# spcl/gms

Measured on AMD Instinct MI355X. Metric: edges-intersected/sec + achieved HBM GB/s, RMAT-26 triangle count @1/2/4/8 GPU, higher is better.
Workload: dtype int32 ids / uint64 counts

## Files before the change

### gms_amd/capi.py

```python
import ctypes as C
import os
import weakref

import numpy as np

_HERE = os.path.dirname(os.path.abspath(__file__))
LIB_PATH = os.environ.get("GMSX_LIB") or os.path.join(_HERE, "lib", "libgmsx.so")

_i64p = np.ctypeslib.ndpointer(np.int64, flags="C_CONTIGUOUS")
_i32p = np.ctypeslib.ndpointer(np.int32, flags="C_CONTIGUOUS")
_u32p = np.ctypeslib.ndpointer(np.uint32, flags="C_CONTIGUOUS")

GEN_KRONECKER, GEN_UNIFORM = 0, 1
RELABEL_NEVER, RELABEL_AUTO, RELABEL_ALWAYS = 0, 1, 2
TC_AUTO, TC_ORIENTED, TC_FULL = 0, 1, 2
UPLOAD_DEFAULT, UPLOAD_TRUSTED, UPLOAD_FOR_TC = 0, 1, 2
PREPARE_TC = 1
SETOP_INTERSECT, SETOP_DIFFERENCE = 0, 1
OK, ERR_INVALID, ERR_NOMEM, ERR_IO, ERR_FORMAT, ERR_DIRECTED, ERR_NO_DEVICE = 0, -1, -2, -3, -4, -5, -6
ERR_DEVICE_MEM, ERR_NOT_CANONICAL, ERR_OVERFLOW, ERR_UNSUPPORTED, ERR_KERNEL, ERR_COMM, ERR_TIMEOUT = -7, -8, -9, -10, -11, -12, -13
COMM_ID_BYTES = 128

SYMBOLS = [
    "gmsx_strerror", "gmsx_version",
# ... 264 lines not shown
        _check(lib().gmsx_csr_save_sgx(self._h, os.fsencode(path)), "gmsx_csr_save_sgx")

    @property
    def is_mapped(self):
        return bool(lib().gmsx_csr_is_mapped(self._h))

    def relabel_by_degree(self):
        h = C.c_void_p()
        _check(lib().gmsx_csr_relabel_by_degree(self._h, C.byref(h)), "gmsx_csr_relabel_by_degree")
        return HostCSR(h)

    def worth_relabelling(self):
        return bool(lib().gmsx_csr_worth_relabelling(self._h))

    @property
    def num_nodes(self):
        return lib().gmsx_csr_num_nodes(self._h)

    @property
    def num_edges(self):
        return lib().gmsx_csr_num_edges(self._h)

    @property
    def nnz(self):
        return lib().gmsx_csr_num_edges_directed(self._h)

    def offsets(self):
        return np.ctypeslib.as_array(lib().gmsx_csr_offsets(self._h), shape=(self.num_nodes + 1,))

    def neighbors(self):
        nnz = self.nnz
        if nnz == 0:
            return np.zeros(0, dtype=np.int32)
        return np.ctypeslib.as_array(lib().gmsx_csr_neighbors(self._h), shape=(nnz,))

    def merge_elements(self):
        return int(lib().gmsx_csr_merge_elements(self._h))

    def fingerprint(self):
        return int(lib().gmsx_csr_fingerprint(self._h, 0)), int(lib().gmsx_csr_fingerprint(self._h, 1))

    def __del__(self):
        if getattr(self, "_h", None):
            lib().gmsx_csr_free(self._h)
            self._h = None


def set_host_threads(n=0):
    return int(lib().gmsx_set_host_threads(int(n)))


def set_option(name, value):
    _check(lib().gmsx_set_option(name.encode(), None if value is None else str(value).encode()), f"gmsx_set_option({name})")


def reset_options():
    lib().gmsx_reset_options()


def option_names():
    out, i, p = [], 0, C.c_char_p()
    while lib().gmsx_option_name(i, C.byref(p)) == 0:
        out.append(p.value.decode())
        i += 1
    return out


class options:

    def __init__(self, **kw):
        self.kw = kw

    def __enter__(self):
        for k, v in self.kw.items():
            set_option(k, v)
        return self

    def __exit__(self, *exc):
        for k in self.kw:
            set_option(k, None)
        return False


def init(device=-1):
    _check(lib().gmsx_init(device), "gmsx_init")


def set_stream(stream_ptr):
    _check(lib().gmsx_set_stream(C.c_void_p(stream_ptr)), "gmsx_set_stream")


def hbm_read_probe(nbytes=4 << 30, iterations=20):
    v = C.c_double(0)
    _check(lib().gmsx_hbm_read_probe(int(nbytes), int(iterations), C.byref(v)), "gmsx_hbm_read_probe")
    return v.value


def device_info():
    name = C.create_string_buffer(256)
    cu, mem = C.c_int(0), C.c_int64(0)
    _check(lib().gmsx_device_info(name, 256, C.byref(cu), C.byref(mem)), "gmsx_device_info")
    return {"name": name.value.decode(), "compute_units": cu.value, "hbm_bytes": mem.value}


class DeviceGraph:

    def __init__(self, handle):
        self._h = handle

    @classmethod
    def upload(cls, off, neigh, flags=UPLOAD_DEFAULT):
        off = np.ascontiguousarray(off, dtype=np.int64)
        neigh = np.ascontiguousarray(neigh, dtype=np.int32)
        h = C.c_void_p()
        _check(lib().gmsx_graph_upload(off.size - 1, off, neigh if neigh.size else np.zeros(1, np.int32), flags, C.byref(h)),
               "gmsx_graph_upload")
        g = cls(h)
        g._host = (weakref.ref(off), weakref.ref(neigh))
        return g

    @classmethod
    def from_csr(cls, csr, flags=UPLOAD_DEFAULT, shard=None):
        h = C.c_void_p()
        if shard is None:
            _check(lib().gmsx_graph_upload_csr(csr._h, flags, C.byref(h)), "gmsx_graph_upload_csr")
        else:
            _check(lib().gmsx_graph_upload_csr_shard(csr._h, flags, int(shard[0]), int(shard[1]), C.byref(h)), "gmsx_graph_upload_csr_shard")
        g = cls(h)
        g._host = (weakref.ref(csr),)
        return g

    num_nodes = property(lambda self: lib().gmsx_graph_num_nodes(self._h))
    num_edges = property(lambda self: lib().gmsx_graph_num_edges(self._h))
    device_bytes = property(lambda self: lib().gmsx_graph_device_bytes(self._h))
    max_out_degree = property(lambda self: lib().gmsx_graph_max_out_degree(self._h))
    tc_passes = property(lambda self: lib().gmsx_graph_tc_passes(self._h))

    def prepare(self, what=PREPARE_TC):
        _check(lib().gmsx_graph_prepare(self._h, what), "gmsx_graph_prepare")

    def tc_total(self, algo=TC_AUTO, stats=False):
        out, st = C.c_uint64(0), Stats()
        _check(lib().gmsx_tc_total(self._h, algo, C.byref(out), C.byref(st)), "gmsx_tc_total")
        return (int(out.value), st.as_dict()) if stats else int(out.value)

    def tc_partial(self, part, nparts, algo=TC_AUTO, stats=False):
        out, st = C.c_uint64(0), Stats()
        _check(lib().gmsx_tc_partial(self._h, algo, part, nparts, C.byref(out), C.byref(st)), "gmsx_tc_partial")
        return (int(out.value), st.as_dict()) if stats else int(out.value)

    BREAKDOWN = ["hub_rows_list", "hub_rows_bitset", "hub_rows_delta", "tail_rows_list", "tail_rows_delta", "entries", "pivot_containers",
                 "of_which_inline_rows", "light_streamed_hub_rows", "light_streamed_tail_rows", "light_pivot_lists_and_descriptors",
                 "count_entries", "count_inline_entries", "count_work_items", "count_light_streamed_members",
                 "core_matrix", "core_k", "reserved17", "reserved18", "reserved19", "reserved20"]
    BREAKDOWN_BYTES = ("hub_rows_list", "hub_rows_bitset", "hub_rows_delta", "tail_rows_list", "tail_rows_delta", "entries", "pivot_containers",
                       "light_streamed_hub_rows", "light_streamed_tail_rows", "light_pivot_lists_and_descriptors", "core_matrix")

    def tc_stream_breakdown(self):
        out = np.zeros(21, dtype=np.uint64)
        _check(lib().gmsx_tc_stream_breakdown(self._h, out), "gmsx_tc_stream_breakdown")
        return dict(zip(self.BREAKDOWN, (int(x) for x in out)))

    def tc_row_histogram(self):
        out = np.zeros(256, dtype=np.uint64)
        _check(lib().gmsx_tc_row_histogram(self._h, out), "gmsx_tc_row_histogram")
        return out[:240].reshape(5, 24, 2).astype(np.int64), out[240:].astype(np.int64)

    def tc_comembership(self, batch):
        out = np.zeros(8, dtype=np.uint64)
        _check(lib().gmsx_tc_comembership(self._h, int(batch), out), "gmsx_tc_comembership")
        return dict(entries=int(out[0]), units=int(out[1]), distinct_rows=int(out[2]), batched_units=int(out[3]), items=int(out[4]))

    def tc_vertex_count2(self, stats=False):
        c, st = np.zeros(self.num_nodes, dtype=np.int64), Stats()
        _check(lib().gmsx_tc_vertex_count2(self._h, c, C.byref(st)), "gmsx_tc_vertex_count2")
        return (c, st.as_dict()) if stats else c

    def intersect_count_batch(self, u, v, stats=False):
        u = np.ascontiguousarray(u, dtype=np.int32)
        v = np.ascontiguousarray(v, dtype=np.int32)
        out, st = np.zeros(max(u.size, 1), dtype=np.uint32), Stats()
        _check(lib().gmsx_intersect_count_batch(self._h, u.size, u if u.size else np.zeros(1, np.int32),
                                                v if v.size else np.zeros(1, np.int32), out, C.byref(st)),
               "gmsx_intersect_count_batch")
        out = out[:u.size]
        return (out, st.as_dict()) if stats else out

    def set_op_batch(self, op, u, v, stats=False):
        code = {"intersect": SETOP_INTERSECT, "difference": SETOP_DIFFERENCE}[op]
        u = np.ascontiguousarray(u, dtype=np.int32)
        v = np.ascontiguousarray(v, dtype=np.int32)
        uu, vv = (u if u.size else np.zeros(1, np.int32)), (v if v.size else np.zeros(1, np.int32))
        off, st = np.zeros(u.size + 1, dtype=np.int64), Stats()
        _check(lib().gmsx_set_op_batch(self._h, code, u.size, uu, vv, off, None, 0, C.byref(st)), "gmsx_set_op_batch (sizing)")
        ids = np.zeros(max(int(off[-1]), 1), dtype=np.int32)
        _check(lib().gmsx_set_op_batch(self._h, code, u.size, uu, vv, off, ids.ctypes.data_as(C.c_void_p), int(off[-1]), C.byref(st)), "gmsx_set_op_batch")
        ids = ids[:int(off[-1])]
        return (off, ids, st.as_dict()) if stats else (off, ids)

    SIM = {"jaccard": 0, "overlap": 1, "adamic_adar": 2, "resource": 3, "common_neighbors": 4, "total_neighbors": 5, "pref_attachment": 6}

    def vertex_similarity_batch(self, metric, u, v, stats=False):
        u = np.ascontiguousarray(u, dtype=np.int32)
        v = np.ascontiguousarray(v, dtype=np.int32)
        out, st = np.zeros(max(u.size, 1), dtype=np.float64), Stats()
        m = self.SIM[metric] if isinstance(metric, str) else int(metric)
        _check(lib().gmsx_vertex_similarity_batch(self._h, m, u.size, u if u.size else np.zeros(1, np.int32),
                                                  v if v.size else np.zeros(1, np.int32), out, C.byref(st)), "gmsx_vertex_similarity_batch")
        out = out[:u.size]
        return (out, st.as_dict()) if stats else out

    def kclique_count(self, k, stats=False):
        ordered, cliques, st = C.c_uint64(0), C.c_uint64(0), Stats()
        _check(lib().gmsx_kclique_count(self._h, k, C.byref(ordered), C.byref(cliques), C.byref(st)), "gmsx_kclique_count")
        r = (int(ordered.value), int(cliques.value))
        return (r + (st.as_dict(),)) if stats else r

    def kclique_star_count(self, k, members=True, stats=False):
        stars, mem, st = C.c_uint64(0), C.c_uint64(0), Stats()
        _check(lib().gmsx_kclique_star_count(self._h, k, C.byref(stars), C.byref(mem) if members else None, C.byref(st)), "gmsx_kclique_star_count")
        r = (int(stars.value), int(mem.value) if members else None)
        return (r + (st.as_dict(),)) if stats else r

    def kclique_star_list_info(self, k, cliques_only=False, part=0, nparts=1):
        info = KcliqueStarListInfo()
        flags = KCSTAR_CLIQUES_ONLY if cliques_only else KCSTAR_DEFAULT
        _check(lib().gmsx_kclique_star_list(self._h, k, flags, part, nparts, None, None, None, 0, 0, C.byref(info), None),
               "gmsx_kclique_star_list (sizing)")
        return info.as_dict()

    def kclique_star_list(self, k, cliques_only=False, part=0, nparts=1, stats=False):
        info, st = KcliqueStarListInfo(), Stats()
        flags = KCSTAR_CLIQUES_ONLY if cliques_only else KCSTAR_DEFAULT
        _check(lib().gmsx_kclique_star_list(self._h, k, flags, part, nparts, None, None, None, 0, 0, C.byref(info), C.byref(st)),
               "gmsx_kclique_star_list (sizing)")
        sizing = st.as_dict()
        nc, nm = int(info.cliques), int(info.star_members)
        cl = np.zeros(max(nc * k, 1), dtype=np.int32)
        soff = mem = None
        if not cliques_only:
            soff = np.zeros(nc + 1, dtype=np.int64)
            mem = np.zeros(max(nm, 1), dtype=np.int32)
        _check(lib().gmsx_kclique_star_list(self._h, k, flags, part, nparts, cl.ctypes.data_as(C.c_void_p),
                                            None if cliques_only else soff.ctypes.data_as(C.c_void_p),
                                            None if cliques_only else mem.ctypes.data_as(C.c_void_p), nc, nm, C.byref(info), C.byref(st)),
               "gmsx_kclique_star_list")
        cl = cl[:nc * k].reshape(nc, k)
        if mem is not None:
            mem = mem[:nm]
        if stats:
            return cl, soff, mem, {"sizing": sizing, "fill": st.as_dict(), "info": info.as_dict()}
        return cl, soff, mem

    def kclique_partial(self, k, part, nparts, stats=False):
        out, st = C.c_uint64(0), Stats()
        _check(lib().gmsx_kclique_partial(self._h, k, part, nparts, C.byref(out), C.byref(st)), "gmsx_kclique_partial")
        return (int(out.value), st.as_dict()) if stats else int(out.value)

    def bk_count(self, rank=None, stats=False):
        out, st = C.c_uint64(0), Stats()
        rp = None
        if rank is not None:
            rank = np.ascontiguousarray(rank, dtype=np.int32)
            rp = rank.ctypes.data_as(C.c_void_p)
        _check(lib().gmsx_bk_count(self._h, rp, C.byref(out), C.byref(st)), "gmsx_bk_count")
        return (int(out.value), st.as_dict()) if stats else int(out.value)

    def bk_partial(self, part, nparts, rank=None, stats=False):
        out, st = C.c_uint64(0), Stats()
        rp = None
        if rank is not None:
            rank = np.ascontiguousarray(rank, dtype=np.int32)
            rp = rank.ctypes.data_as(C.c_void_p)
        _check(lib().gmsx_bk_partial(self._h, rp, part, nparts, C.byref(out), C.byref(st)), "gmsx_bk_partial")
        return (int(out.value), st.as_dict()) if stats else int(out.value)

    def bk_list_info(self, rank=None, part=0, nparts=1):
        info = BkListInfo()
        rp = None
        if rank is not None:
            rank = np.ascontiguousarray(rank, dtype=np.int32)
            rp = rank.ctypes.data_as(C.c_void_p)
        _check(lib().gmsx_bk_list(self._h, rp, part, nparts, None, None, 0, 0, C.byref(info), None), "gmsx_bk_list (sizing)")
        return info.as_dict()

    def bk_list(self, rank=None, part=0, nparts=1, stats=False):
        info, st = BkListInfo(), Stats()
        rp = None
        if rank is not None:
            rank = np.ascontiguousarray(rank, dtype=np.int32)
            rp = rank.ctypes.data_as(C.c_void_p)
        _check(lib().gmsx_bk_list(self._h, rp, part, nparts, None, None, 0, 0, C.byref(info), C.byref(st)), "gmsx_bk_list (sizing)")
        sizing = st.as_dict()
        off = np.zeros(int(info.cliques) + 1, dtype=np.int64)
        mem = np.zeros(max(int(info.members), 1), dtype=np.int32)
        _check(lib().gmsx_bk_list(self._h, rp, part, nparts, off.ctypes.data_as(C.c_void_p), mem.ctypes.data_as(C.c_void_p), off.size,
                                  int(info.members), C.byref(info), C.byref(st)), "gmsx_bk_list")
        mem = mem[:int(info.members)]
        if stats:
            return off, mem, {"sizing": sizing, "fill": st.as_dict(), "info": info.as_dict()}
        return off, mem

    def adg_rank(self, epsilon=0.001, rank_format=True, stats=False):
        out, rounds, st = np.zeros(max(self.num_nodes, 1), dtype=np.int32), C.c_int32(0), Stats()
        _check(lib().gmsx_adg_rank(self._h, float(epsilon), int(bool(rank_format)), out, C.byref(rounds), C.byref(st)), "gmsx_adg_rank")
        r = (out[:self.num_nodes], int(rounds.value))
        return (r + (st.as_dict(),)) if stats else r
# ... 182 lines not shown
```

### gms_amd/csrc/hip/device_graph.hip

```cpp
#include "device_graph.hpp"

#include <algorithm>
#include <mutex>
#include <array>
#include <chrono>
#include <cstdio>
#include <cstdlib>
#include <cstring>
#include <memory>
#include <new>
#include <random>

#include <rocprim/device/device_radix_sort.hpp>
#include <rocprim/device/device_scan.hpp>
#include <rocprim/device/device_segmented_radix_sort.hpp>
#include <rocprim/iterator/transform_iterator.hpp>

#include "../host/gmsx_internal.hpp"
#include "../host/tc_core_plan.hpp"
#include "kc4_mfma.hpp"

namespace gmsx {

Ctx &ctx() {
// ... 235 lines not shown
            int rf = kFormList;
            if (rl >= 24 && delta_mode > 0) {
                const uint32_t d = delta_encode(hadj + b + k, rl, nullptr);
                if (d * 100u <= r * uint32_t(delta_pct)) { r = d; rf = kFormDelta; }
            }
            const uint32_t cand = uint32_t(B / 128) + r;
            if (cand < tot && (hybrid_mode == 2 || cand * 100u <= best * 90u)) {
                tot = cand;
                ks = k;
                best2 = r;
                form2 = rf;
            }
        }
        if (ks > 0) {
            best = tot - best2;
            form = kFormBitset;
        }
    }
    ksplit[v] = ks;
    const uint32_t u2[2] = {best, best2};
    const int f2[2] = {form, form2};
    for (int sl = 0; sl < 2; ++sl) {
        const bool big = u2[sl] >= 8u;
        units_out[2 * v + sl] = big ? int64_t((u2[sl] + 7u) & ~7u) : 0;
        small_out[2 * v + sl] = big ? 0 : int64_t(u2[sl]);
        real_out[2 * v + sl] = u2[sl];
        form_out[2 * v + sl] = (unsigned char)f2[sl];
    }
}
__global__ void k_srow_fill(int64_t n, const int64_t *__restrict__ hoff, const uint16_t *__restrict__ hadj, const int64_t *__restrict__ bmoff,
                            const uint32_t *__restrict__ bmpool, const int64_t *__restrict__ uoff, const int64_t *__restrict__ soff,
                            const uint32_t *__restrict__ real, const unsigned char *__restrict__ form, const int32_t *__restrict__ ksplit,
                            unsigned long long *__restrict__ srow, unsigned long long *__restrict__ srow2, uint32_t *__restrict__ spool) {
    const int64_t v = int64_t(blockIdx.x) * blockDim.x + threadIdx.x;
    if (v >= n) return;
    const int64_t b = hoff[v];
    const int len = int(hoff[v + 1] - b);
    const int ks = ksplit[v];
    for (int sl = 0; sl < 2; ++sl) {
        const int64_t units = int64_t(real[2 * v + sl]);
        const int64_t u0 = units >= 8 ? uoff[2 * v + sl] : uoff[2 * n] + soff[2 * v + sl];
        const int fm = form[2 * v + sl];
        const unsigned long long d = units ? ((unsigned long long)u0 << 24) | ((unsigned long long)fm << 22) | (unsigned long long)units : 0ull;
        if (sl == 0) srow[v] = units ? d : ((unsigned long long)u0 << 24) | ((unsigned long long)fm << 22);
        else srow2[v] = d;
        if (units == 0) continue;
        uint32_t *dst = spool + u0 * 4;
        const uint16_t *row = hadj + b + (sl ? ks : 0);
        const int rl = sl ? len - ks : len;
        if (sl == 0 && ks > 0) {
            for (int64_t w = 0; w < units * 4; ++w) dst[w] = 0;
            for (int i = 0; i < ks; ++i) dst[row[i] >> 5] |= 1u << (row[i] & 31u);
        } else if (fm == kFormDelta) {
            delta_encode(row, rl, dst);
        } else if (fm == kFormGap12) {
            gap12_encode(row, rl, dst);
        } else if (fm == kFormBitset) {
            const uint32_t *src = bmpool + bmoff[v];
            for (int64_t w = 0; w < units * 4; ++w) dst[w] = src[w];
        } else {
            for (int64_t w = 0; w < units * 4; ++w) {
                const int i = int(w) * 2;
                const uint32_t lo = i < rl ? row[i] : 0xFFFFu, hi = i + 1 < rl ? row[i + 1] : 0xFFFFu;
                dst[w] = lo | (hi << 16);
            }
        }
    }
}

__device__ inline uint32_t tail_delta_encode(const int32_t *__restrict__ row, int len, uint32_t *__restrict__ emit) {
    uint32_t units = 0;
    int i = 0;
    while (i < len) {
        uint32_t w[4] = {uint32_t(row[i]), 0u, 0u, 0u};
        uint32_t cur = uint32_t(row[i]);
        int slot = 1;
        ++i;
        while (i < len && slot < 6) {
            const uint32_t gap = uint32_t(row[i]) - cur;
            if (gap > 65535u) break;
            w[1 + (slot >> 1)] |= gap << ((slot & 1) * 16);
            ++slot;
            cur = uint32_t(row[i]);
            ++i;
        }
        w[1] |= uint32_t(slot);
        if (emit) {
            emit[units * 4 + 0] = w[0]; emit[units * 4 + 1] = w[1]; emit[units * 4 + 2] = w[2]; emit[units * 4 + 3] = w[3];
        }
        ++units;
    }
    return units;
}
__global__ void k_trow_sizes(int64_t n, const int64_t *__restrict__ toff, const int32_t *__restrict__ tadj, int delta_mode,
                             int64_t *__restrict__ units_out, int64_t *__restrict__ small_out, uint32_t *__restrict__ real_out, unsigned char *__restrict__ form_out) {
    const int64_t v = int64_t(blockIdx.x) * blockDim.x + threadIdx.x;
    if (v > n) return;
    if (v == n) { units_out[n] = 0; small_out[n] = 0; return; }
    const int64_t b = toff[v];
    const int len = int(toff[v + 1] - b);
    uint32_t best = uint32_t((len + 3) / 4);
    int form = kFormList;
    if (len >= 8 && delta_mode > 0) {
        const uint32_t d = tail_delta_encode(tadj + b, len, nullptr);
        if (delta_mode == 2 || d * 100u <= best * 85u) { best = d; form = kFormDelta; }
    }
    const bool big = best >= 8u;
    units_out[v] = big ? int64_t((best + 7u) & ~7u) : 0;
    small_out[v] = big ? 0 : int64_t(best);
    real_out[v] = best;
    form_out[v] = (unsigned char)form;
}
__global__ void k_trow_fill(int64_t n, const int64_t *__restrict__ toff, const int32_t *__restrict__ tadj, const int64_t *__restrict__ uoff,
                            const int64_t *__restrict__ soff, const uint32_t *__restrict__ real, const unsigned char *__restrict__ form,
                            unsigned long long *__restrict__ trow, uint32_t *__restrict__ tpool) {
    const int64_t v = int64_t(blockIdx.x) * blockDim.x + threadIdx.x;
    if (v >= n) return;
    const int64_t units = int64_t(real[v]);
    const int64_t u0 = units >= 8 ? uoff[v] : uoff[n] + soff[v];
    trow[v] = ((unsigned long long)u0 << 24) | ((unsigned long long)form[v] << 22) | (unsigned long long)units;
    if (units == 0) return;
    uint32_t *dst = tpool + u0 * 4;
    const int64_t b = toff[v];
    const int64_t len = toff[v + 1] - b;
    if (form[v] == kFormDelta) tail_delta_encode(tadj + b, int(len), dst);
    else
        for (int64_t w = 0; w < units * 4; ++w) dst[w] = w < len ? uint32_t(tadj[b + w]) : 0xfffffffeu;
}

__global__ void k_dense_sizes(int32_t limit, const int32_t *__restrict__ dplus, int64_t *__restrict__ sizes) {
    const int32_t v = int32_t(blockIdx.x * blockDim.x + threadIdx.x);
    if (v < limit) sizes[v] = bitset_words(v);
    if (v == limit) sizes[v] = 0;
}
__global__ __launch_bounds__(256) void k_dense_fill(int32_t limit, const int64_t *__restrict__ hoff, const uint16_t *__restrict__ hadj,
                                                    const int64_t *__restrict__ toff, const int32_t *__restrict__ tadj,
                                                    const int64_t *__restrict__ bmoff, uint32_t *__restrict__ pool) {
    const int lane = threadIdx.x & 63;
    const int32_t wave0 = int32_t((int64_t(blockIdx.x) * blockDim.x + threadIdx.x) >> 6);
    const int32_t nwaves = int32_t((int64_t(gridDim.x) * blockDim.x) >> 6);
    for (int32_t v = wave0; v < limit; v += nwaves) {
        const int64_t b = bmoff[v];
        if (bmoff[v + 1] == b) continue;
        for (int64_t j = hoff[v] + lane; j < hoff[v + 1]; j += 64) {
            const uint32_t id = hadj[j];
            if (id != 0xFFFFu) atomicOr(&pool[b + (id >> 5)], 1u << (id & 31u));
        }
        for (int64_t j = toff[v] + lane; j < toff[v + 1]; j += 64) {
            const uint32_t id = uint32_t(tadj[j]);
            atomicOr(&pool[b + (id >> 5)], 1u << (id & 31u));
        }
    }
}
__global__ __launch_bounds__(256) void k_core_fill(int32_t K, int WS, const int64_t *__restrict__ hoff, const uint16_t *__restrict__ hadj,
                                                   uint32_t *__restrict__ bits) {
    const int lane = threadIdx.x & 63;
    const int32_t wave0 = int32_t((int64_t(blockIdx.x) * blockDim.x + threadIdx.x) >> 6);
    const int32_t nwaves = int32_t((int64_t(gridDim.x) * blockDim.x) >> 6);
    for (int32_t i = wave0; i < K; i += nwaves)
        for (int64_t j = hoff[i] + lane; j < hoff[i + 1]; j += 64) {
            const uint32_t id = hadj[j];
            if (id < uint32_t(i)) atomicOr(&bits[size_t(i) * size_t(WS) + (id >> 5)], 1u << (id & 31u));
        }
}
__global__ __launch_bounds__(256) void k_core_units(int32_t cap, const int64_t *__restrict__ hoff, const uint16_t *__restrict__ hadj,
                                                    const int32_t *__restrict__ dplus, unsigned long long *__restrict__ bucket) {
    const int lane = threadIdx.x & 63;
    const int32_t wave0 = int32_t((int64_t(blockIdx.x) * blockDim.x + threadIdx.x) >> 6);
    const int32_t nwaves = int32_t((int64_t(gridDim.x) * blockDim.x) >> 6);
    for (int32_t u = wave0; u < cap; u += nwaves) {
        const int64_t hb = hoff[u];
        const int hl = int(hoff[u + 1] - hb);
        unsigned long long units = 0;
        for (int i = lane; i < hl; i += 64) {
            const uint32_t v = hadj[hb + i];
            if (v >= uint32_t(u)) continue;
            const uint32_t ids = uint32_t(min(i, dplus[v]));
            units += min((ids + 7u) / 8u, (v + 127u) / 128u);
        }
        for (int s = 32; s > 0; s >>= 1) units += __shfl_down(units, s);
        if (lane == 0 && units) atomicAdd(&bucket[u / kTcCoreBucket], units);
    }
}
__global__ __launch_bounds__(256) void k_tail_split(int64_t n, const int64_t *__restrict__ toff, const int32_t *__restrict__ tadj, int32_t limit,
                                                    int32_t *__restrict__ tsplit) {
    const int lane = threadIdx.x & 63;
    const int64_t wave0 = (int64_t(blockIdx.x) * blockDim.x + threadIdx.x) >> 6;
    const int64_t nwaves = (int64_t(gridDim.x) * blockDim.x) >> 6;
    for (int64_t u = wave0; u < n; u += nwaves) {
        int c = 0;
        for (int64_t j = toff[u] + lane; j < toff[u + 1]; j += 64) c += tadj[j] < limit;
        for (int s = 32; s > 0; s >>= 1) c += __shfl_down(c, s);
        if (lane == 0) tsplit[u] = c;
    }
}

__global__ void k_order_keys(int64_t n, const int32_t *__restrict__ dplus, int32_t *__restrict__ keys, int32_t *__restrict__ vals) {
    const int64_t i = int64_t(blockIdx.x) * blockDim.x + threadIdx.x;
    if (i < n) {
        keys[i] = dplus[i];
        vals[i] = int32_t(i);
    }
}

__global__ void k_warm(unsigned long long *p) {
    if (p) p[0] = 0;
}
__global__ void k_count_ge(int64_t n, const int32_t *__restrict__ order, const int32_t *__restrict__ dplus, int32_t thr, int64_t *__restrict__ out) {
    int64_t lo = 0, hi = n;
    while (lo < hi) {
        const int64_t mid = (lo + hi) >> 1;
        if (dplus[order[mid]] >= thr) lo = mid + 1; else hi = mid;
    }
    out[0] = lo;
}
__global__ void k_task_limits(int64_t n, const unsigned long long *__restrict__ srow, const unsigned long long *__restrict__ srow2,
                              const unsigned long long *__restrict__ trow, uint32_t hub_max, uint32_t tail_max, unsigned long long *__restrict__ out) {
    const int64_t v = int64_t(blockIdx.x) * blockDim.x + threadIdx.x;
    if (v >= n) return;
    if ((srow[v] & 0x3fffffull) > hub_max || (srow2[v] & 0x3fffffull) > hub_max || (trow[v] & 0x3fffffull) > tail_max) atomicOr(out, 1ull);
}

static constexpr int kInlineChunk = 64;
static constexpr int kDefaultInlineFirst = 28;
static constexpr int kInlineFirstMax = 64;
__device__ __forceinline__ bool takes_inline(int32_t v, int32_t inline_limit, const int32_t *__restrict__ dplus) {
    return v < inline_limit || dplus[v] >= kHeavy;
}
template <bool FILL>
__global__ __launch_bounds__(256) void k_inline_rows(int64_t first, int64_t end, const int32_t *__restrict__ order, const int64_t *__restrict__ hoff,
                                                     const uint16_t *__restrict__ hadj, const int64_t *__restrict__ toff, const int32_t *__restrict__ tadj,
                                                     const int32_t *__restrict__ dplus, int32_t inline_limit, int inline_first, int32_t core, const int32_t *__restrict__ opos, int nparts, int part,
                                                     unsigned long long *__restrict__ cnt_h,
                                                     unsigned long long *__restrict__ cnt_t, const int64_t *__restrict__ ihoff,
                                                     const int64_t *__restrict__ itoff, int64_t base_h, uint16_t *__restrict__ pool_h, int64_t base_t,
                                                     int32_t *__restrict__ pool_t) {
    const int lane = threadIdx.x & 63;
    const int64_t wave0 = (int64_t(blockIdx.x) * blockDim.x + threadIdx.x) >> 6;
    const int64_t nwaves = (int64_t(gridDim.x) * blockDim.x) >> 6;
    for (int64_t pos = first + wave0; pos < end; pos += nwaves) {
        const int32_t u = order[pos];
        if (u < core) continue;
        const int64_t hb = hoff[u], tb = toff[u];
        const int first_u = dplus[u] >= kHeavy ? inline_first : kInlineFirstMax;
        const int hl = min(int(hoff[u + 1] - hb), first_u), tl = min(int(toff[u + 1] - tb), first_u - hl);
        int32_t mv = 0x7fffffff;
        if (lane < hl) {
            const uint32_t x = hadj[hb + lane];
            if (x != 0xFFFFu) mv = int32_t(x);
        } else if (lane - hl < tl) {
            mv = tadj[tb + (lane - hl)];
        }
        const bool valid = mv != 0x7fffffff, is_tail = valid && lane >= hl;
        const unsigned long long vmask = __ballot(valid);
        const int nhub = __popcll(__ballot(valid && lane < hl));
        const int below = __popcll(vmask & ((1ull << lane) - 1ull));
        const bool give = valid && below > 0 && takes_inline(mv, inline_limit, dplus);
        const bool mine = give && (nparts <= 1 || shard_of(opos[mv], nparts) == part);
        const int nh = mine ? (is_tail ? nhub : below) : 0;
        const int nt = mine && is_tail ? lane - hl : 0;
        if (!FILL) {
            if (nh) atomicAdd(&cnt_h[mv], (unsigned long long)nh);
            if (nt) atomicAdd(&cnt_t[mv], (unsigned long long)nt);
        } else {
            int64_t at_h = 0, at_t = 0;
            if (nh) at_h = (base_h + ihoff[mv]) * 8 + int64_t(atomicAdd(&cnt_h[mv], (unsigned long long)nh));
            if (nt) at_t = (base_t + itoff[mv]) * 4 + int64_t(atomicAdd(&cnt_t[mv], (unsigned long long)nt));
            for (int k = 0; k < nhub; ++k) {
                const int32_t x = __shfl(mv, k);
                if (k < nh) pool_h[at_h + k] = uint16_t(x);
            }
            for (int k = 0; k < tl; ++k) {
                const int32_t x = __shfl(mv, hl + k);
                if (k < nt) pool_t[at_t + k] = x;
            }
        }
    }
}
__global__ void k_inline_units(int64_t n, const unsigned long long *__restrict__ ids_h, const unsigned long long *__restrict__ ids_t,
                               int64_t *__restrict__ units_h, int64_t *__restrict__ units_t) {
    const int64_t v = int64_t(blockIdx.x) * blockDim.x + threadIdx.x;
    if (v > n) return;
    units_h[v] = v < n ? int64_t((ids_h[v] + 7) / 8) : 0;
    units_t[v] = v < n ? int64_t((ids_t[v] + 3) / 4) : 0;
}
static constexpr int kDefaultHotWindows = 0, kDefaultHotKB = 2048, kDefaultHotMin = 16;
__device__ __forceinline__ int64_t receiver_of(int32_t w, const int32_t *__restrict__ dplus, const int32_t *__restrict__ opos, const int64_t *__restrict__ lidx,
                                               int64_t n_heavy) {
    return dplus[w] >= kHeavy ? int64_t(opos[w]) : n_heavy + lidx[w];
}
__global__ void k_opos(int64_t n, const int32_t *__restrict__ order, int32_t *__restrict__ opos) {
    const int64_t p = int64_t(blockIdx.x) * blockDim.x + threadIdx.x;
    if (p < n) opos[order[p]] = int32_t(p);
}
__global__ void k_light_flags(int64_t limit, const int32_t *__restrict__ dplus, int64_t *__restrict__ flags) {
    const int64_t w = int64_t(blockIdx.x) * blockDim.x + threadIdx.x;
    if (w <= limit) flags[w] = (w < limit && dplus[w] < kHeavy) ? 1 : 0;
}
__global__ void k_recv_vertices(int64_t n_heavy, int64_t limit, const int32_t *__restrict__ order, const int32_t *__restrict__ dplus, const int64_t *__restrict__ lidx,
                                int32_t *__restrict__ recv_v) {
    const int64_t i = int64_t(blockIdx.x) * blockDim.x + threadIdx.x;
    if (i < n_heavy) recv_v[i] = order[i];
    if (i < limit && dplus[i] < kHeavy) recv_v[n_heavy + lidx[i]] = int32_t(i);
}
template <bool FILL>
__global__ void k_inline_entries(int64_t n, const int32_t *__restrict__ dplus, const int32_t *__restrict__ opos, const int64_t *__restrict__ lidx, int64_t n_heavy,
                                 int32_t inline_limit, const int64_t *__restrict__ ihoff, const int64_t *__restrict__ itoff, int64_t base_h, int64_t base_t,
                                 uint32_t *__restrict__ cnt, uint32_t *__restrict__ cur, const int64_t *__restrict__ hbeg, const int64_t *__restrict__ tbeg,
                                 TaskList htask, TaskList ttask, unsigned long long *__restrict__ totals, TcClasses cc) {
    const int kClasses = cc.count();
    const int64_t v = int64_t(blockIdx.x) * blockDim.x + threadIdx.x;
    if (v >= n) return;
    const int64_t uh = ihoff[v + 1] - ihoff[v], ut = itoff[v + 1] - itoff[v];
    if (uh == 0 && ut == 0) return;
    if (dplus[v] < kHeavy && v >= inline_limit) return;
    const int64_t p = receiver_of(int32_t(v), dplus, opos, lidx, n_heavy);
    uint32_t *c = cnt + p * kClasses;
    for (int64_t o = 0; o < uh; o += kInlineChunk) {
        const unsigned long long units = (unsigned long long)min(int64_t(kInlineChunk), uh - o);
        const unsigned long long d = ((unsigned long long)(base_h + ihoff[v] + o) << 24) | ((unsigned long long)kFormList << 22) | units;
        const int cls = hub_class(cc, d);
        if (!FILL) atomicAdd(&c[cls], 1u);
        else htask.put(hbeg[p] + c[cls] + atomicAdd(&cur[p * kClasses + cls], 1u), d);
    }
    for (int64_t o = 0; o < ut; o += kInlineChunk) {
        const unsigned long long units = (unsigned long long)min(int64_t(kInlineChunk), ut - o);
        const unsigned long long d = ((unsigned long long)(base_t + itoff[v] + o) << 24) | ((unsigned long long)kFormList << 22) | units;
        const int cls = tail_class(cc, d);
        if (!FILL) atomicAdd(&c[cls], 1u);
        else ttask.put(tbeg[p] + c[cls] + atomicAdd(&cur[p * kClasses + cls], 1u), d);
    }
    if (!FILL) {
        atomicAdd(&totals[0], (unsigned long long)((uh + kInlineChunk - 1) / kInlineChunk));
        atomicAdd(&totals[1], (unsigned long long)((ut + kInlineChunk - 1) / kInlineChunk));
    }
}
__global__ void k_list_sizes(int64_t n_recv, uint32_t *__restrict__ cnt, int64_t *__restrict__ hcnt, int64_t *__restrict__ tcnt, TcClasses cc) {
    const int kClasses = cc.count(), hub_end = cc.tail_base();
    const int64_t p = int64_t(blockIdx.x) * blockDim.x + threadIdx.x;
    if (p > n_recv) return;
    if (p == n_recv) { hcnt[p] = 0; tcnt[p] = 0; return; }
    uint32_t *c = cnt + p * kClasses;
    uint32_t run = 0;
    for (int k = 0; k < hub_end; ++k) { const uint32_t x = c[k]; c[k] = run; run += x; }
    hcnt[p] = run;
    run = 0;
    for (int k = hub_end; k < kClasses; ++k) { const uint32_t x = c[k]; c[k] = run; run += x; }
    tcnt[p] = run;
}

__global__ void k_ledge_count(int64_t first, int64_t end, const int32_t *__restrict__ order, const int64_t *__restrict__ toff, const int32_t *__restrict__ tadj,
                              const int32_t *__restrict__ tsplit, const int32_t *__restrict__ dplus, int32_t core, int64_t *__restrict__ cnt) {
    const int64_t pos = first + int64_t(blockIdx.x) * blockDim.x + threadIdx.x;
    if (pos > end) return;
    int64_t c = 0;
    if (pos < end) {
        const int32_t u = order[pos];
        const int64_t tb = toff[u];
        const int tl = int(toff[u + 1] - tb);
        if (u >= core)
            for (int i = tsplit[u]; i < tl; ++i) c += dplus[tadj[tb + i]] < kHeavy ? 1 : 0;
    }
    cnt[pos - first] = c;
}
__global__ void k_ledge_fill(int64_t first, int64_t end, const int32_t *__restrict__ order, const int64_t *__restrict__ hoff, const int64_t *__restrict__ toff,
                             const int32_t *__restrict__ tadj, const int32_t *__restrict__ tsplit, const int32_t *__restrict__ dplus,
                             int32_t core, const int64_t *__restrict__ ebeg, int nparts, int part, uint4 *__restrict__ ledge) {
    const int64_t pos = first + int64_t(blockIdx.x) * blockDim.x + threadIdx.x;
    if (pos >= end) return;
    const int32_t u = order[pos];
    if (u < core) return;
    const int64_t hb = hoff[u], tb = toff[u];
    const int tl = int(toff[u + 1] - tb);
    const unsigned long long hu = (unsigned long long)hb | ((unsigned long long)(hoff[u + 1] - hb) << 40);
    int64_t e = ebeg[pos - first];
    for (int i = tsplit[u]; i < tl; ++i) {
        const int32_t v = tadj[tb + i];
        if (dplus[v] >= kHeavy) continue;
        if (nparts <= 1 || shard_of(e, nparts) == part) {
            const unsigned long long tu = (unsigned long long)tb | ((unsigned long long)i << 40);
            const unsigned long long hv = (unsigned long long)hoff[v] | ((unsigned long long)(hoff[v + 1] - hoff[v]) << 40);
            const unsigned long long tv = (unsigned long long)toff[v] | ((unsigned long long)(toff[v + 1] - toff[v]) << 40);
            const int64_t slot = nparts <= 1 ? e : e / nparts;
            ledge[2 * slot] = make_uint4(uint32_t(hu), uint32_t(hu >> 32), uint32_t(tu), uint32_t(tu >> 32));
            ledge[2 * slot + 1] = make_uint4(uint32_t(hv), uint32_t(hv >> 32), uint32_t(tv), uint32_t(tv >> 32));
        }
        ++e;
    }
}

__device__ __forceinline__ uint32_t cut_hub_units(const uint32_t *__restrict__ spool, unsigned long long d, int below, int32_t v) {
    const uint32_t units = uint32_t(d) & 0x3fffffu, form = (uint32_t(d) >> 22) & 3u;
    if (form == kFormList) return min(units, uint32_t(below + 7) / 8u);
    if (form == kFormBitset) return min(units, uint32_t(v + 127) / 128u);
    const uint4 *row = reinterpret_cast<const uint4 *>(spool) + (d >> 24);
    uint32_t lo = 0, hi = units;
    while (lo < hi) {
        const uint32_t mid = (lo + hi) >> 1;
        if (int32_t(row[mid].x & 0xffffu) < v) lo = mid + 1; else hi = mid;
    }
    return lo;
}
__device__ __forceinline__ uint32_t cut_tail_units(const uint32_t *__restrict__ tpool, unsigned long long d, int below, int32_t v) {
    const uint32_t units = uint32_t(d) & 0x3fffffu, form = (uint32_t(d) >> 22) & 3u;
    if (form != kFormDelta) return min(units, uint32_t(below + 3) / 4u);
    const uint4 *row = reinterpret_cast<const uint4 *>(tpool) + (d >> 24);
    uint32_t lo = 0, hi = units;
    while (lo < hi) {
        const uint32_t mid = (lo + hi) >> 1;
        if (int32_t(row[mid].x) < v) lo = mid + 1; else hi = mid;
    }
    return lo;
}
__device__ __forceinline__ uint32_t claim_by_class(uint32_t *ctr, int cls, bool active, int lane) {
    uint32_t mine = 0;
    unsigned long long todo = __ballot(active);
    while (todo) {
        const int leader = __ffsll((long long)todo) - 1;
        const int c = __builtin_amdgcn_readlane(cls, leader);
        const unsigned long long same = __ballot(active && cls == c);
        uint32_t base = 0;
        if (lane == leader) base = atomicAdd(&ctr[c], uint32_t(__popcll(same)));
        base = uint32_t(__builtin_amdgcn_readlane(int(base), leader));
        if (active && cls == c) mine = base + uint32_t(__popcll(same & ((1ull << lane) - 1ull)));
        todo &= ~same;
    }
    return mine;
}
template <bool FILL>
__global__ __launch_bounds__(256) void k_task_lists(int64_t n_heavy, const int32_t *__restrict__ order, const int64_t *__restrict__ hoff,
                                                    const uint16_t *__restrict__ hadj, const int64_t *__restrict__ toff, const int32_t *__restrict__ tadj,
                                                    const int32_t *__restrict__ dplus, const unsigned long long *__restrict__ srow,
                                                    const unsigned long long *__restrict__ srow2, const int32_t *__restrict__ ksplit,
                                                    const unsigned long long *__restrict__ trow, int two_sided, const int32_t *__restrict__ opos,
                                                    uint32_t *__restrict__ cnt, uint32_t *__restrict__ cur, const int64_t *__restrict__ hbeg,
                                                    const int64_t *__restrict__ tbeg, TaskList htask, TaskList ttask,
                                                    int32_t *__restrict__ tunits, unsigned long long *__restrict__ reversed, const uint32_t *__restrict__ spool,
                                                    const uint32_t *__restrict__ tpool, int32_t inline_limit, int inline_first, int32_t core, int nparts, int part, TcClasses cc) {
    const int kClasses = cc.count();
    const int lane = threadIdx.x & 63;
    const int64_t wave0 = (int64_t(blockIdx.x) * blockDim.x + threadIdx.x) >> 6;
    const int64_t nwaves = (int64_t(gridDim.x) * blockDim.x) >> 6;
    unsigned long long rev = 0;
    for (int64_t pos = wave0; pos < n_heavy; pos += nwaves) {
        const int32_t u = order[pos];
        if (u < core) continue;
        const int64_t hb = hoff[u], tb = toff[u];
        const int hl = int(hoff[u + 1] - hb), tl = int(toff[u + 1] - tb);
        const unsigned long long du_s = srow[u], du_s2 = srow2[u], du_t = trow[u];
        const int ks_u = ksplit[u];
        uint32_t *cu = cnt + pos * kClasses, *ru = cur + pos * kClasses;
        const bool own_u = nparts <= 1 || shard_of(pos, nparts) == part;
        int kept = 0;
        for (int base = 0; base < hl + tl; base += 64) {
            const int i = base + lane;
            int32_t v = -1;
            if (i < hl) {
                const uint32_t x = hadj[hb + i];
                if (x != 0xFFFFu) v = int32_t(x);
            } else if (i < hl + tl) v = tadj[tb + i - hl];
            if (v >= 0 && i > 0 && i < inline_first && takes_inline(v, inline_limit, dplus)) v = -1;
            bool reverse = false;
            uint32_t ch = 0, ch2 = 0, ct = 0;
            if (v >= 0 && i > 0 && two_sided && dplus[v] >= kHeavy) {
                if (i < hl) {
                    ch = cut_hub_units(spool, du_s, i, v);
                    if (du_s2 && i > ks_u) ch2 = cut_hub_units(spool, du_s2, i - ks_u, v);
                } else {
                    ch = uint32_t(du_s) & 0x3fffffu;
                    ch2 = uint32_t(du_s2) & 0x3fffffu;
                }
                ct = (i < hl || toff[v + 1] == toff[v]) ? 0u : cut_tail_units(tpool, du_t, i - hl, v);
                const uint32_t keep = uint32_t(srow[v] & 0x3fffffull) + uint32_t(srow2[v] & 0x3fffffull) + (i > hl ? uint32_t(trow[v] & 0x3fffffull) : 0u);
                reverse = ch + ch2 + ct < keep;
            }
            const bool fwd = v >= 0 && !reverse && own_u;
            if (reverse && nparts > 1 && shard_of(opos[v], nparts) != part) v = -1;
            const unsigned long long fh = (fwd && i > 0) ? srow[v] : 0ull, fh2 = (fwd && i > 0) ? srow2[v] : 0ull, ft = (fwd && i > hl) ? trow[v] : 0ull;
            const bool fh_on = (fh & 0x3fffffull) != 0, fh2_on = (fh2 & 0x3fffffull) != 0, ft_on = (ft & 0x3fffffull) != 0;
            const uint32_t sh = claim_by_class(FILL ? ru : cu, hub_class(cc, fh), fh_on, lane);
            const uint32_t sh2 = claim_by_class(FILL ? ru : cu, hub_class(cc, fh2), fh2_on, lane);
            const uint32_t st = claim_by_class(FILL ? ru : cu, tail_class(cc, ft), ft_on, lane);
            if (FILL) {
                if (fh_on) htask.put(hbeg[pos] + cu[hub_class(cc, fh)] + sh, fh);
                if (fh2_on) htask.put(hbeg[pos] + cu[hub_class(cc, fh2)] + sh2, fh2);
                if (ft_on) ttask.put(tbeg[pos] + cu[tail_class(cc, ft)] + st, ft);
            }
            kept += __popcll(__ballot(fwd));
            if (v >= 0 && reverse) {
                const int64_t pv = opos[v];
                const unsigned long long rh = ch ? (du_s & ~0x3fffffull) | ch : 0ull, rh2 = ch2 ? (du_s2 & ~0x3fffffull) | ch2 : 0ull,
                                         rt = ct ? (du_t & ~0x3fffffull) | ct : 0ull;
                uint32_t *cv = cnt + pv * kClasses;
                if (!FILL) {
                    if (rh) atomicAdd(&cv[hub_class(cc, rh)], 1u);
                    if (rh2) atomicAdd(&cv[hub_class(cc, rh2)], 1u);
                    if (rt) atomicAdd(&cv[tail_class(cc, rt)], 1u);
                    atomicAdd(&tunits[pv], 1);
                    ++rev;
                } else {
                    uint32_t *rv = cur + pv * kClasses;
                    if (rh) htask.put(hbeg[pv] + cv[hub_class(cc, rh)] + atomicAdd(&rv[hub_class(cc, rh)], 1u), rh);
                    if (rh2) htask.put(hbeg[pv] + cv[hub_class(cc, rh2)] + atomicAdd(&rv[hub_class(cc, rh2)], 1u), rh2);
                    if (rt) ttask.put(tbeg[pv] + cv[tail_class(cc, rt)] + atomicAdd(&rv[tail_class(cc, rt)], 1u), rt);
                }
            }
        }
        if (!FILL && lane == 0 && kept) atomicAdd(&tunits[pos], kept);
    }
    if (!FILL) {
        for (int s = 32; s > 0; s >>= 1) rev += __shfl_down(rev, s);
        if (lane == 0 && rev) atomicAdd(reversed, rev);
    }
}
__global__ void k_item_counts(int64_t n_recv, const int64_t *__restrict__ lbeg, const uint32_t *__restrict__ cnt, TcClasses cc, int phases, int64_t *__restrict__ items) {
    const int64_t p = int64_t(blockIdx.x) * blockDim.x + threadIdx.x;
    if (p > n_recv) return;
    if (p == n_recv) { items[int64_t(phases) * n_recv] = 0; return; }
    for (int ph = 0; ph < phases; ++ph) {
        int64_t b = 0, e = lbeg[p + 1] - lbeg[p];
        if (phases > 1) hub_phase_range(cc, cnt + p * cc.count(), e, ph, &b, &e);
        items[int64_t(ph) * n_recv + p] = (e - b + kTaskChunk - 1) / kTaskChunk;
    }
}
__global__ void k_item_fill(int64_t n_recv, const int32_t *__restrict__ recv_v, const int32_t *__restrict__ opos, const int64_t *__restrict__ lbeg,
                            const int64_t *__restrict__ ioff, TaskList task, const int64_t *__restrict__ coff, int kind,
                            const uint32_t *__restrict__ cnt, TcClasses cc, int phases, gmsx_tc_item *__restrict__ items) {
    const int64_t p = int64_t(blockIdx.x) * blockDim.x + threadIdx.x;
    if (p >= n_recv) return;
    const int32_t w = recv_v[p];
    const uint64_t cont = uint64_t(coff[w]) | (uint64_t(coff[w + 1] - coff[w]) << 40);
    for (int ph = 0; ph < phases; ++ph) {
    int64_t b = 0, e = lbeg[p + 1] - lbeg[p];
    if (phases > 1) hub_phase_range(cc, cnt + p * cc.count(), e, ph, &b, &e);
    b += lbeg[p];
    e += lbeg[p];
    int64_t k = ioff[int64_t(ph) * n_recv + p];
    for (int64_t x = b; x < e; x += kTaskChunk, ++k) {
        const int ne = int(min(int64_t(kTaskChunk), e - x));
        gmsx_tc_item it{};
        it.bc = uint64_t(x) | (uint64_t(ne) << 40);
        it.cont = cont;
        it.pivot = w;
        it.pos = opos[w];
        it.kind = uint32_t(kind);
        for (int f = 0; f < 4; ++f) {
            int lo = 0, hi = ne;
            while (lo < hi) {
                const int mid = (lo + hi) >> 1;
                if (int((uint32_t(task.get(x + mid)) >> 22) & 3u) < f) lo = mid + 1; else hi = mid;
            }
            it.fbeg[f] = uint16_t(lo);
        }
        items[k] = it;
    }
    }
}

static int grid_for_waves(int64_t rows) {
    const int64_t want = (rows + 3) / 4;
    const int64_t cap = int64_t(ctx().compute_units > 0 ? ctx().compute_units : 256) * 32;
    return int(want < 1 ? 1 : (want > cap ? cap : want));
}

template <class T>
static int dmalloc(T **p, int64_t count, gmsx_graph *g, int line = __builtin_LINE()) {
    const size_t bytes = size_t(count > 0 ? count : 1) * sizeof(T);
    const bool trace = opt("MEM_TRACE") != nullptr;
    if (trace && g && bytes >= (1u << 20)) std::fprintf(stderr, "gmsx mem: device_graph.hip:%d %.3f GB (elements of %zu B)\n", line, double(bytes) * 1e-9, sizeof(T));
    if (g && g->tc_building && g->tc_limit_bytes > 0 && g->device_bytes + int64_t(bytes) - g->tc_base_bytes > g->tc_limit_bytes) {
        *p = nullptr;
        return GMSX_ERR_DEVICE_MEM;
    }
    if (hipMalloc(reinterpret_cast<void **>(p), bytes) != hipSuccess) {
        (void)hipGetLastError();
        *p = nullptr;
        return GMSX_ERR_DEVICE_MEM;
    }
    if (g) g->device_bytes += int64_t(bytes);
    return GMSX_OK;
}

struct DevGuard {
    void *p;
    ~DevGuard() { (void)hipFree(p); }
};

static void free_tc(gmsx_graph *g) {
    auto drop = [](auto *&p) {
        (void)hipFree(p);
        p = nullptr;
    };
    drop(g->tsplit); drop(g->srow); drop(g->srow2); drop(g->ksplit); drop(g->spool); drop(g->trow); drop(g->htask.lo); drop(g->htask.hi); drop(g->ttask.lo); drop(g->ttask.hi); drop(g->hitem); drop(g->titem); drop(g->tunits);
    drop(g->ledge); drop(g->tpool); drop(g->shard_hitem); drop(g->shard_titem); drop(g->core_bits);
    g->tc_core = 0;
    g->shard_idx_part = g->shard_idx_nparts = -1;
    g->device_bytes -= g->tc_bytes;
    g->tc_bytes = 0;
    g->tc_ready = false;
    g->htask_entries = g->ttask_entries = g->hitems = g->titems = g->inline_hentries = g->inline_tentries = 0;
    g->n_ledge = g->ledge_total = 0;
    g->task_reverse = g->inline_units = g->spool_units = g->tpool_units = 0;
    g->stats_part = g->stats_nparts = -1;
}

static void free_graph(gmsx_graph *g) {
    if (!g) return;
    (void)hipFree(g->off);
    (void)hipFree(g->adj);
    (void)hipFree(g->newid);
    (void)hipFree(g->oldid);
    (void)hipFree(g->hoff);
    (void)hipFree(g->hadj);
    (void)hipFree(g->toff);
    (void)hipFree(g->tadj);
    (void)hipFree(g->bmoff);
    (void)hipFree(g->bmpool);
    (void)hipFree(g->tsplit);
    (void)hipFree(g->srow);
    (void)hipFree(g->srow2);
    (void)hipFree(g->ksplit);
    (void)hipFree(g->spool);
    (void)hipFree(g->trow);
    (void)hipFree(g->htask.lo);
    (void)hipFree(g->htask.hi);
    (void)hipFree(g->ttask.lo);
    (void)hipFree(g->ttask.hi);
    (void)hipFree(g->hitem);
    (void)hipFree(g->titem);
    (void)hipFree(g->tunits);
    (void)hipFree(g->shard_hitem);
    (void)hipFree(g->shard_titem);
    (void)hipFree(g->ledge);
    (void)hipFree(g->core_bits);
    (void)hipFree(g->tpool);
    (void)hipFree(g->dplus);
    (void)hipFree(g->order);
    (void)hipFree(g->kc_rel);
    (void)hipFree(g->kc_aoff);
    (void)hipFree(g->kc_arena);
    (void)hipFree(g->kc_rec);
    (void)hipFree(g->kc_item);
    (void)hipFree(g->kc_relt);
    (void)hipFree(g->kc_rect);
    (void)hipFree(g->kc_itemt);
    (void)hipFree(g->scratch);
    (void)hipFree(g->acc);
    delete g;
}

int exclusive_scan_i64(const int64_t *in, int64_t *out, int64_t count, hipStream_t s) {
    size_t tmp_bytes = 0;
    GMSX_HIP(rocprim::exclusive_scan(nullptr, tmp_bytes, in, out, int64_t(0), size_t(count), rocprim::plus<int64_t>(), s));
    void *tmp = nullptr;
    GMSX_HIP(hipMalloc(&tmp, tmp_bytes ? tmp_bytes : 8));
    DevGuard g_tmp{tmp};
    GMSX_HIP(rocprim::exclusive_scan(tmp, tmp_bytes, in, out, int64_t(0), size_t(count), rocprim::plus<int64_t>(), s));
    GMSX_HIP(hipStreamSynchronize(s));
    return GMSX_OK;
}

struct OffsetMinus {
    int64_t base;
    __host__ __device__ int64_t operator()(int64_t x) const { return x - base; }
};
__global__ void k_lower_bound_i64(int64_t count, const int64_t *__restrict__ a, int64_t target, int64_t *__restrict__ out) {
    int64_t lo = 0, hi = count;
    while (lo < hi) {
        const int64_t mid = (lo + hi) >> 1;
        if (a[mid] < target) lo = mid + 1; else hi = mid;
    }
    out[0] = lo;
}
template <class K>
static int sort_rows(K *keys, int64_t entries, int64_t n, const int64_t *d_off, int end_bit, hipStream_t s) {
    if (n <= 0 || entries <= 0) return GMSX_OK;
    int64_t chunk = int64_t(1) << 31;
    if (const char *e = opt("SORT_CHUNK")) {
        const long long v = std::atoll(e);
        if (v > 0) chunk = v;
    }
    int64_t *d_v = nullptr;
    GMSX_HIP(hipMalloc(reinterpret_cast<void **>(&d_v), sizeof(int64_t)));
    DevGuard g_v{d_v};
    GMSX_HIP(hipStreamSynchronize(s));
    int64_t v0 = 0, base = 0;
    while (v0 < n) {
        int64_t v1 = n;
        if (entries - base > chunk) {
            hipLaunchKernelGGL(k_lower_bound_i64, dim3(1), dim3(1), 0, s, n + 1, d_off, base + chunk + 1, d_v);
            GMSX_HIP(hipStreamSynchronize(s));
            GMSX_HIP(hipMemcpy(&v1, d_v, sizeof(int64_t), hipMemcpyDeviceToHost));
            v1 = std::max(v0 + 1, std::min(n, v1 - 1));
        }
        int64_t end = 0;
        GMSX_HIP(hipMemcpy(&end, d_off + v1, sizeof(int64_t), hipMemcpyDeviceToHost));
        const int64_t cnt = end - base;
        if (cnt >= (int64_t(1) << 32)) return GMSX_ERR_UNSUPPORTED;
        if (cnt > 0) {
            K *sorted = nullptr;
            GMSX_HIP(hipMalloc(reinterpret_cast<void **>(&sorted), size_t(cnt) * sizeof(K)));
            DevGuard g_sorted{sorted};
            auto begin = rocprim::make_transform_iterator(d_off + v0, OffsetMinus{base});
            auto endit = rocprim::make_transform_iterator(d_off + v0 + 1, OffsetMinus{base});
            size_t tmp_bytes = 0;
            GMSX_HIP(rocprim::segmented_radix_sort_keys(nullptr, tmp_bytes, keys + base, sorted, unsigned(cnt), unsigned(v1 - v0), begin, endit, 0, end_bit, s));
            void *tmp = nullptr;
            GMSX_HIP(hipMalloc(&tmp, tmp_bytes ? tmp_bytes : 8));
            DevGuard g_tmp{tmp};
            GMSX_HIP(rocprim::segmented_radix_sort_keys(tmp, tmp_bytes, keys + base, sorted, unsigned(cnt), unsigned(v1 - v0), begin, endit, 0, end_bit, s));
            GMSX_HIP(hipMemcpyAsync(keys + base, sorted, size_t(cnt) * sizeof(K), hipMemcpyDeviceToDevice, s));
            GMSX_HIP(hipStreamSynchronize(s));
        }
        v0 = v1;
        base = end;
    }
    return GMSX_OK;
}

template <class K, class V>
static int sort_segment_pairs(K *keys, V *vals, int64_t entries, int64_t n, const int64_t *d_off, int end_bit, hipStream_t s) {
    if (n <= 0 || entries <= 0) return GMSX_OK;
    int64_t chunk = int64_t(1) << 31;
    if (const char *e = opt("SORT_CHUNK")) {
        const long long v = std::atoll(e);
        if (v > 0) chunk = v;
    }
    int64_t *d_v = nullptr;
    GMSX_HIP(hipMalloc(reinterpret_cast<void **>(&d_v), sizeof(int64_t)));
    DevGuard g_v{d_v};
    GMSX_HIP(hipStreamSynchronize(s));
    int64_t v0 = 0, base = 0;
    while (v0 < n) {
        int64_t v1 = n;
        if (entries - base > chunk) {
            hipLaunchKernelGGL(k_lower_bound_i64, dim3(1), dim3(1), 0, s, n + 1, d_off, base + chunk + 1, d_v);
            GMSX_HIP(hipStreamSynchronize(s));
            GMSX_HIP(hipMemcpy(&v1, d_v, sizeof(int64_t), hipMemcpyDeviceToHost));
            v1 = std::max(v0 + 1, std::min(n, v1 - 1));
        }
        int64_t end = 0;
        GMSX_HIP(hipMemcpy(&end, d_off + v1, sizeof(int64_t), hipMemcpyDeviceToHost));
        const int64_t cnt = end - base;
        if (cnt >= (int64_t(1) << 32)) return GMSX_ERR_UNSUPPORTED;
        if (cnt > 0) {
            K *k_out = nullptr;
            V *v_out = nullptr;
            GMSX_HIP(hipMalloc(reinterpret_cast<void **>(&k_out), size_t(cnt) * sizeof(K)));
            DevGuard g_ko{k_out};
            GMSX_HIP(hipMalloc(reinterpret_cast<void **>(&v_out), size_t(cnt) * sizeof(V)));
            DevGuard g_vo{v_out};
            auto begin = rocprim::make_transform_iterator(d_off + v0, OffsetMinus{base});
            auto endit = rocprim::make_transform_iterator(d_off + v0 + 1, OffsetMinus{base});
            size_t tmp_bytes = 0;
            GMSX_HIP(rocprim::segmented_radix_sort_pairs(nullptr, tmp_bytes, keys + base, k_out, vals + base, v_out, unsigned(cnt), unsigned(v1 - v0), begin, endit, 0,
                                                         end_bit, s));
            void *tmp = nullptr;
            GMSX_HIP(hipMalloc(&tmp, tmp_bytes ? tmp_bytes : 8));
            DevGuard g_tmp{tmp};
            GMSX_HIP(rocprim::segmented_radix_sort_pairs(tmp, tmp_bytes, keys + base, k_out, vals + base, v_out, unsigned(cnt), unsigned(v1 - v0), begin, endit, 0,
                                                         end_bit, s));
            GMSX_HIP(hipMemcpyAsync(vals + base, v_out, size_t(cnt) * sizeof(V), hipMemcpyDeviceToDevice, s));
            GMSX_HIP(hipStreamSynchronize(s));
        }
        v0 = v1;
        base = end;
    }
    return GMSX_OK;
}

struct PhaseTimer {
    hipStream_t s;
    bool on;
    std::chrono::steady_clock::time_point t0;
    const char *what;
    PhaseTimer(hipStream_t st, const char *w) : s(st), on(opt("TIMING") != nullptr), t0(std::chrono::steady_clock::now()), what(w) {}
    void mark(const char *phase) {
        if (!on) return;
        (void)hipStreamSynchronize(s);
        const auto t1 = std::chrono::steady_clock::now();
        std::fprintf(stderr, "[gmsx %s] %-28s %8.1f ms\n", what, phase, std::chrono::duration<double, std::milli>(t1 - t0).count());
        t0 = t1;
    }
};

static constexpr size_t kH2dChunk = size_t(64) << 20;
struct H2dStage {
// ... 44 lines not shown
        used[b] = true;
    }
    return GMSX_OK;
}

static int build_device_sets(gmsx_graph *g, uint32_t flags) {
    hipStream_t s = ctx().stream;
    PhaseTimer pt(s, "base build");
    const int64_t n = g->n;
    if (int rc = dmalloc(&g->scratch, 16, g)) return rc;
    if (int rc = dmalloc(&g->acc, kAccWords, g)) return rc;
    GMSX_HIP(hipMemsetAsync(g->scratch, 0, 16 * sizeof(unsigned long long), s));

    const int check_sym = (flags & GMSX_UPLOAD_TRUSTED) ? 0 : 1;
    static const std::array<unsigned long long, 2> sym_keys = []() noexcept {
        try {
            std::random_device rd;
            return std::array<unsigned long long, 2>{((unsigned long long)rd() << 32) | rd(), ((unsigned long long)rd() << 32) | rd()};
        } catch (...) {
            const unsigned long long t = (unsigned long long)std::chrono::steady_clock::now().time_since_epoch().count();
            const unsigned long long a = (unsigned long long)reinterpret_cast<uintptr_t>(&t);
            return std::array<unsigned long long, 2>{t * 0x9E3779B97F4A7C15ull ^ a, (a * 0xC2B2AE3D27D4EB4Full) ^ (t << 17)};
        }
    }();
    if (n > 0)
        hipLaunchKernelGGL(k_validate, dim3(grid_for_waves(n)), dim3(256), 0, s, n, g->off, g->adj, check_sym, sym_keys[0], sym_keys[1], g->scratch);
    unsigned long long acc[7] = {0, 0, 0, 0, 0, 0, 0};
    GMSX_HIP(hipMemcpyAsync(acc, g->scratch, sizeof(acc), hipMemcpyDeviceToHost, s));
    GMSX_HIP(hipStreamSynchronize(s));
    if (check_sym && (acc[3] != acc[4] || acc[5] != acc[6])) acc[0] |= 8;
    if (!(flags & GMSX_UPLOAD_TRUSTED) && acc[0] != 0) return GMSX_ERR_NOT_CANONICAL;
    if ((flags & GMSX_UPLOAD_TRUSTED) && (acc[0] & 2)) return GMSX_ERR_NOT_CANONICAL;
    if (!(flags & GMSX_UPLOAD_TRUSTED) && (g->nnz & 1)) return GMSX_ERR_NOT_CANONICAL;
    g->alg_elements = acc[1];
    g->max_deg = int32_t(acc[2]);
    g->m = g->nnz / 2;

    pt.mark("validate");
    const unsigned tb = unsigned((n + 255) / 256);
    if (int rc = dmalloc(&g->newid, n, g)) return rc;
    if (int rc = dmalloc(&g->oldid, n, g)) return rc;
    if (n > 0) {
        unsigned long long *k_in = nullptr, *k_out = nullptr;
        if (int rc = dmalloc(&k_in, n, nullptr)) return rc;
        DevGuard g1{k_in};
        if (int rc = dmalloc(&k_out, n, nullptr)) return rc;
        DevGuard g2{k_out};
        hipLaunchKernelGGL(k_rank_keys, dim3(tb), dim3(256), 0, s, n, g->off, k_in);
        size_t tmp_bytes = 0;
        GMSX_HIP(rocprim::radix_sort_keys_desc(nullptr, tmp_bytes, k_in, k_out, size_t(n), 0, 64, s));
        void *tmp = nullptr;
        GMSX_HIP(hipMalloc(&tmp, tmp_bytes ? tmp_bytes : 8));
        DevGuard g3{tmp};
        GMSX_HIP(rocprim::radix_sort_keys_desc(tmp, tmp_bytes, k_in, k_out, size_t(n), 0, 64, s));
        hipLaunchKernelGGL(k_assign_ids, dim3(tb), dim3(256), 0, s, n, k_out, g->oldid, g->newid);
        GMSX_HIP(hipStreamSynchronize(s));
    }

    pt.mark("rank ids");
    int hub_limit = int((flags >> 8) & 0xffffu);
    if (hub_limit == 0 || hub_limit > kHub) hub_limit = kHub;
    int64_t *hcnt = nullptr, *tcnt = nullptr;
    if (int rc = dmalloc(&hcnt, n + 1, nullptr)) return rc;
    DevGuard g_h{hcnt};
    if (int rc = dmalloc(&tcnt, n + 1, nullptr)) return rc;
    DevGuard g_t{tcnt};
    GMSX_HIP(hipMemsetAsync(hcnt, 0, size_t(n + 1) * sizeof(int64_t), s));
    GMSX_HIP(hipMemsetAsync(tcnt, 0, size_t(n + 1) * sizeof(int64_t), s));
    if (int rc = dmalloc(&g->dplus, n, g)) return rc;
    if (n > 0)
        hipLaunchKernelGGL(k_count_parts, dim3(grid_for_waves(n)), dim3(256), 0, s, n, g->off, g->adj, g->newid, hub_limit, hcnt, tcnt, g->dplus);
    if (int rc = dmalloc(&g->hoff, n + 1, g)) return rc;
    if (int rc = dmalloc(&g->toff, n + 1, g)) return rc;
    if (int rc = exclusive_scan_i64(hcnt, g->hoff, n + 1, s)) return rc;
    if (int rc = exclusive_scan_i64(tcnt, g->toff, n + 1, s)) return rc;
    GMSX_HIP(hipMemcpy(&g->hub_entries, g->hoff + n, sizeof(int64_t), hipMemcpyDeviceToHost));
    GMSX_HIP(hipMemcpy(&g->tail_entries, g->toff + n, sizeof(int64_t), hipMemcpyDeviceToHost));

    if (int rc = dmalloc(&g->hadj, g->hub_entries + 8, g)) return rc;
    if (int rc = dmalloc(&g->tadj, g->tail_entries + 4, g)) return rc;
    GMSX_HIP(hipMemsetAsync(g->hadj + g->hub_entries, 0xff, 8 * sizeof(uint16_t), s));
    GMSX_HIP(hipMemsetAsync(g->tadj + g->tail_entries, 0xff, 4 * sizeof(int32_t), s));
    if (n > 0)
        hipLaunchKernelGGL(k_fill_parts, dim3(grid_for_waves(n)), dim3(256), 0, s, n, g->off, g->adj, g->newid, hub_limit, g->hoff, g->toff,
                           g->hadj, g->tadj);

    pt.mark("containers count+fill");
    if (int rc = sort_rows(g->hadj, g->hub_entries, n, g->hoff, 16, s)) return rc;
    if (int rc = sort_rows(g->tadj, g->tail_entries, n, g->toff, 32, s)) return rc;
    g->rows_sorted = true;

    pt.mark("row sorts");
    g->dense_limit = int32_t(std::min<int64_t>(n, hub_limit));
    g->bitset_limit = g->dense_limit;
    {
        const int32_t K = g->bitset_limit;
        int64_t *sizes = nullptr;
        if (int rc = dmalloc(&sizes, int64_t(K) + 1, nullptr)) return rc;
        DevGuard g_sz{sizes};
        if (int rc = dmalloc(&g->bmoff, int64_t(K) + 1, g)) return rc;
        hipLaunchKernelGGL(k_dense_sizes, dim3(unsigned(K / 256 + 1)), dim3(256), 0, s, K, g->dplus, sizes);
        if (int rc = exclusive_scan_i64(sizes, g->bmoff, int64_t(K) + 1, s)) return rc;
        GMSX_HIP(hipMemcpy(&g->bmpool_words, g->bmoff + K, sizeof(int64_t), hipMemcpyDeviceToHost));
        if (int rc = dmalloc(&g->bmpool, g->bmpool_words + 4, g)) return rc;
        GMSX_HIP(hipMemsetAsync(g->bmpool, 0, size_t(g->bmpool_words + 4) * sizeof(uint32_t), s));
        if (K > 0 && g->bmpool_words > 0)
            hipLaunchKernelGGL(k_dense_fill, dim3(grid_for_waves(K)), dim3(256), 0, s, K, g->hoff, g->hadj, g->toff, g->tadj, g->bmoff, g->bmpool);
    }
    pt.mark("bitsets");
    if (int rc = dmalloc(&g->order, n, g)) return rc;
    if (n > 0) {
        int32_t *keys_in = nullptr, *vals_in = nullptr, *keys_out = nullptr;
        if (int rc = dmalloc(&keys_out, n, nullptr)) return rc;
        DevGuard g_ko{keys_out};
        if (int rc = dmalloc(&keys_in, n, nullptr)) return rc;
        DevGuard g_ki{keys_in};
        if (int rc = dmalloc(&vals_in, n, nullptr)) return rc;
        DevGuard g_vi{vals_in};
        hipLaunchKernelGGL(k_order_keys, dim3(tb), dim3(256), 0, s, n, g->dplus, keys_in, vals_in);
        size_t tmp_bytes = 0;
        GMSX_HIP(rocprim::radix_sort_pairs_desc(nullptr, tmp_bytes, keys_in, keys_out, vals_in, g->order, size_t(n), 0, 32, s));
        void *tmp = nullptr;
        GMSX_HIP(hipMalloc(&tmp, tmp_bytes ? tmp_bytes : 8));
        DevGuard g_tmp{tmp};
        GMSX_HIP(rocprim::radix_sort_pairs_desc(tmp, tmp_bytes, keys_in, keys_out, vals_in, g->order, size_t(n), 0, 32, s));
        int32_t top = 0;
        GMSX_HIP(hipMemcpyAsync(&top, keys_out, sizeof(int32_t), hipMemcpyDeviceToHost, s));
        GMSX_HIP(hipStreamSynchronize(s));
        g->max_dplus = top;
    }

    pt.mark("d+ order");
    GMSX_HIP(hipStreamSynchronize(s));
    GMSX_HIP(hipGetLastError());
    g->hub_limit = hub_limit;
    g->upload_flags = flags;
    return GMSX_OK;
}

static int build_tc_sets(gmsx_graph *g) {
    hipStream_t s = ctx().stream;
    PhaseTimer pt(s, "tc build");
    const int64_t n = g->n;
    const uint32_t flags = g->upload_flags;
    const int hub_limit = g->hub_limit;
    const unsigned tb = unsigned((n + 255) / 256);
    int32_t *opos = nullptr;
    if (int rc = dmalloc(&opos, n + 1, nullptr)) return rc;
    DevGuard g_opos{opos};
    if (n > 0) hipLaunchKernelGGL(k_opos, dim3(tb), dim3(256), 0, s, n, g->order, opos);
    {
        long long want = kTcCoreDefault;
        if (const char *e = opt("TC_CORE")) want = std::atoll(e);
        g->tc_core = 0;
        if (want > 0) g->tc_core = tc_core_clamp(want, hub_limit, n);
        else if (want < 0) {
            const int cap = tc_core_clamp(kTcCoreCap, hub_limit, n) / kTcCoreBucket * kTcCoreBucket;
            if (cap > 0) {
                const int nbk = cap / kTcCoreBucket;
                unsigned long long *bucket = nullptr;
                if (int rc = dmalloc(&bucket, nbk, nullptr)) return rc;
                DevGuard g_b{bucket};
                GMSX_HIP(hipMemsetAsync(bucket, 0, size_t(nbk) * sizeof(unsigned long long), s));
                hipLaunchKernelGGL(k_core_units, dim3(grid_for_waves(cap)), dim3(256), 0, s, cap, g->hoff, g->hadj, g->dplus, bucket);
                std::vector<uint64_t> h(size_t(nbk), 0);
                static_assert(sizeof(uint64_t) == sizeof(unsigned long long), "bucket words");
                GMSX_HIP(hipMemcpyAsync(h.data(), bucket, size_t(nbk) * sizeof(uint64_t), hipMemcpyDeviceToHost, s));
                GMSX_HIP(hipStreamSynchronize(s));
                g->tc_core = choose_tc_core(h, cap);
            }
        }
        if (g->tc_core > 0) {
            const int32_t K = g->tc_core;
            const int WS = kc4m_stride(K);
            const int64_t words = int64_t(K) * WS + 8;
            if (int rc = dmalloc(&g->core_bits, words, g)) return rc;
            GMSX_HIP(hipMemsetAsync(g->core_bits, 0, size_t(words) * sizeof(uint32_t), s));
            hipLaunchKernelGGL(k_core_fill, dim3(grid_for_waves(K)), dim3(256), 0, s, K, WS, g->hoff, g->hadj, g->core_bits);
        }
    }
    pt.mark("core matrix");
    {
        int64_t want = std::min<int64_t>(524288, n / 256);
        bool forced = false;
        if (const char *e = opt("INLINE_LIMIT")) {
            const long long v = std::atoll(e);
            if (v >= 0 && v <= (1ll << 31) - 1) { want = v; forced = true; }
        }
        if (!forced && ((flags >> 8) & 0xffffu)) want = int64_t(4) * hub_limit;
        g->inline_limit = int32_t(std::min<int64_t>(n, std::max<int64_t>(want, g->dense_limit)));
        g->inline_first = kDefaultInlineFirst;
        if (const char *e = opt("TC_INLINE_FIRST")) g->inline_first = std::max(1, std::min(kInlineFirstMax, std::atoi(e)));
        if (int rc = dmalloc(&g->tsplit, n, g)) return rc;
        if (n > 0) hipLaunchKernelGGL(k_tail_split, dim3(grid_for_waves(n)), dim3(256), 0, s, n, g->toff, g->tadj, g->inline_limit, g->tsplit);
    }

    pt.mark("tail split");
    int64_t n_heavy = 0, n_work = 0;
    unsigned long long *inl_h = nullptr, *inl_t = nullptr;
    int64_t *ihoff = nullptr, *itoff = nullptr;
    if (int rc = dmalloc(&inl_h, n + 1, nullptr)) return rc;
    DevGuard g_inl_h{inl_h};
    if (int rc = dmalloc(&inl_t, n + 1, nullptr)) return rc;
    DevGuard g_inl_t{inl_t};
    if (int rc = dmalloc(&ihoff, n + 1, nullptr)) return rc;
    DevGuard g_ihoff{ihoff};
    if (int rc = dmalloc(&itoff, n + 1, nullptr)) return rc;
    DevGuard g_itoff{itoff};
    int64_t inline_h_units = 0, inline_t_units = 0;
    {
        if (n > 0) {
            int64_t *d_cnt = nullptr;
            if (int rc = dmalloc(&d_cnt, 2, nullptr)) return rc;
            DevGuard g_c{d_cnt};
            hipLaunchKernelGGL(k_count_ge, dim3(1), dim3(1), 0, s, n, g->order, g->dplus, int32_t(kHeavy), d_cnt);
            hipLaunchKernelGGL(k_count_ge, dim3(1), dim3(1), 0, s, n, g->order, g->dplus, int32_t(2), d_cnt + 1);
            GMSX_HIP(hipStreamSynchronize(s));
            int64_t h[2] = {0, 0};
            GMSX_HIP(hipMemcpy(h, d_cnt, sizeof(h), hipMemcpyDeviceToHost));
            n_heavy = h[0];
            n_work = h[1];
        }
        GMSX_HIP(hipMemsetAsync(inl_h, 0, size_t(n + 1) * sizeof(unsigned long long), s));
        GMSX_HIP(hipMemsetAsync(inl_t, 0, size_t(n + 1) * sizeof(unsigned long long), s));
        if (n_work > 0)
            hipLaunchKernelGGL(k_inline_rows<false>, dim3(grid_for_waves(n_work)), dim3(256), 0, s, int64_t(0), n_work, g->order, g->hoff, g->hadj,
                               g->toff, g->tadj, g->dplus, g->inline_limit, g->inline_first, g->tc_core, opos, g->shard_nparts, g->shard_part, inl_h, inl_t, ihoff, itoff, int64_t(0), static_cast<uint16_t *>(nullptr),
                               int64_t(0), static_cast<int32_t *>(nullptr));
        int64_t *uh = nullptr, *ut = nullptr;
        if (int rc = dmalloc(&uh, n + 1, nullptr)) return rc;
        DevGuard g_uh{uh};
        if (int rc = dmalloc(&ut, n + 1, nullptr)) return rc;
        DevGuard g_ut{ut};
        hipLaunchKernelGGL(k_inline_units, dim3(unsigned(n / 256 + 1)), dim3(256), 0, s, n, inl_h, inl_t, uh, ut);
        if (int rc = exclusive_scan_i64(uh, ihoff, n + 1, s)) return rc;
        if (int rc = exclusive_scan_i64(ut, itoff, n + 1, s)) return rc;
        GMSX_HIP(hipMemcpy(&inline_h_units, ihoff + n, sizeof(int64_t), hipMemcpyDeviceToHost));
        GMSX_HIP(hipMemcpy(&inline_t_units, itoff + n, sizeof(int64_t), hipMemcpyDeviceToHost));
        g->inline_units = inline_h_units + inline_t_units;
    }

    pt.mark("inline row sizes");
    int64_t inline_h_base = 0, inline_t_base = 0;
    {
        int delta_mode = g->rows_sorted ? 1 : 0;
        if (const char *e = opt("TC_DELTA")) {
            const int v = std::atoi(e);
            if (v >= 0 && v <= 2 && g->rows_sorted) delta_mode = v;
        }
        int delta_pct = 85;
        if (const char *e = opt("TC_DELTA_PCT")) {
            const int v = std::atoi(e);
            if (v >= 10 && v <= 100) delta_pct = v;
        }
        int gap12_mode = 0;
        if (const char *e = opt("TC_GAP12")) {
            const int v = std::atoi(e);
            if (v >= 0 && v <= 2 && g->rows_sorted) gap12_mode = v;
        }
        int hybrid_mode = 0;
        if (const char *e = opt("TC_HYBRID")) {
            const int v = std::atoi(e);
            if (v >= 0 && v <= 2 && g->rows_sorted) hybrid_mode = v;
        }
        int64_t *units = nullptr, *uoff = nullptr, *small = nullptr, *soff = nullptr;
        uint32_t *real = nullptr;
        unsigned char *form = nullptr;
        const int64_t n2 = 2 * n;
        if (int rc = dmalloc(&units, n2 + 1, nullptr)) return rc;
        DevGuard g_u{units};
        if (int rc = dmalloc(&uoff, n2 + 1, nullptr)) return rc;
        DevGuard g_o{uoff};
        if (int rc = dmalloc(&small, n2 + 1, nullptr)) return rc;
        DevGuard g_s{small};
        if (int rc = dmalloc(&soff, n2 + 1, nullptr)) return rc;
        DevGuard g_so{soff};
        if (int rc = dmalloc(&real, n2 + 1, nullptr)) return rc;
        DevGuard g_r{real};
        if (int rc = dmalloc(&form, n2 + 1, nullptr)) return rc;
        DevGuard g_f{form};
        if (int rc = dmalloc(&g->ksplit, n + 1, g)) return rc;
        hipLaunchKernelGGL(k_srow_sizes, dim3(unsigned(n / 256 + 1)), dim3(256), 0, s, n, g->hoff, g->hadj, g->dplus, g->dense_limit, delta_mode, delta_pct, gap12_mode,
                           hybrid_mode, units, small, real, form, g->ksplit);
        if (int rc = exclusive_scan_i64(units, uoff, n2 + 1, s)) return rc;
        if (int rc = exclusive_scan_i64(small, soff, n2 + 1, s)) return rc;
        int64_t big_units = 0, small_units = 0;
        GMSX_HIP(hipMemcpy(&big_units, uoff + n2, sizeof(int64_t), hipMemcpyDeviceToHost));
        GMSX_HIP(hipMemcpy(&small_units, soff + n2, sizeof(int64_t), hipMemcpyDeviceToHost));
        g->spool_units = big_units + small_units + inline_h_units;
        inline_h_base = big_units + small_units;
        if (g->spool_units >= (int64_t(1) << 40)) return GMSX_ERR_DEVICE_MEM;
        if (int rc = dmalloc(&g->srow, n, g)) return rc;
        if (int rc = dmalloc(&g->srow2, n, g)) return rc;
        if (int rc = dmalloc(&g->spool, (g->spool_units + kPoolSlack) * 4, g)) return rc;
        GMSX_HIP(hipMemsetAsync(g->spool, 0, size_t((g->spool_units + kPoolSlack) * 4) * sizeof(uint32_t), s));
        if (inline_h_units > 0) GMSX_HIP(hipMemsetAsync(g->spool + inline_h_base * 4, 0xff, size_t(inline_h_units) * 16, s));
        if (n > 0)
            hipLaunchKernelGGL(k_srow_fill, dim3(unsigned((n + 255) / 256)), dim3(256), 0, s, n, g->hoff, g->hadj, g->bmoff, g->bmpool, uoff, soff, real, form,
                               g->ksplit, g->srow, g->srow2, g->spool);
        GMSX_HIP(hipStreamSynchronize(s));
    }
    {
        int delta_mode = g->rows_sorted ? 1 : 0;
        if (const char *e = opt("TC_TAIL_DELTA")) {
            const int v = std::atoi(e);
            if (v >= 0 && v <= 2 && g->rows_sorted) delta_mode = v;
        }
        int64_t *units = nullptr, *uoff = nullptr, *small = nullptr, *soff = nullptr;
        uint32_t *real = nullptr;
        unsigned char *form = nullptr;
        if (int rc = dmalloc(&units, n + 1, nullptr)) return rc;
        DevGuard g_u{units};
        if (int rc = dmalloc(&uoff, n + 1, nullptr)) return rc;
        DevGuard g_o{uoff};
        if (int rc = dmalloc(&small, n + 1, nullptr)) return rc;
        DevGuard g_s{small};
        if (int rc = dmalloc(&soff, n + 1, nullptr)) return rc;
        DevGuard g_so{soff};
        if (int rc = dmalloc(&real, n + 1, nullptr)) return rc;
        DevGuard g_r{real};
        if (int rc = dmalloc(&form, n + 1, nullptr)) return rc;
        DevGuard g_f{form};
        hipLaunchKernelGGL(k_trow_sizes, dim3(unsigned(n / 256 + 1)), dim3(256), 0, s, n, g->toff, g->tadj, delta_mode, units, small, real, form);
        if (int rc = exclusive_scan_i64(units, uoff, n + 1, s)) return rc;
        if (int rc = exclusive_scan_i64(small, soff, n + 1, s)) return rc;
        int64_t big_units = 0, small_units = 0;
        GMSX_HIP(hipMemcpy(&big_units, uoff + n, sizeof(int64_t), hipMemcpyDeviceToHost));
        GMSX_HIP(hipMemcpy(&small_units, soff + n, sizeof(int64_t), hipMemcpyDeviceToHost));
        inline_t_base = big_units + small_units;
        g->tpool_units = inline_t_base + inline_t_units;
        if (g->tpool_units >= (int64_t(1) << 40)) return GMSX_ERR_DEVICE_MEM;
        if (int rc = dmalloc(&g->trow, n, g)) return rc;
        if (int rc = dmalloc(&g->tpool, (g->tpool_units + kPoolSlack) * 4, g)) return rc;
        GMSX_HIP(hipMemsetD32Async(reinterpret_cast<hipDeviceptr_t>(g->tpool), int(0xFFFFFFFEu), size_t(g->tpool_units + kPoolSlack) * 4, s));
        if (n > 0)
            hipLaunchKernelGGL(k_trow_fill, dim3(unsigned((n + 255) / 256)), dim3(256), 0, s, n, g->toff, g->tadj, uoff, soff, real, form, g->trow, g->tpool);
        GMSX_HIP(hipStreamSynchronize(s));
    }

    pt.mark("tail stream rows");
    if (n_work > 0) {
        GMSX_HIP(hipMemsetAsync(inl_h, 0, size_t(n + 1) * sizeof(unsigned long long), s));
        GMSX_HIP(hipMemsetAsync(inl_t, 0, size_t(n + 1) * sizeof(unsigned long long), s));
        hipLaunchKernelGGL(k_inline_rows<true>, dim3(grid_for_waves(n_work)), dim3(256), 0, s, int64_t(0), n_work, g->order, g->hoff, g->hadj, g->toff,
                           g->tadj, g->dplus, g->inline_limit, g->inline_first, g->tc_core, opos, g->shard_nparts, g->shard_part, inl_h, inl_t, ihoff, itoff, inline_h_base, reinterpret_cast<uint16_t *>(g->spool),
                           inline_t_base, reinterpret_cast<int32_t *>(g->tpool));
    }
    pt.mark("inline rows fill");
    {
        const int64_t nl = n_work - n_heavy;
        g->n_ledge = g->ledge_total = 0;
        if (nl > 0) {
            int64_t *ecnt = nullptr, *ebeg = nullptr;
            if (int rc = dmalloc(&ecnt, nl + 1, nullptr)) return rc;
            DevGuard g_ec{ecnt};
            if (int rc = dmalloc(&ebeg, nl + 1, nullptr)) return rc;
            DevGuard g_eb{ebeg};
            hipLaunchKernelGGL(k_ledge_count, dim3(unsigned(nl / 256 + 1)), dim3(256), 0, s, n_heavy, n_work, g->order, g->toff, g->tadj, g->tsplit, g->dplus, g->tc_core, ecnt);
            if (int rc = exclusive_scan_i64(ecnt, ebeg, nl + 1, s)) return rc;
            GMSX_HIP(hipMemcpy(&g->ledge_total, ebeg + nl, sizeof(int64_t), hipMemcpyDeviceToHost));
            const int np = g->shard_nparts > 1 ? g->shard_nparts : 1, pp = g->shard_nparts > 1 ? g->shard_part : 0;
            {
                const int64_t full = g->ledge_total / np, rem = g->ledge_total % np;
                g->n_ledge = np <= 1 ? g->ledge_total : full + (((full & 1) ? np - 1 - pp : pp) < rem ? 1 : 0);
            }
            if (int rc = dmalloc(&g->ledge, 2 * g->n_ledge + 2, g)) return rc;
            hipLaunchKernelGGL(k_ledge_fill, dim3(unsigned(nl / 256 + 1)), dim3(256), 0, s, n_heavy, n_work, g->order, g->hoff, g->toff, g->tadj, g->tsplit, g->dplus, g->tc_core, ebeg,
                               np, pp, g->ledge);
            GMSX_HIP(hipStreamSynchronize(s));
        }
    }
    pt.mark("light pivot list");
    {
        int two_sided = 1;
        if (const char *e = opt("TC_TWO_SIDED")) two_sided = std::atoi(e) != 0;
        const unsigned vb = unsigned(n / 256 + 1);
        const int64_t L = g->inline_limit;
        int64_t *lflag = nullptr, *lidx = nullptr;
        if (int rc = dmalloc(&lflag, L + 1, nullptr)) return rc;
        DevGuard g_lf{lflag};
        if (int rc = dmalloc(&lidx, L + 1, nullptr)) return rc;
        DevGuard g_li{lidx};
        hipLaunchKernelGGL(k_light_flags, dim3(unsigned(L / 256 + 1)), dim3(256), 0, s, L, g->dplus, lflag);
        if (int rc = exclusive_scan_i64(lflag, lidx, L + 1, s)) return rc;
        int64_t n_light_recv = 0;
        GMSX_HIP(hipMemcpy(&n_light_recv, lidx + L, sizeof(int64_t), hipMemcpyDeviceToHost));
        const int64_t n_recv = n_heavy + n_light_recv;
        int32_t *recv_v = nullptr;
        if (int rc = dmalloc(&recv_v, n_recv + 1, nullptr)) return rc;
        DevGuard g_rv{recv_v};
        if (std::max<int64_t>(n_heavy, L) > 0)
            hipLaunchKernelGGL(k_recv_vertices, dim3(unsigned(std::max<int64_t>(n_heavy, L) / 256 + 1)), dim3(256), 0, s, n_heavy, L, g->order, g->dplus, lidx, recv_v);
        {
            auto env_int = [](const char *name, int dflt) { return int(opt_int(name, dflt)); };
            g->tc_hot_windows = std::max(0, std::min(kMaxHotWindows, env_int("TC_HOT_WINDOWS", kDefaultHotWindows)));
            g->tc_window_units = uint32_t(std::max(1, env_int("TC_HOT_KB", kDefaultHotKB))) * 64u;
            g->tc_hot_min = std::max(1, env_int("TC_HOT_MIN", kDefaultHotMin));
        }
        const TcClasses cc{g->tc_hot_windows, g->tc_window_units, g->tc_hot_min};
        const int kClasses = cc.count();
        uint32_t *cnt = nullptr, *cur = nullptr;
        if (int rc = dmalloc(&cnt, n_recv * kClasses + 1, nullptr)) return rc;
        DevGuard g_cnt{cnt};
        if (int rc = dmalloc(&cur, n_recv * kClasses + 1, nullptr)) return rc;
        DevGuard g_cur{cur};
        GMSX_HIP(hipMemsetAsync(cnt, 0, size_t(n_recv * kClasses + 1) * sizeof(uint32_t), s));
        GMSX_HIP(hipMemsetAsync(cur, 0, size_t(n_recv * kClasses + 1) * sizeof(uint32_t), s));
        if (int rc = dmalloc(&g->tunits, n_heavy + 1, g)) return rc;
        GMSX_HIP(hipMemsetAsync(g->tunits, 0, size_t(n_heavy + 1) * sizeof(int32_t), s));
        unsigned long long *totals = nullptr;
        if (int rc = dmalloc(&totals, 4, nullptr)) return rc;
        DevGuard g_tot{totals};
        GMSX_HIP(hipMemsetAsync(totals, 0, 4 * sizeof(unsigned long long), s));
        int64_t *hcnt = nullptr, *tcnt = nullptr, *hbeg = nullptr, *tbeg = nullptr;
        if (int rc = dmalloc(&hcnt, n_recv + 1, nullptr)) return rc;
        DevGuard g_hc{hcnt};
        if (int rc = dmalloc(&tcnt, n_recv + 1, nullptr)) return rc;
        DevGuard g_tc{tcnt};
        if (int rc = dmalloc(&hbeg, n_recv + 1, nullptr)) return rc;
        DevGuard g_hb{hbeg};
        if (int rc = dmalloc(&tbeg, n_recv + 1, nullptr)) return rc;
        DevGuard g_tb{tbeg};
        const int grid = grid_for_waves(n_heavy);
        if (g->spool_units + kPoolSlack >= (int64_t(1) << 32) || g->tpool_units + kPoolSlack >= (int64_t(1) << 32)) return GMSX_ERR_DEVICE_MEM;
        {
            uint32_t hub_max = kTaskHubUnitsMax, tail_max = kTaskTailUnitsMax;
            if (const char *e = opt("TC_TEST_MAX_UNITS")) hub_max = tail_max = uint32_t(std::max(1, std::atoi(e)));
            if (n > 0) hipLaunchKernelGGL(k_task_limits, dim3(vb), dim3(256), 0, s, n, g->srow, g->srow2, g->trow, hub_max, tail_max, totals + 3);
        }
        if (n > 0)
            hipLaunchKernelGGL(k_inline_entries<false>, dim3(vb), dim3(256), 0, s, n, g->dplus, opos, lidx, n_heavy, g->inline_limit, ihoff, itoff, inline_h_base,
                               inline_t_base, cnt, cur, hbeg, tbeg, TaskList{}, TaskList{}, totals, cc);
        if (n_heavy > 0)
            hipLaunchKernelGGL(k_task_lists<false>, dim3(grid), dim3(256), 0, s, n_heavy, g->order, g->hoff, g->hadj, g->toff, g->tadj, g->dplus, g->srow, g->srow2, g->ksplit, g->trow,
                               two_sided, opos, cnt, cur, hbeg, tbeg, TaskList{}, TaskList{}, g->tunits,
                               totals + 2, g->spool, g->tpool, g->inline_limit, g->inline_first, g->tc_core, g->shard_nparts, g->shard_part, cc);
        pt.mark("task lists count");
        hipLaunchKernelGGL(k_list_sizes, dim3(unsigned(n_recv / 256 + 1)), dim3(256), 0, s, n_recv, cnt, hcnt, tcnt, cc);
        if (int rc = exclusive_scan_i64(hcnt, hbeg, n_recv + 1, s)) return rc;
        if (int rc = exclusive_scan_i64(tcnt, tbeg, n_recv + 1, s)) return rc;
        unsigned long long tot[4] = {0, 0, 0, 0};
        GMSX_HIP(hipMemcpy(&g->htask_entries, hbeg + n_recv, sizeof(int64_t), hipMemcpyDeviceToHost));
        GMSX_HIP(hipMemcpy(&g->ttask_entries, tbeg + n_recv, sizeof(int64_t), hipMemcpyDeviceToHost));
        GMSX_HIP(hipMemcpy(tot, totals, sizeof(tot), hipMemcpyDeviceToHost));
        if (tot[3]) return GMSX_ERR_UNSUPPORTED;
        g->inline_hentries = int64_t(tot[0]);
        g->inline_tentries = int64_t(tot[1]);
        g->task_reverse = int64_t(tot[2]);
        if (g->htask_entries >= (int64_t(1) << 40) || g->ttask_entries >= (int64_t(1) << 40)) return GMSX_ERR_DEVICE_MEM;
        if (int rc = dmalloc(&g->htask.lo, g->htask_entries + 2, g)) return rc;
        if (int rc = dmalloc(&g->htask.hi, g->htask_entries + 2, g)) return rc;
        if (int rc = dmalloc(&g->ttask.lo, g->ttask_entries + 2, g)) return rc;
        if (int rc = dmalloc(&g->ttask.hi, g->ttask_entries + 2, g)) return rc;
        if (n > 0)
            hipLaunchKernelGGL(k_inline_entries<true>, dim3(vb), dim3(256), 0, s, n, g->dplus, opos, lidx, n_heavy, g->inline_limit, ihoff, itoff, inline_h_base,
                               inline_t_base, cnt, cur, hbeg, tbeg, g->htask, g->ttask, totals, cc);
        if (n_heavy > 0)
            hipLaunchKernelGGL(k_task_lists<true>, dim3(grid), dim3(256), 0, s, n_heavy, g->order, g->hoff, g->hadj, g->toff, g->tadj, g->dplus, g->srow, g->srow2, g->ksplit, g->trow,
                               two_sided, opos, cnt, cur, hbeg, tbeg, g->htask, g->ttask, g->tunits, totals + 2, g->spool, g->tpool, g->inline_limit, g->inline_first, g->tc_core, g->shard_nparts, g->shard_part, cc);
        pt.mark("task lists fill");
        const int hub_phases = cc.hub_phases();
        const int64_t slots = int64_t(hub_phases) * n_recv;
        int64_t *icnt = nullptr, *ioff = nullptr;
        if (int rc = dmalloc(&icnt, slots + 1, nullptr)) return rc;
        DevGuard g_ic{icnt};
        if (int rc = dmalloc(&ioff, slots + 1, nullptr)) return rc;
        DevGuard g_io{ioff};
        const unsigned rb = unsigned(n_recv / 256 + 1);
        hipLaunchKernelGGL(k_item_counts, dim3(rb), dim3(256), 0, s, n_recv, hbeg, cnt, cc, hub_phases, icnt);
        if (int rc = exclusive_scan_i64(icnt, ioff, slots + 1, s)) return rc;
        GMSX_HIP(hipMemcpy(&g->hitems, ioff + slots, sizeof(int64_t), hipMemcpyDeviceToHost));
        if (int rc = dmalloc(&g->hitem, g->hitems + 1, g)) return rc;
        if (n_recv > 0) hipLaunchKernelGGL(k_item_fill, dim3(rb), dim3(256), 0, s, n_recv, recv_v, opos, hbeg, ioff, g->htask, g->hoff, 0, cnt, cc, hub_phases, g->hitem);
        hipLaunchKernelGGL(k_item_counts, dim3(rb), dim3(256), 0, s, n_recv, tbeg, cnt, cc, 1, icnt);
        if (int rc = exclusive_scan_i64(icnt, ioff, n_recv + 1, s)) return rc;
        GMSX_HIP(hipMemcpy(&g->titems, ioff + n_recv, sizeof(int64_t), hipMemcpyDeviceToHost));
        if (int rc = dmalloc(&g->titem, g->titems + 1, g)) return rc;
        if (n_recv > 0) hipLaunchKernelGGL(k_item_fill, dim3(rb), dim3(256), 0, s, n_recv, recv_v, opos, tbeg, ioff, g->ttask, g->toff, 1, cnt, cc, 1, g->titem);
        if (g->hitems >= (int64_t(1) << 31) || g->titems >= (int64_t(1) << 31)) return GMSX_ERR_DEVICE_MEM;
        GMSX_HIP(hipStreamSynchronize(s));
    }
    pt.mark("work items");
    GMSX_HIP(hipStreamSynchronize(s));
    GMSX_HIP(hipGetLastError());
    {
        auto drop = [&](auto *&p, size_t bytes) {
            if (!p) return;
            (void)hipFree(p);
            p = nullptr;
            g->device_bytes -= int64_t(bytes);
        };
        const size_t nn = size_t(n > 0 ? n : 1);
        drop(g->tsplit, nn * sizeof(int32_t));
        drop(g->srow2, nn * sizeof(unsigned long long));
        const char *keep = opt("TC_KEEP_ROWS");
        if (!(keep && std::atoi(keep) != 0)) {
            drop(g->srow, nn * sizeof(unsigned long long));
            drop(g->trow, nn * sizeof(unsigned long long));
        }
        drop(g->ksplit, size_t(n + 1) * sizeof(int32_t));
    }
    return GMSX_OK;
}

static int build_tc_once(gmsx_graph *g) {
    g->tc_base_bytes = g->device_bytes;
    g->tc_building = true;
    const int rc = build_tc_sets(g);
    g->tc_building = false;
    g->tc_bytes = g->device_bytes - g->tc_base_bytes;
    if (rc) {
        free_tc(g);
        return rc;
    }
    g->tc_ready = true;
    return GMSX_OK;
}

int ensure_tc(const gmsx_graph *cg) {
    gmsx_graph *g = const_cast<gmsx_graph *>(cg);
    if (g->tc_ready) return GMSX_OK;
    if (const char *e = opt("TC_MEM_LIMIT_MB")) {
        const long long v = std::atoll(e);
        g->tc_limit_bytes = v > 0 ? int64_t(v) << 20 : 0;
    }
    int rc = build_tc_once(g);
    if (rc == GMSX_ERR_DEVICE_MEM && g->shard_nparts == 1) {
        (void)hipGetLastError();
        for (int k = 2; k <= 4096 && rc == GMSX_ERR_DEVICE_MEM; k *= 2) {
            g->shard_part = 0;
            g->shard_nparts = k;
            rc = build_tc_once(g);
            if (rc == GMSX_OK) g->tc_passes = k;
        }
        if (rc) {
            g->shard_part = 0;
            g->shard_nparts = 1;
        }
    }
    return rc;
}

__global__ void k_shard_flags(int64_t n_items, const gmsx_tc_item *__restrict__ items, int nparts, int part, int64_t *__restrict__ flags) {
    const int64_t i = int64_t(blockIdx.x) * blockDim.x + threadIdx.x;
    if (i <= n_items) flags[i] = (i < n_items && shard_of(items[i].pos, nparts) == part) ? 1 : 0;
}
__global__ void k_shard_scatter(int64_t n_items, const int64_t *__restrict__ flags, const int64_t *__restrict__ slot, const gmsx_tc_item *__restrict__ items,
                                gmsx_tc_item *__restrict__ out) {
    const int64_t i = int64_t(blockIdx.x) * blockDim.x + threadIdx.x;
    if (i < n_items && flags[i]) out[slot[i]] = items[i];
}
int tc_shard_items(const gmsx_graph *g, int part, int nparts) {
    if (g->shard_idx_part == part && g->shard_idx_nparts == nparts) return GMSX_OK;
    hipStream_t s = ctx().stream;
    (void)hipFree(g->shard_hitem);
    (void)hipFree(g->shard_titem);
    g->shard_hitem = g->shard_titem = nullptr;
    g->shard_idx_part = g->shard_idx_nparts = -1;
    auto one = [&](const gmsx_tc_item *items, int64_t n_items, gmsx_tc_item **idx, int64_t *count) -> int {
        *count = 0;
        if (n_items == 0) return GMSX_OK;
        int64_t *flags = nullptr, *slot = nullptr;
        if (int rc = dmalloc(&flags, n_items + 1, nullptr)) return rc;
        DevGuard g_f{flags};
        if (int rc = dmalloc(&slot, n_items + 1, nullptr)) return rc;
        DevGuard g_s{slot};
        hipLaunchKernelGGL(k_shard_flags, dim3(unsigned(n_items / 256 + 1)), dim3(256), 0, s, n_items, items, nparts, part, flags);
        if (int rc = exclusive_scan_i64(flags, slot, n_items + 1, s)) return rc;
        GMSX_HIP(hipMemcpy(count, slot + n_items, sizeof(int64_t), hipMemcpyDeviceToHost));
        if (int rc = dmalloc(idx, *count + 1, nullptr)) return rc;
        hipLaunchKernelGGL(k_shard_scatter, dim3(unsigned(n_items / 256 + 1)), dim3(256), 0, s, n_items, flags, slot, items, *idx);
        GMSX_HIP(hipStreamSynchronize(s));
        return GMSX_OK;
    };
    if (int rc = one(g->hitem, g->hitems, &g->shard_hitem, &g->shard_hitems)) return rc;
    if (int rc = one(g->titem, g->titems, &g->shard_titem, &g->shard_titems)) return rc;
    g->shard_idx_part = part;
    g->shard_idx_nparts = nparts;
    return GMSX_OK;
}

int ensure_tc_shard(const gmsx_graph *cg, int part, int nparts) {
    gmsx_graph *g = const_cast<gmsx_graph *>(cg);
    if (g->tc_ready && g->shard_part == part && g->shard_nparts == nparts) return GMSX_OK;
    free_tc(g);
    g->shard_part = part;
    g->shard_nparts = nparts;
    return build_tc_once(g);
}

int count_dplus_ge(const gmsx_graph *g, int32_t threshold, int64_t *out) {
    if (g->n == 0) {
        *out = 0;
        return GMSX_OK;
    }
    for (int i = 0; i < g->ge_used; ++i)
        if (g->ge_thr[i] == threshold) {
            *out = g->ge_cnt[i];
            return GMSX_OK;
        }
    hipStream_t s = ctx().stream;
    hipLaunchKernelGGL(k_count_ge, dim3(1), dim3(1), 0, s, g->n, g->order, g->dplus, threshold, reinterpret_cast<int64_t *>(g->scratch + 8));
    GMSX_HIP(hipMemcpyAsync(out, g->scratch + 8, sizeof(int64_t), hipMemcpyDeviceToHost, s));
    GMSX_HIP(hipStreamSynchronize(s));
    if (g->ge_used < 40) {
        g->ge_thr[g->ge_used] = threshold;
        g->ge_cnt[g->ge_used] = *out;
        ++g->ge_used;
    }
    return GMSX_OK;
}

// ... 167 lines not shown
```

### gms_amd/csrc/hip/device_graph.hpp

```cpp
#pragma once
#include <hip/hip_runtime.h>

#include <cstdint>

#include "gmsx.h"
#include "gmsx_internal.hpp"

#if !defined(GMSX_DEV_HOOKS) &&                                                                                                               \
    (defined(GMSX_KC_NO_PROBE) || defined(GMSX_KC_NO_HITS) || defined(GMSX_KC_NO_TAIL) || defined(GMSX_KC_NO_INNER) || defined(GMSX_KC_CELLS_ONLY) ||   \
     defined(GMSX_KC_NO_ROWS) || defined(GMSX_KC_BUILD_ONLY) || defined(GMSX_KC_NO_SLAB_CALL) || defined(GMSX_KC_NO_PAIRS) || defined(GMSX_KC_SLAB_ROW_SCAN) || \
     defined(GMSX_BK_AB) || defined(GMSX_BK_NO_HIT_ATOMICS) || defined(GMSX_BK_STATS) || defined(GMSX_TC_NO_PROBE) || defined(GMSX_TC_STAGING_ONLY))
#error "A/B switches need -DGMSX_DEV_HOOKS (tools/ab_lib.sh sets it); the default build of libgmsx.so carries none of them"
#endif

struct __attribute__((aligned(64))) gmsx_tc_item {
    uint64_t bc;
    uint64_t cont;
    int32_t pivot;
    int32_t pos;
    uint32_t kind;
    uint16_t fbeg[4];
    uint32_t reserved[7];
};
static_assert(sizeof(gmsx_tc_item) == 64, "work item record = one 64-byte line");
constexpr uint32_t kTaskHubUnitsMax = (1u << 14) - 1, kTaskTailUnitsMax = (1u << 15) - 1;
struct TaskList {
    uint32_t *lo = nullptr;
    uint16_t *hi = nullptr;
    bool tail = false;
    __host__ __device__ TaskList at(int64_t first) const { return TaskList{lo + first, hi + first, tail}; }
    __device__ __forceinline__ unsigned long long get(int64_t i) const {
        const uint32_t l = lo[i], h = hi[i];
        const unsigned long long first = ((unsigned long long)h << 16) | (l >> 16);
        const uint32_t form = tail ? ((l >> 15) & 1u) << 1 : (l >> 14) & 3u, units = tail ? l & kTaskTailUnitsMax : l & kTaskHubUnitsMax;
        return (first << 24) | ((unsigned long long)form << 22) | units;
    }
    __device__ __forceinline__ void put(int64_t i, unsigned long long d) const {
        const uint32_t first = uint32_t(d >> 24), form = (uint32_t(d) >> 22) & 3u, units = uint32_t(d) & 0x3fffffu;
        lo[i] = (first << 16) | (tail ? (form >> 1) << 15 : form << 14) | units;
        hi[i] = uint16_t(first >> 16);
    }
};
struct gmsx_graph {
    int64_t n = 0, nnz = 0, m = 0;
    int64_t *off = nullptr;
    int32_t *adj = nullptr;
    int32_t *newid = nullptr;
    int32_t *oldid = nullptr;
    int64_t *hoff = nullptr;
    uint16_t *hadj = nullptr;
    int64_t *toff = nullptr;
    int32_t *tadj = nullptr;
    int64_t *bmoff = nullptr;
    uint32_t *bmpool = nullptr;
    int32_t dense_limit = 0;
    int32_t bitset_limit = 0;
    unsigned long long *srow = nullptr;
    unsigned long long *srow2 = nullptr;
    int32_t *ksplit = nullptr;
    uint32_t *spool = nullptr;
    int64_t spool_units = 0;
    TaskList htask{nullptr, nullptr, false};
    TaskList ttask{nullptr, nullptr, true};
    int64_t htask_entries = 0, ttask_entries = 0;
    struct gmsx_tc_item *hitem = nullptr, *titem = nullptr;
    int64_t hitems = 0, titems = 0;
    int64_t inline_hentries = 0, inline_tentries = 0;
    mutable struct gmsx_tc_item *shard_hitem = nullptr, *shard_titem = nullptr;
    mutable int64_t shard_hitems = 0, shard_titems = 0;
    mutable int shard_idx_part = -1, shard_idx_nparts = -1;
    int32_t *tunits = nullptr;
    int64_t task_reverse = 0;
    uint4 *ledge = nullptr;
    int64_t n_ledge = 0, ledge_total = 0;
    uint32_t *core_bits = nullptr;
    int32_t tc_core = 0;
    mutable int core_bytes_k = -1, core_bytes_part = -1, core_bytes_nparts = -1;
    mutable uint64_t core_bytes = 0;
    int tc_hot_windows = 0;
    uint32_t tc_window_units = 1;
    int tc_hot_min = 0;
    int inline_first = 64;
    int32_t inline_limit = 0;
    int64_t inline_units = 0;
    unsigned long long *trow = nullptr;
    uint32_t *tpool = nullptr;
    int64_t tpool_units = 0;
    int32_t *tsplit = nullptr;
    int64_t dense_rows = 0, bmpool_words = 0;
    bool rows_sorted = false;
    int32_t *dplus = nullptr;
    int32_t *order = nullptr;
    int64_t hub_entries = 0, tail_entries = 0;
    int32_t max_dplus = 0;
    int32_t max_deg = 0;
    mutable bool kc_rev_tried = false;
    mutable uint32_t *kc_rel = nullptr;
    mutable int64_t *kc_aoff = nullptr;
    mutable uint32_t *kc_arena = nullptr;
    mutable ulonglong2 *kc_rec = nullptr;
    mutable uint4 *kc_item = nullptr;
    mutable uint32_t *kc_relt = nullptr;
    mutable ulonglong2 *kc_rect = nullptr;
    mutable uint4 *kc_itemt = nullptr;
    mutable int64_t kc_recst = 0, kc_itemst = 0;
    mutable int64_t kc_recs = 0, kc_items = 0, kc_arena_words = 0, kc_rev_bytes = 0;
    mutable double kc_rev_build_ms = 0.0;
    unsigned long long *scratch = nullptr;
    unsigned long long *acc = nullptr;
    mutable int32_t ge_thr[40] = {0};
    mutable int64_t ge_cnt[40] = {0};
    mutable int ge_used = 0;
    mutable int stats_part = -1, stats_nparts = -1;
    mutable uint64_t stats_units = 0, stats_probes = 0, stats_bytes = 0;
    int shard_part = 0, shard_nparts = 1;
    int tc_passes = 1;
    int64_t tc_limit_bytes = 0, tc_base_bytes = 0;
    bool tc_building = false;
    bool tc_ready = false;
    int64_t tc_bytes = 0;
    int hub_limit = 0;
    uint32_t upload_flags = 0;
    uint64_t alg_elements = 0;
    int64_t device_bytes = 0;
};

namespace gmsx {

static constexpr int kHub = 65535;
static constexpr int kBitmapWords = 2048;
static constexpr int kAccWords = 64 * 16 + 16;
static constexpr int kFormList = 0, kFormBitset = 1, kFormDelta = 2, kFormGap12 = 3;
static constexpr int kPoolSlack = 64;
static constexpr int kTaskChunk = 512;
static constexpr int kLenClasses = 12;
static constexpr int kHubClasses = 4 * kLenClasses, kTailClasses = 2 * kLenClasses;
static constexpr int kMaxHotWindows = 8;
struct TcClasses {
    int hot_windows;
    uint32_t window_units;
    int hot_min;
    __host__ __device__ int hub_phases() const { return hot_windows + 1; }
    __host__ __device__ int tail_base() const { return hub_phases() * kHubClasses; }
    __host__ __device__ int count() const { return tail_base() + kTailClasses; }
    __host__ __device__ int phase(unsigned long long d) const {
        if (hot_windows <= 0) return 0;
        const unsigned long long w = (d >> 24) / window_units;
        return w < (unsigned long long)hot_windows ? int(w) : hot_windows;
    }
};
__host__ __device__ inline int length_class(uint32_t u) {
    return u <= 16 ? (u <= 4 ? 0 : u <= 8 ? 1 : u <= 12 ? 2 : 3) : u <= 64 ? (u <= 24 ? 4 : u <= 32 ? 5 : u <= 48 ? 6 : 7) : (u <= 96 ? 8 : u <= 128 ? 9 : u <= 192 ? 10 : 11);
}
__host__ __device__ inline int hub_class(const TcClasses &cc, unsigned long long d) {
    return cc.phase(d) * kHubClasses + int((uint32_t(d) >> 22) & 3u) * kLenClasses + length_class(uint32_t(d) & 0x3fffffu);
}
__host__ __device__ inline int tail_class(const TcClasses &cc, unsigned long long d) {
    return cc.tail_base() + (((uint32_t(d) >> 22) & 3u) == 2u ? kLenClasses : 0) + length_class(uint32_t(d) & 0x3fffffu);
}
__host__ __device__ inline void hub_phase_range(const TcClasses &cc, const uint32_t *c, int64_t len, int ph, int64_t *b, int64_t *e) {
    int64_t start = 0;
    for (int q = 0;; ++q) {
        const int64_t end = q < cc.hot_windows ? int64_t(c[(q + 1) * kHubClasses]) : len;
        const bool own = q == cc.hot_windows || end - start >= cc.hot_min;
        if (q == ph) {
            *b = start;
            *e = own ? end : start;
            return;
        }
        if (own) start = end;
    }
}
__host__ __device__ inline int shard_of(int64_t pos, int nparts) {
    const int j = int(pos % nparts);
    return ((pos / nparts) & 1) ? nparts - 1 - j : j;
}
static constexpr int kHeavy = 64;
static constexpr int kDeltaIds = 14;

__host__ __device__ inline int64_t bitset_words(int32_t v) { return ((int64_t(v) + 31) / 32 + 3) & ~int64_t(3); }

struct Ctx {
    int device = -1;
    hipStream_t stream = nullptr;
    hipStream_t own_stream = nullptr;
    hipEvent_t ev[4] = {nullptr, nullptr, nullptr, nullptr};
    hipStream_t side[2] = {nullptr, nullptr};
    hipEvent_t ev_fork = nullptr, ev_join[2] = {nullptr, nullptr};
    int compute_units = 0;
};
Ctx &ctx();
int ensure_init();
int kclique_vertex_counts(const gmsx_graph *g, unsigned long long *d_counts, gmsx_stats *st);
int count_dplus_ge(const gmsx_graph *g, int32_t threshold, int64_t *out);
int exclusive_scan_i64(const int64_t *in, int64_t *out, int64_t count, hipStream_t s);
int ensure_tc(const gmsx_graph *g);
int ensure_tc_shard(const gmsx_graph *g, int part, int nparts);
int tc_shard_items(const gmsx_graph *g, int part, int nparts);
int tc_vertex_counts_device(const gmsx_graph *g, unsigned long long *d_counts, gmsx_stats *st);
int tc_full_partial(const gmsx_graph *g, int part, int nparts, uint64_t *partial, gmsx_stats *st);

__device__ __forceinline__ int uni32(int x) { return __builtin_amdgcn_readfirstlane(x); }
__device__ __forceinline__ uint32_t uni32(uint32_t x) { return uint32_t(__builtin_amdgcn_readfirstlane(int(x))); }
__device__ __forceinline__ int64_t uni64(int64_t x) {
    const uint32_t lo = uint32_t(__builtin_amdgcn_readfirstlane(int(uint32_t(uint64_t(x)))));
    const uint32_t hi = uint32_t(__builtin_amdgcn_readfirstlane(int(uint32_t(uint64_t(x) >> 32))));
    return int64_t((uint64_t(hi) << 32) | lo);
}
__device__ __forceinline__ unsigned long long uni64(unsigned long long x) { return (unsigned long long)uni64(int64_t(x)); }

#define GMSX_HIP(call)                                                    \
    do {                                                                  \
        hipError_t e_ = (call);                                           \
        if (e_ != hipSuccess) {                                           \
            (void)hipGetLastError();                                      \
            return e_ == hipErrorOutOfMemory ? GMSX_ERR_DEVICE_MEM : GMSX_ERR_KERNEL; \
        }                                                                 \
    } while (0)

}
```

### gms_amd/csrc/hip/tc.hip

```cpp
#include "device_graph.hpp"
#include "kc4_mfma.hpp"
#include "../host/tc_core_plan.hpp"

#include <algorithm>
#include <type_traits>
#include <rocprim/device/device_radix_sort.hpp>
#include <rocprim/device/device_reduce.hpp>
#include <rocprim/device/device_reduce_by_key.hpp>
#include <cstdio>
#include <cstdlib>
#include <cstring>

namespace gmsx {

static constexpr int kAccSlots = 64;
static constexpr int kAccStride = 16;

struct __attribute__((packed, aligned(4))) u4u { uint32_t x, y, z, w; };

__device__ __forceinline__ int64_t readlane64(int64_t x, int l) {
    const uint32_t lo = __builtin_amdgcn_readlane(uint32_t(uint64_t(x)), l);
    const uint32_t hi = __builtin_amdgcn_readlane(uint32_t(uint64_t(x) >> 32), l);
    return int64_t((uint64_t(hi) << 32) | lo);
}
// ... 484 lines not shown
                if (neA > nl) {
                    st.start(sd, oddA, pool, nl, neA, tid);
                    c += st.run([=](uint4 p, int, int) { return tail_delta_unit_hits(flt, tbl, mask, shift, p); });
                }
#endif
            }
            if (!staged) {
                __syncthreads();
                if (vB) stage(L.rec[rb], buf ^ 1, lane, wave);
                if (fetch) L.chunk[1] = pend < unsigned(n_items) ? int(pend) : -1;
            }
        }
        total += c;
        ra = rb;
        vA = vB;
        vB = vC;
        buf ^= 1;
    }
}

#ifndef GMSX_TC_HUB_MIN_WAVES
#define GMSX_TC_HUB_MIN_WAVES 8
#endif
#ifndef GMSX_TC_TAIL_MIN_WAVES
#define GMSX_TC_TAIL_MIN_WAVES 8
#endif
template <bool TAIL>
__global__ __launch_bounds__(256) __attribute__((amdgpu_waves_per_eu(TAIL ? GMSX_TC_TAIL_MIN_WAVES : GMSX_TC_HUB_MIN_WAVES, 8))) void k_tc_items(
    const uint16_t *__restrict__ hadj, const int32_t *__restrict__ tadj, const uint32_t *__restrict__ pool, const TaskList task,
    const gmsx_tc_item *__restrict__ items, int n_items, unsigned int *__restrict__ qhead, unsigned long long *__restrict__ acc) {
    __shared__ __attribute__((aligned(16))) ItemLds L;
    const int tid = threadIdx.x;
    unsigned long long total = 0;
    item_loop<TAIL>(L, hadj, tadj, pool, task, items, n_items, qhead, total);
    block_add(total, L.red, tid & 63, tid >> 6, tid, acc);
}

template <int K>
__device__ __forceinline__ uint32_t ror_in_row(uint32_t x) {
    if constexpr (K == 0) return x;
    else return uint32_t(__builtin_amdgcn_mov_dpp(int(x), 0x120 + K, 0xf, 0xf, false));
}
__device__ __forceinline__ bool row_has(uint32_t a, uint32_t x) {
    bool m = false;
#define GMSX_ROT(K) m |= a == ror_in_row<K>(x);
    GMSX_ROT(0) GMSX_ROT(1) GMSX_ROT(2) GMSX_ROT(3) GMSX_ROT(4) GMSX_ROT(5) GMSX_ROT(6) GMSX_ROT(7)
    GMSX_ROT(8) GMSX_ROT(9) GMSX_ROT(10) GMSX_ROT(11) GMSX_ROT(12) GMSX_ROT(13) GMSX_ROT(14) GMSX_ROT(15)
#undef GMSX_ROT
    return m;
}
struct LightRows {
    uint32_t ah[4], at[4], bh[4], bt[4];
};
struct LightRec {
    uint4 r0, r1;
};
__global__ __launch_bounds__(256) void k_tc_light(const uint16_t *__restrict__ hadj, const int32_t *__restrict__ tadj, const uint4 *__restrict__ ledge, int nparts,
                                                  int part, int64_t count, unsigned long long *__restrict__ acc) {
    __shared__ unsigned long long red[4];
    const int tid = threadIdx.x, lane = tid & 63, wave = tid >> 6, sub = lane & 15;
    const int64_t ngroups = int64_t(gridDim.x) * 16, g0 = int64_t(blockIdx.x) * 16 + (tid >> 4);
    const int64_t trips = (count + ngroups - 1) / ngroups;
    auto load_rec = [&](int64_t t) -> LightRec {
        const int64_t k = g0 + t * ngroups;
        const int64_t kk = k < count ? k : 0;
        const int64_t e = nparts <= 1 ? kk : kk * nparts + ((kk & 1) ? nparts - 1 - part : part);
        LightRec r;
        r.r0 = ledge[2 * e];
        r.r1 = ledge[2 * e + 1];
        if (k >= count) {
            r.r0.y &= 0xffu;
            r.r0.w &= 0xffu;
            r.r1.y &= 0xffu;
            r.r1.w &= 0xffu;
        }
        return r;
    };
    auto wave_max = [](int x) {
        return max(max(__builtin_amdgcn_readlane(x, 0), __builtin_amdgcn_readlane(x, 16)), max(__builtin_amdgcn_readlane(x, 32), __builtin_amdgcn_readlane(x, 48)));
    };
    auto load_rows = [&](const LightRec &r) -> LightRows {
        const int64_t hu = int64_t((uint64_t(r.r0.y & 0xffu) << 32) | r.r0.x), tu = int64_t((uint64_t(r.r0.w & 0xffu) << 32) | r.r0.z);
        const int64_t hv = int64_t((uint64_t(r.r1.y & 0xffu) << 32) | r.r1.x), tv = int64_t((uint64_t(r.r1.w & 0xffu) << 32) | r.r1.z);
        const int hlu = int(r.r0.y >> 8), tlu = int(r.r0.w >> 8), hlv = int(r.r1.y >> 8), tlv = int(r.r1.w >> 8);
        const int more = wave_max((max(max(hlu, hlv), max(tlu, tlv)) + 15) >> 4);
        LightRows w;
        w.ah[0] = hadj[hlu ? hu + min(sub, hlu - 1) : 0];
        w.bh[0] = hadj[hlv ? hv + min(sub, hlv - 1) : 0];
        w.at[0] = uint32_t(tadj[tlu ? tu + min(sub, tlu - 1) : 0]);
        w.bt[0] = uint32_t(tadj[tlv ? tv + min(sub, tlv - 1) : 0]);
#pragma unroll
        for (int k = 1; k < 4; ++k) {
            w.ah[k] = w.bh[k] = w.at[k] = w.bt[k] = 0;
            if (k < more) {
                const int i = sub + 16 * k;
                w.ah[k] = hadj[hlu ? hu + min(i, hlu - 1) : 0];
                w.bh[k] = hadj[hlv ? hv + min(i, hlv - 1) : 0];
                w.at[k] = uint32_t(tadj[tlu ? tu + min(i, tlu - 1) : 0]);
                w.bt[k] = uint32_t(tadj[tlv ? tv + min(i, tlv - 1) : 0]);
            }
        }
        return w;
    };
    unsigned long long total = 0;
    if (trips > 0) {
        LightRec rec = load_rec(0);
        LightRows rows = load_rows(rec);
        LightRec rec_n = load_rec(1);
        for (int64_t t = 0; t < trips; ++t) {
            const LightRows rows_n = load_rows(rec_n);
            const LightRec rec_nn = load_rec(t + 2);
            const int hlu = int(rec.r0.y >> 8), tlu = int(rec.r0.w >> 8), hlv = int(rec.r1.y >> 8), tlv = int(rec.r1.w >> 8);
            const int nah = wave_max((hlu + 15) >> 4), nbh = wave_max((hlv + 15) >> 4), nat = wave_max((tlu + 15) >> 4), nbt = wave_max((tlv + 15) >> 4);
            uint32_t c = 0;
#pragma unroll
            for (int ka = 0; ka < 4; ++ka) {
                if (ka >= nah) break;
                const int ia = sub + 16 * ka;
                const uint32_t a = (ia < hlu && rows.ah[ka] != 0xFFFFu) ? rows.ah[ka] : 0xFFFFFFFFu;
                bool m = false;
#pragma unroll
                for (int kb = 0; kb < 4; ++kb) {
                    if (kb >= nbh) break;
                    const int ib = sub + 16 * kb;
                    const uint32_t x = (ib < hlv && rows.bh[kb] != 0xFFFFu) ? rows.bh[kb] : 0xFFFFFFFEu;
                    m |= row_has(a, x);
                }
                c += m ? 1u : 0u;
            }
#pragma unroll
            for (int ka = 0; ka < 4; ++ka) {
                if (ka >= nat) break;
                const int ia = sub + 16 * ka;
                const uint32_t a = ia < tlu ? rows.at[ka] : 0xFFFFFFFFu;
                bool m = false;
#pragma unroll
                for (int kb = 0; kb < 4; ++kb) {
                    if (kb >= nbt) break;
                    const int ib = sub + 16 * kb;
                    const uint32_t x = ib < tlv ? rows.bt[kb] : 0xFFFFFFFEu;
                    m |= row_has(a, x);
                }
                c += m ? 1u : 0u;
            }
            total += c;
            rec = rec_n;
            rows = rows_n;
            rec_n = rec_nn;
        }
    }
    block_add(total, red, lane, wave, tid, acc);
}

__global__ __launch_bounds__(1024) void k_tc_core(const uint32_t *__restrict__ bits, int WS, int K, int nb, int nblk, int part, int nparts,
                                                  unsigned long long *__restrict__ acc) {
    __shared__ unsigned long long red[16];
    auto lane_id = [] { return int(__builtin_amdgcn_mbcnt_hi(~0u, __builtin_amdgcn_mbcnt_lo(~0u, 0u))); };
    const int wave = uni32(int(threadIdx.x) >> 6);
    const int x = blockIdx.x & 7, y = blockIdx.x >> 3, Y = int(gridDim.x) >> 3;
    const int Q = 16 * Y, q = y * 16 + wave;
    const int ns = (nblk - part + nparts - 1) / nparts;
    uint32_t cnt = 0;
    for (int j = 0;; ++j) {
        const int sidx = (8 * j + ((j & 1) ? 7 - x : x)) * Q + q;
        if (sidx >= ns) break;
        const int t = sidx * nparts + part;
        int c = int((__builtin_sqrtf(8.0f * float(t) + 1.0f) - 1.0f) * 0.5f);
        while (c * (c + 1) / 2 > t) --c;
        while ((c + 1) * (c + 2) / 2 <= t) ++c;
        const int bj = nb - 1 - c, bi = bj + (t - c * (c + 1) / 2);
        int lane = lane_id();
        asm volatile("" : "+v"(lane));
        cnt += Kc4mBlock<2>::run(bits, WS, K, bi, bj, lane);
    }
    const int lane = lane_id();
    unsigned long long total = cnt;
    for (int sft = 32; sft > 0; sft >>= 1) total += __shfl_down(total, sft);
    if (lane == 0) red[wave] = total;
    __syncthreads();
    if (wave == 0 && lane == 0) {
        unsigned long long t = 0;
        for (int w = 0; w < 16; ++w) t += red[w];
        if (t) atomicAdd(&acc[(blockIdx.x & (kAccSlots - 1)) * kAccStride], t);
    }
}

__global__ __launch_bounds__(256) void k_tc_stats(const int64_t *__restrict__ hoff, const uint16_t *__restrict__ hadj,
                                                  const int64_t *__restrict__ toff, const int32_t *__restrict__ tadj,
                                                  const int32_t *__restrict__ dplus, const int32_t *__restrict__ order,
                                                  const int32_t *__restrict__ tunits, int32_t inline_limit, int inline_first, int32_t core, int64_t end, int nparts, int part,
                                                  unsigned long long *__restrict__ out) {
    const int lane = threadIdx.x & 63;
    const int64_t wave0 = (int64_t(blockIdx.x) * blockDim.x + threadIdx.x) >> 6;
    const int64_t nwaves = (int64_t(gridDim.x) * blockDim.x) >> 6;
    unsigned long long units = 0, probes = 0, bytes = 0;
    for (int64_t pos = wave0; pos < end; pos += nwaves) {
        if (nparts > 1 && shard_of(pos, nparts) != part) continue;
        const int32_t u = order[pos];
        const int du = dplus[u];
        if (du >= kHeavy) {
            if (lane == 0) units += (unsigned long long)tunits[pos];
            if (u < core) {
                if (lane == 0) units += (unsigned long long)du;
                continue;
            }
            const int hl = min(int(hoff[u + 1] - hoff[u]), inline_first), tl = min(int(toff[u + 1] - toff[u]), inline_first - hl);
            int32_t v = -1;
            if (lane < hl) {
                const uint32_t x = hadj[hoff[u] + lane];
                if (x != 0xFFFFu) v = int32_t(x);
            } else if (lane - hl < tl) v = tadj[toff[u] + lane - hl];
            if (v >= 0 && lane > 0 && (v < inline_limit || dplus[v] >= kHeavy)) ++units;
            continue;
        }
        const int hl = int(hoff[u + 1] - hoff[u]);
        if (lane == 0) units += (unsigned long long)du;
        if (du < 2 || u < core) continue;
        for (int64_t j = toff[u] + lane; j < toff[u + 1]; j += 64) {
            const int32_t v = tadj[j];
            if (v < inline_limit || dplus[v] >= kHeavy) continue;
            const unsigned long long hv = (unsigned long long)(hoff[v + 1] - hoff[v]), tv = (unsigned long long)(toff[v + 1] - toff[v]);
            bytes += 32ull + 2ull * hl + 4ull * (unsigned long long)(j - toff[u]) + 2ull * hv + 4ull * tv;
            probes += hv + tv;
        }
    }
    for (int s = 32; s > 0; s >>= 1) {
        units += __shfl_down(units, s);
        probes += __shfl_down(probes, s);
        bytes += __shfl_down(bytes, s);
    }
    if (lane == 0) {
        if (units) atomicAdd(&out[0], units);
        if (probes) atomicAdd(&out[1], probes);
        if (bytes) atomicAdd(&out[2], bytes);
    }
}
__global__ __launch_bounds__(256) void k_tc_item_stats(const int64_t *__restrict__ coff, int bytes_per_id, int tail, const TaskList task,
                                                       const gmsx_tc_item *__restrict__ items, int64_t n_items, int nparts, int part,
                                                       unsigned long long *__restrict__ out) {
    const int lane = threadIdx.x & 63;
    const int64_t wave0 = (int64_t(blockIdx.x) * blockDim.x + threadIdx.x) >> 6;
    const int64_t nwaves = (int64_t(gridDim.x) * blockDim.x) >> 6;
    unsigned long long probes = 0, bytes = 0;
    auto slots = [tail](unsigned long long d) -> unsigned long long {
        const unsigned long long n = d & 0x3fffffull, f = (d >> 22) & 3ull;
        return n * (tail ? (f == kFormDelta ? 6ull : 4ull) : (f == kFormList ? 8ull : f == kFormDelta ? 14ull : f == kFormGap12 ? 10ull : 4ull));
    };
    for (int64_t q = wave0; q < n_items; q += nwaves) {
        const gmsx_tc_item &it = items[q];
        if (nparts > 1 && shard_of(it.pos, nparts) != part) continue;
        const int ne = int(it.bc >> 40);
        const int64_t b = int64_t(it.bc & 0xffffffffffull);
        if (lane == 0) bytes += (unsigned long long)bytes_per_id * (unsigned long long)(coff[it.pivot + 1] - coff[it.pivot]);
        for (int i = lane; i < ne; i += 64) {
            const unsigned long long d = task.get(b + i);
            bytes += 6ull + 16ull * (d & 0x3fffffull);
            probes += slots(d);
        }
    }
    for (int s = 32; s > 0; s >>= 1) {
        probes += __shfl_down(probes, s);
        bytes += __shfl_down(bytes, s);
    }
    if (lane == 0) {
        if (probes) atomicAdd(&out[1], probes);
        if (bytes) atomicAdd(&out[2], bytes);
    }
}

__global__ __launch_bounds__(256) void k_tc_breakdown(const int64_t *__restrict__ hoff, const int64_t *__restrict__ toff, const int32_t *__restrict__ tadj,
                                                      const int32_t *__restrict__ dplus, const int32_t *__restrict__ order,
                                                      const TaskList htask, const gmsx_tc_item *__restrict__ hitem, int64_t hitems,
                                                      const TaskList ttask, const gmsx_tc_item *__restrict__ titem, int64_t titems,
                                                      int32_t inline_limit, int32_t core, int64_t first_light, int64_t end_light,
                                                      unsigned long long *__restrict__ out) {
    const int lane = threadIdx.x & 63;
    const int64_t wave0 = (int64_t(blockIdx.x) * blockDim.x + threadIdx.x) >> 6;
    const int64_t nwaves = (int64_t(gridDim.x) * blockDim.x) >> 6;
    unsigned long long c[15] = {0, 0, 0, 0, 0, 0, 0, 0, 0, 0, 0, 0, 0, 0, 0};
    for (int64_t q = wave0; q < hitems + titems; q += nwaves) {
        const bool tail = q >= hitems;
        const gmsx_tc_item &it = tail ? titem[q - hitems] : hitem[q];
        const TaskList task = tail ? ttask : htask;
        const int ne = int(it.bc >> 40);
        const int64_t b0 = int64_t(it.bc & 0xffffffffffull);
        if (lane == 0) {
            c[6] += tail ? 4ull * (unsigned long long)(toff[it.pivot + 1] - toff[it.pivot]) : 2ull * (unsigned long long)(hoff[it.pivot + 1] - hoff[it.pivot]);
            c[11] += (unsigned long long)ne;
            c[13] += 1;
        }
        for (int i = lane; i < ne; i += 64) {
            const unsigned long long d = task.get(b0 + i);
            const unsigned long long db = 16ull * (d & 0x3fffffull);
            const int fd = int((d >> 22) & 3);
            if (tail) c[fd == kFormDelta ? 4 : 3] += db;
            else c[fd == kFormList ? 0 : fd == kFormBitset ? 1 : 2] += db;
            c[5] += 6;
        }
    }
    for (int64_t pos = first_light + wave0; pos < end_light; pos += nwaves) {
        const int32_t u = order[pos];
        if (u < core) continue;
        const int64_t tb0 = toff[u], te = toff[u + 1];
        const unsigned long long hl = (unsigned long long)(hoff[u + 1] - hoff[u]);
        for (int64_t j = tb0 + lane; j < te; j += 64) {
            const int32_t v = tadj[j];
            if (v < inline_limit || dplus[v] >= kHeavy) continue;
            c[8] += 2ull * (unsigned long long)(hoff[v + 1] - hoff[v]);
            c[9] += 4ull * (unsigned long long)(toff[v + 1] - toff[v]);
            c[10] += 32ull + 2ull * hl + 4ull * (unsigned long long)(j - tb0);
            c[14] += 1;
        }
    }
    for (int k = 0; k < 15; ++k) {
        unsigned long long x = c[k];
        for (int s = 32; s > 0; s >>= 1) x += __shfl_down(x, s);
        if (lane == 0 && x) atomicAdd(&out[k], x);
    }
}

__device__ __forceinline__ int hist_bin(unsigned long long units) {
    if (units <= 16) return int(units) - 1;
    int b = 16;
    for (unsigned long long lim = 32; units > lim && b < 23; lim <<= 1) ++b;
    return b;
}
__global__ __launch_bounds__(256) void k_tc_comember_keys(const TaskList htask, const gmsx_tc_item *__restrict__ hitem, int64_t hitems, int batch,
                                                         unsigned long long *__restrict__ keys, uint32_t *__restrict__ vals, unsigned long long *__restrict__ sums) {
    unsigned long long ents = 0, units = 0;
    for (int64_t i = blockIdx.x; i < hitems; i += gridDim.x) {
        const gmsx_tc_item it = hitem[i];
        const unsigned long long first = it.bc & 0xffffffffffull;
        const int n = int(it.bc >> 40);
        const unsigned long long b = (unsigned long long)(it.pos / batch) << 40;
        for (int e = threadIdx.x; e < n; e += 256) {
            const unsigned long long d = htask.get(int64_t(first + e));
            keys[first + e] = b | (d >> 24);
            vals[first + e] = uint32_t(d & 0x3fffffull);
            ++ents;
            units += d & 0x3fffffull;
        }
    }
    for (int sft = 32; sft > 0; sft >>= 1) {
        ents += __shfl_xor(ents, sft);
        units += __shfl_xor(units, sft);
    }
    if ((threadIdx.x & 63) == 0) {
        atomicAdd(&sums[0], ents);
        atomicAdd(&sums[1], units);
    }
}
__global__ __launch_bounds__(256) void k_tc_sum_u32(const uint32_t *__restrict__ v, unsigned long long n, unsigned long long *__restrict__ out) {
    unsigned long long t = 0;
    for (unsigned long long i = (unsigned long long)blockIdx.x * 256 + threadIdx.x; i < n; i += (unsigned long long)gridDim.x * 256) t += v[i];
    for (int sft = 32; sft > 0; sft >>= 1) t += __shfl_xor(t, sft);
    if ((threadIdx.x & 63) == 0) atomicAdd(out, t);
}
__global__ __launch_bounds__(256) void k_tc_row_hist(const int64_t *__restrict__ hoff, const uint16_t *__restrict__ hadj,
                                                     const int64_t *__restrict__ toff, const int32_t *__restrict__ tadj,
                                                     const int32_t *__restrict__ dplus, const int32_t *__restrict__ order,
                                                     const unsigned long long *__restrict__ srow, const unsigned long long *__restrict__ trow,
                                                     const TaskList htask, const gmsx_tc_item *__restrict__ hitem, int64_t hitems,
                                                     const TaskList ttask, const gmsx_tc_item *__restrict__ titem, int64_t titems,
                                                     int64_t end, unsigned long long *__restrict__ out) {
    __shared__ unsigned long long h[256];
    for (int i = threadIdx.x; i < 256; i += 256) h[i] = 0;
    __syncthreads();
    const int lane = threadIdx.x & 63;
    const int64_t wave0 = (int64_t(blockIdx.x) * blockDim.x + threadIdx.x) >> 6;
    const int64_t nwaves = (int64_t(gridDim.x) * blockDim.x) >> 6;
    auto add = [&](int cls, unsigned long long units) {
        if (units == 0) return;
        const int b = (cls * 24 + hist_bin(units)) * 2;
        atomicAdd(&h[b], 1ull);
        atomicAdd(&h[b + 1], units);
    };
    for (int64_t q = wave0; q < hitems + titems; q += nwaves) {
        const bool tail = q >= hitems;
        const gmsx_tc_item &it = tail ? titem[q - hitems] : hitem[q];
        const TaskList task = tail ? ttask : htask;
        const int ne = int(it.bc >> 40);
        const int64_t b0 = int64_t(it.bc & 0xffffffffffull);
        if (lane == 0) {
            atomicAdd(&h[240], (unsigned long long)ne);
            atomicAdd(&h[242], 1ull);
            atomicAdd(&h[243], tail ? 4ull * (unsigned long long)(toff[it.pivot + 1] - toff[it.pivot]) : 2ull * (unsigned long long)(hoff[it.pivot + 1] - hoff[it.pivot]));
        }
        for (int i = lane; i < ne; i += 64) {
            const unsigned long long d = task.get(b0 + i);
            if (tail) add(((d >> 22) & 3) == kFormDelta ? 4 : 3, d & 0x3fffffull);
            else add(min(int((d >> 22) & 3), 2), d & 0x3fffffull);
        }
    }
    for (int64_t pos = wave0; pos < end; pos += nwaves) {
        if (!srow || !trow) break;
        const int32_t u = order[pos];
        const int du = dplus[u];
        if (du < 2) continue;
        const int64_t hb = hoff[u], tb = toff[u];
        const int hl = int(hoff[u + 1] - hb), tl = int(toff[u + 1] - tb);
        const unsigned long long su = (srow[u] & 0x3fffffull) + (trow[u] & 0x3fffffull);
        unsigned long long cur = 0, best = 0, cut = 0;
        for (int i = lane; i < hl + tl; i += 64) {
            int32_t v;
            if (i < hl) {
                const uint32_t x = hadj[hb + i];
                if (x == 0xFFFFu) continue;
                v = int32_t(x);
            } else v = tadj[tb + i - hl];
            const unsigned long long sv = (srow[v] & 0x3fffffull) + (trow[v] & 0x3fffffull);
            cur += sv;
            best += min(su, sv);
            cut += min(sv, dplus[v] >= kHeavy ? (su * (unsigned long long)i + du - 1) / (unsigned long long)du : ~0ull);
        }
        atomicAdd(&h[du >= kHeavy ? 248 : 250], cur);
        atomicAdd(&h[du >= kHeavy ? 249 : 251], best);
        if (du >= kHeavy) atomicAdd(&h[252], cut);
    }
    __syncthreads();
    for (int i = threadIdx.x; i < 256; i += 256)
        if (h[i]) atomicAdd(&out[i], h[i]);
}

static int tc_one(const gmsx_graph *g, int part, int nparts, int cpart, int cnparts, uint64_t *partial, gmsx_stats *st);
static uint64_t core_bytes_of(const gmsx_graph *g, int part, int nparts) {
    if (g->tc_core <= 0 || nparts < 1) return 0;
    if (!(g->core_bytes_k == g->tc_core && g->core_bytes_part == part && g->core_bytes_nparts == nparts)) {
        g->core_bytes = tc_core_bytes(g->tc_core, part, nparts);
        g->core_bytes_k = g->tc_core;
        g->core_bytes_part = part;
        g->core_bytes_nparts = nparts;
    }
    return g->core_bytes;
}

static int tc_oriented(const gmsx_graph *g, int part, int nparts, uint64_t *partial, gmsx_stats *st) {
    if (int rc = ensure_tc(g)) return rc;
    if (g->tc_passes == 1) return tc_one(g, part, nparts, part, nparts, partial, st);
    if (nparts > 1) {
        auto restore = [&](int rc) {
            gmsx_graph *m = const_cast<gmsx_graph *>(g);
            if (m->tc_ready && m->shard_part == 0 && m->shard_nparts == m->tc_passes) return rc;
            (void)ensure_tc_shard(g, 0, g->tc_passes);
            return rc;
        };
        int J = nparts >= g->tc_passes ? 1 : (g->tc_passes + nparts - 1) / nparts;
        if (J > 1 && (J & 1)) ++J;
        for (;; J *= 2) {
            uint64_t total = 0;
            gmsx_stats sum{};
            int rc = GMSX_OK;
            for (int a = 0; a < J && rc == GMSX_OK; ++a) {
                const int sub = a * nparts + ((a & 1) ? nparts - 1 - part : part);
                rc = ensure_tc_shard(g, sub, nparts * J);
                if (rc) break;
                uint64_t pp = 0;
                gmsx_stats sp{};
                rc = tc_one(g, sub, nparts * J, part, a == 0 ? nparts : 0, &pp, st ? &sp : nullptr);
                total += pp;
                sum.kernel_ms += sp.kernel_ms;
                sum.setup_ms += sp.setup_ms;
                sum.units += sp.units;
                sum.probes += sp.probes;
                sum.stream_bytes += sp.stream_bytes;
                sum.launches += sp.launches;
            }
            if (rc == GMSX_ERR_DEVICE_MEM && nparts * J <= (1 << 20)) continue;
            if (rc) return restore(rc);
            *partial = total;
            if (st) *st = sum;
            return GMSX_OK;
        }
    }
    uint64_t total = 0;
    gmsx_stats sum{};
    for (int p = 0; p < g->tc_passes; ++p) {
        if (int rc = ensure_tc_shard(g, p, g->tc_passes)) return rc;
        uint64_t pp = 0;
        gmsx_stats sp{};
        if (int rc = tc_one(g, p, g->tc_passes, 0, p == 0 ? 1 : 0, &pp, st ? &sp : nullptr)) return rc;
        total += pp;
        sum.kernel_ms += sp.kernel_ms;
        sum.setup_ms += sp.setup_ms;
        sum.units += sp.units;
        sum.probes += sp.probes;
        sum.stream_bytes += sp.stream_bytes;
        sum.launches += sp.launches;
    }
    *partial = total;
    if (st) {
        sum.alg_elements = g->alg_elements;
        *st = sum;
    }
    return GMSX_OK;
}

static int tc_one(const gmsx_graph *g, int part, int nparts, int cpart, int cnparts, uint64_t *partial, gmsx_stats *st) {
    const bool use_idx = nparts > 1 && g->shard_nparts == 1;
    if (use_idx)
        if (int rc = tc_shard_items(g, part, nparts)) return rc;
    const gmsx_tc_item *hitem = use_idx ? g->shard_hitem : g->hitem, *titem = use_idx ? g->shard_titem : g->titem;
    int64_t n_hitems = use_idx ? g->shard_hitems : g->hitems, n_titems = use_idx ? g->shard_titems : g->titems;
#ifdef GMSX_DEV_HOOKS
    const char *only = std::getenv("GMSX_TC_ONLY");
    if (only) {
        if (std::strcmp(only, "hub") != 0) n_hitems = 0;
        if (std::strcmp(only, "tail") != 0) n_titems = 0;
    }
#else
    const char *only = nullptr;
#endif
    Ctx &c = ctx();
    hipStream_t s = c.stream;
    unsigned long long *acc = g->acc;
    static_assert(kAccSlots * kAccStride + 16 <= kAccWords, "gmsx_graph::acc too small");
    unsigned int *qhead = reinterpret_cast<unsigned int *>(acc + kAccSlots * kAccStride + 4);
    static_assert((kQueueStride + 1) * sizeof(unsigned int) <= 12 * sizeof(unsigned long long), "queue heads past gmsx_graph::acc");
    GMSX_HIP(hipEventRecord(c.ev[0], s));
    GMSX_HIP(hipMemsetAsync(acc, 0, sizeof(unsigned long long) * kAccWords, s));
    GMSX_HIP(hipEventRecord(c.ev[1], s));

    int launches = 0;
    const int cus = c.compute_units > 0 ? c.compute_units : 256;
    const int64_t cap_blocks = int64_t(cus) * 16;
    const bool run_light = !only || std::strcmp(only, "light") == 0;
    const bool strided = nparts > 1 && g->shard_nparts == 1;
    const int64_t cnt_light = [&]() -> int64_t {
        if (!run_light) return 0;
        if (!strided) return g->n_ledge;
        const int64_t full = g->n_ledge / nparts, rem = g->n_ledge % nparts;
        return full + (((full & 1) ? nparts - 1 - part : part) < rem ? 1 : 0);
    }();
    const int overlap = [] { const char *e = opt("TC_OVERLAP"); return e ? std::atoi(e) : 0; }();
    const int persist = [] { const char *e = opt("TC_PERSIST"); return e ? std::atoi(e) : 1; }();
    const bool sides = overlap && c.side[0] && c.side[1];
    struct Join {
        Ctx &c;
        hipStream_t s;
        bool armed[2] = {false, false};
        ~Join() {
            for (int i = 0; i < 2; ++i)
                if (armed[i] && hipEventRecord(c.ev_join[i], c.side[i]) == hipSuccess) (void)hipStreamWaitEvent(s, c.ev_join[i], 0);
        }
    } join{c, s};
    const bool side_light = sides && cnt_light > 0 && n_hitems + n_titems > 0;
    const bool side_tail = sides && !persist && n_hitems > 0 && n_titems > 0;
    if (side_light || side_tail) GMSX_HIP(hipEventRecord(c.ev_fork, s));
    if (side_tail) {
        GMSX_HIP(hipStreamWaitEvent(c.side[0], c.ev_fork, 0));
        join.armed[0] = true;
    }
    if (side_light) {
        GMSX_HIP(hipStreamWaitEvent(c.side[1], c.ev_fork, 0));
        join.armed[1] = true;
    }
    const bool run_core = g->tc_core > 0 && cnparts > 0 && !only;
    if (run_core) {
        const int K = g->tc_core, nb = (K + 63) / 64, nblk = int(tc_core_blocks(K));
        const int64_t ns = (int64_t(nblk) - cpart + cnparts - 1) / cnparts;
        if (ns > 0) {
            const int64_t wgs = std::max<int64_t>(8, std::min<int64_t>(cus / 8 * 8, ((ns + 15) / 16 + 7) / 8 * 8));
            hipLaunchKernelGGL(k_tc_core, dim3(unsigned(wgs)), dim3(1024), 0, s, g->core_bits, kc4m_stride(K), K, nb, nblk, cpart, cnparts, acc);
            ++launches;
        }
    }
    if (persist) {
        const int wgs_env = [] { const char *e = opt("TC_ITEM_WGS"); return e ? std::atoi(e) : 0; }();
        auto grid = [&](int64_t n, int wgs) {
            return unsigned(std::max<int64_t>(1, std::min<int64_t>((n + kGrab - 1) / kGrab, int64_t(cus) * (wgs_env > 0 ? wgs_env : wgs))));
        };
        if (n_hitems > 0) {
            hipLaunchKernelGGL(k_tc_items<false>, dim3(grid(n_hitems, GMSX_TC_HUB_MIN_WAVES)), dim3(256), 0, s, g->hadj, g->tadj, g->spool, g->htask, hitem, int(n_hitems), qhead, acc);
            ++launches;
        }
        if (n_titems > 0) {
            hipLaunchKernelGGL(k_tc_items<true>, dim3(grid(n_titems, GMSX_TC_TAIL_MIN_WAVES)), dim3(256), 0, s, g->hadj, g->tadj, g->tpool, g->ttask, titem, int(n_titems),
                               qhead + kQueueStride, acc);
            ++launches;
        }
    } else {
        if (n_hitems > 0) {
            hipLaunchKernelGGL(k_tc_block, dim3(unsigned(n_hitems)), dim3(256), 0, s, g->hoff, g->hadj, g->spool, g->htask, hitem, acc);
            ++launches;
        }
        if (n_titems > 0) {
            hipLaunchKernelGGL(k_tc_tail, dim3(unsigned(n_titems)), dim3(256), 0, side_tail ? c.side[0] : s, g->toff, g->tadj, g->tpool, g->ttask, titem, acc);
            ++launches;
        }
    }
    if (cnt_light > 0) {
        const int64_t blocks = std::min<int64_t>((cnt_light + 15) / 16, int64_t(cus) * 8);
        hipLaunchKernelGGL(k_tc_light, dim3(unsigned(blocks)), dim3(256), 0, side_light ? c.side[1] : s, g->hadj, g->tadj, g->ledge, strided ? nparts : 1,
                           strided ? part : 0, cnt_light, acc);
        ++launches;
    }
    for (int i = 0; i < 2; ++i)
        if (join.armed[i]) {
            join.armed[i] = false;
            GMSX_HIP(hipEventRecord(c.ev_join[i], c.side[i]));
            GMSX_HIP(hipStreamWaitEvent(s, c.ev_join[i], 0));
        }
    GMSX_HIP(hipEventRecord(c.ev[2], s));
    GMSX_HIP(hipGetLastError());

    const bool need_stats = st && !(g->stats_part == part && g->stats_nparts == nparts);
    if (need_stats) {
        if (g->n > 0) {
            const int64_t blocks = std::min<int64_t>((g->n + 3) / 4, cap_blocks);
            hipLaunchKernelGGL(k_tc_stats, dim3(unsigned(blocks)), dim3(256), 0, s, g->hoff, g->hadj, g->toff, g->tadj, g->dplus, g->order,
                               g->tunits, g->inline_limit, g->inline_first, g->tc_core, g->n, nparts, part, acc + kAccSlots * kAccStride);
        }
        if (g->hitems > 0)
            hipLaunchKernelGGL(k_tc_item_stats, dim3(unsigned(std::min<int64_t>((g->hitems + 3) / 4, cap_blocks))), dim3(256), 0, s, g->hoff, 2, 0, g->htask, g->hitem,
                               g->hitems, nparts, part, acc + kAccSlots * kAccStride);
        if (g->titems > 0)
            hipLaunchKernelGGL(k_tc_item_stats, dim3(unsigned(std::min<int64_t>((g->titems + 3) / 4, cap_blocks))), dim3(256), 0, s, g->toff, 4, 1, g->ttask, g->titem,
                               g->titems, nparts, part, acc + kAccSlots * kAccStride);
    }
    unsigned long long host[kAccSlots * kAccStride + 3];
    GMSX_HIP(hipMemcpyAsync(host, acc, sizeof(host), hipMemcpyDeviceToHost, s));
    GMSX_HIP(hipStreamSynchronize(s));
    unsigned long long total = 0;
    for (int i = 0; i < kAccSlots; ++i) total += host[i * kAccStride];
    *partial = total;
    if (st) {
        float ms_setup = 0.f, ms_kernel = 0.f;
        GMSX_HIP(hipEventElapsedTime(&ms_setup, c.ev[0], c.ev[1]));
        GMSX_HIP(hipEventElapsedTime(&ms_kernel, c.ev[1], c.ev[2]));
        st->kernel_ms = ms_kernel;
        st->setup_ms = ms_setup;
        if (need_stats) {
            g->stats_part = part;
            g->stats_nparts = nparts;
            g->stats_units = host[kAccSlots * kAccStride];
            g->stats_probes = host[kAccSlots * kAccStride + 1];
            g->stats_bytes = host[kAccSlots * kAccStride + 2];
        }
        st->units = g->stats_units;
        st->probes = g->stats_probes;
        st->alg_elements = nparts == 1 ? g->alg_elements : 0;
        st->launches = launches;
        st->reserved = 0;
        st->stream_bytes = g->stats_bytes + (run_core ? core_bytes_of(g, cpart, cnparts) : 0);
    }
    return GMSX_OK;
}

}

using namespace gmsx;

extern "C" {

int gmsx_tc_divisor(int algo) { return algo == GMSX_TC_FULL ? 3 : 1; }

int gmsx_tc_stream_breakdown(const gmsx_graph *g, uint64_t *out21) {
    return gmsx::guard([&]() -> int {
        if (!g || !out21) return GMSX_ERR_INVALID;
        if (int rc = ensure_init()) return rc;
        if (int rc = ensure_tc(g)) return rc;
        hipStream_t s = ctx().stream;
        std::memset(out21, 0, 21 * sizeof(uint64_t));
        if (g->n == 0) return GMSX_OK;
        int64_t n_block = 0, n_work = 0;
        if (int rc = count_dplus_ge(g, kHeavy, &n_block)) return rc;
        if (int rc = count_dplus_ge(g, 2, &n_work)) return rc;
        unsigned long long *acc = nullptr;
        GMSX_HIP(hipMalloc(reinterpret_cast<void **>(&acc), 21 * 8));
        struct Guard { void *p; ~Guard() { (void)hipFree(p); } } g1{acc};
        GMSX_HIP(hipMemsetAsync(acc, 0, 21 * 8, s));
        const int cus = ctx().compute_units > 0 ? ctx().compute_units : 256;
        hipLaunchKernelGGL(k_tc_breakdown, dim3(unsigned(cus * 16)), dim3(256), 0, s, g->hoff, g->toff, g->tadj, g->dplus, g->order, g->htask,
                           g->hitem, g->hitems, g->ttask, g->titem, g->titems, g->inline_limit, g->tc_core, n_block, n_work, acc);
        GMSX_HIP(hipMemcpyAsync(out21, acc, 21 * 8, hipMemcpyDeviceToHost, s));
        GMSX_HIP(hipStreamSynchronize(s));
        GMSX_HIP(hipGetLastError());
        out21[7] = uint64_t(g->inline_units) * 16ull;
        out21[12] = uint64_t(g->inline_hentries + g->inline_tentries);
        out21[15] = core_bytes_of(g, 0, 1);
        out21[16] = uint64_t(g->tc_core);
        return GMSX_OK;
    });
}

int gmsx_tc_row_histogram(const gmsx_graph *g, uint64_t *out256) {
    return gmsx::guard([&]() -> int {
        uint64_t *out248 = out256;
        if (!g || !out248) return GMSX_ERR_INVALID;
        if (int rc = ensure_init()) return rc;
        if (int rc = ensure_tc(g)) return rc;
        hipStream_t s = ctx().stream;
        std::memset(out248, 0, 256 * sizeof(uint64_t));
        if (g->n == 0) return GMSX_OK;
        unsigned long long *acc = nullptr;
        GMSX_HIP(hipMalloc(reinterpret_cast<void **>(&acc), 256 * 8));
        struct Guard { void *p; ~Guard() { (void)hipFree(p); } } g1{acc};
        GMSX_HIP(hipMemsetAsync(acc, 0, 256 * 8, s));
        const int cus = ctx().compute_units > 0 ? ctx().compute_units : 256;
        hipLaunchKernelGGL(k_tc_row_hist, dim3(unsigned(cus * 8)), dim3(256), 0, s, g->hoff, g->hadj, g->toff, g->tadj, g->dplus, g->order, g->srow, g->trow,
                           g->htask, g->hitem, g->hitems, g->ttask, g->titem, g->titems, g->n, acc);
        GMSX_HIP(hipGetLastError());
        GMSX_HIP(hipMemcpyAsync(out248, acc, 256 * 8, hipMemcpyDeviceToHost, s));
        GMSX_HIP(hipStreamSynchronize(s));
        GMSX_HIP(hipGetLastError());
        out248[241] = uint64_t(g->inline_hentries + g->inline_tentries);
        return GMSX_OK;
    });
}

int gmsx_tc_comembership(const gmsx_graph *g, int batch, uint64_t *out8) {
    return gmsx::guard([&]() -> int {
        if (!g || !out8 || batch < 1) return GMSX_ERR_INVALID;
        if (int rc = ensure_init()) return rc;
        if (int rc = ensure_tc(g)) return rc;
        hipStream_t s = ctx().stream;
        std::memset(out8, 0, 8 * sizeof(uint64_t));
        const int64_t ne = g->htask_entries;
        if (g->n == 0 || ne == 0 || g->hitems == 0) return GMSX_OK;
        struct Guard { void *p = nullptr; ~Guard() { (void)hipFree(p); } } gk0, gk1, gv0, gv1, gu, ga, gc, gt, gsum;
        unsigned long long *k0 = nullptr, *k1 = nullptr, *uk = nullptr, *cnt = nullptr, *sum = nullptr;
        uint32_t *v0 = nullptr, *v1 = nullptr, *agg = nullptr;
        GMSX_HIP(hipMalloc(reinterpret_cast<void **>(&k0), size_t(ne) * 8)); gk0.p = k0;
        GMSX_HIP(hipMalloc(reinterpret_cast<void **>(&k1), size_t(ne) * 8)); gk1.p = k1;
        GMSX_HIP(hipMalloc(reinterpret_cast<void **>(&v0), size_t(ne) * 4)); gv0.p = v0;
        GMSX_HIP(hipMalloc(reinterpret_cast<void **>(&v1), size_t(ne) * 4)); gv1.p = v1;
        GMSX_HIP(hipMalloc(reinterpret_cast<void **>(&sum), 4 * 8)); gsum.p = sum;
        GMSX_HIP(hipMemsetAsync(k0, 0xff, size_t(ne) * 8, s));
        GMSX_HIP(hipMemsetAsync(v0, 0, size_t(ne) * 4, s));
        GMSX_HIP(hipMemsetAsync(sum, 0, 4 * 8, s));
        hipLaunchKernelGGL(k_tc_comember_keys, dim3(unsigned(std::min<int64_t>(g->hitems, 1 << 20))), dim3(256), 0, s, g->htask, g->hitem, g->hitems, batch, k0, v0, sum);
        size_t tb = 0;
        GMSX_HIP(rocprim::radix_sort_pairs(nullptr, tb, k0, k1, v0, v1, size_t(ne), 0, 64, s));
        void *tmp = nullptr;
        GMSX_HIP(hipMalloc(&tmp, tb ? tb : 8)); gt.p = tmp;
        GMSX_HIP(rocprim::radix_sort_pairs(tmp, tb, k0, k1, v0, v1, size_t(ne), 0, 64, s));
        uk = k0;
        agg = v0;
        GMSX_HIP(hipMalloc(reinterpret_cast<void **>(&cnt), 8)); gc.p = cnt;
        size_t rb = 0;
        GMSX_HIP(rocprim::reduce_by_key(nullptr, rb, k1, v1, size_t(ne), uk, agg, cnt, rocprim::maximum<uint32_t>(), rocprim::equal_to<unsigned long long>(), s));
        void *tmp2 = nullptr;
        Guard g2;
        GMSX_HIP(hipMalloc(&tmp2, rb ? rb : 8)); g2.p = tmp2;
        GMSX_HIP(rocprim::reduce_by_key(tmp2, rb, k1, v1, size_t(ne), uk, agg, cnt, rocprim::maximum<uint32_t>(), rocprim::equal_to<unsigned long long>(), s));
        unsigned long long nuniq = 0;
        GMSX_HIP(hipMemcpyAsync(&nuniq, cnt, 8, hipMemcpyDeviceToHost, s));
        GMSX_HIP(hipStreamSynchronize(s));
        hipLaunchKernelGGL(k_tc_sum_u32, dim3(1024), dim3(256), 0, s, agg, (unsigned long long)nuniq, sum + 2);
        unsigned long long h[4] = {0, 0, 0, 0};
        GMSX_HIP(hipMemcpyAsync(h, sum, sizeof(h), hipMemcpyDeviceToHost, s));
        GMSX_HIP(hipStreamSynchronize(s));
        GMSX_HIP(hipGetLastError());
        out8[0] = uint64_t(h[0]);
        out8[1] = uint64_t(h[1]);
        out8[2] = uint64_t(nuniq);
        out8[3] = uint64_t(h[2]);
        out8[4] = uint64_t(g->hitems);
        return GMSX_OK;
    });
}

int gmsx_tc_partial(const gmsx_graph *g, int algo, int part, int nparts, uint64_t *partial, gmsx_stats *stats) {
    return gmsx::guard([&]() -> int {
        if (!g || !partial || nparts < 1 || part < 0 || part >= nparts) return GMSX_ERR_INVALID;
        if (algo != GMSX_TC_AUTO && algo != GMSX_TC_ORIENTED && algo != GMSX_TC_FULL) return GMSX_ERR_INVALID;
        if (int rc = ensure_init()) return rc;
        if (algo == GMSX_TC_FULL) return tc_full_partial(g, part, nparts, partial, stats);
        if (g->tc_passes == 1 && g->shard_nparts > 1 && (nparts != g->shard_nparts || part != g->shard_part)) return GMSX_ERR_INVALID;
        return tc_oriented(g, part, nparts, partial, stats);
    });
}

int gmsx_tc_total(const gmsx_graph *g, int algo, uint64_t *triangles, gmsx_stats *stats) {
    return gmsx::guard([&]() -> int {
        if (!triangles) return GMSX_ERR_INVALID;
        uint64_t partial = 0;
        if (int rc = gmsx_tc_partial(g, algo, 0, 1, &partial, stats)) return rc;
        const uint64_t div = uint64_t(gmsx_tc_divisor(algo));
        if (partial % div != 0) return GMSX_ERR_KERNEL;
        *triangles = partial / div;
        return GMSX_OK;
    });
}

}
```

### gms_amd/csrc/host/loader.cpp

```cpp
#include "gmsx_internal.hpp"

#include <fcntl.h>
#include <sys/mman.h>
#include <sys/stat.h>
#include <unistd.h>

#include <algorithm>
#ifdef _OPENMP
#include <parallel/algorithm>
#endif
#include <atomic>
#include <cerrno>
#include <cmath>
#include <cstdio>
#include <cstdlib>
#include <cstring>
#include <ctime>
#include <fstream>
#include <limits>
#include <memory>
#include <new>
#include <random>
#include <sstream>
#include <string>
// ... 501 lines not shown
        ++u;
    }
    return finish_el(us, vs, el);
}
static int read_mtx(const std::string &path, EdgeList &el) {
    std::ifstream in(path);
    if (!in.is_open()) return GMSX_ERR_IO;
    std::string start, object, format, field, symmetry, line;
    if (!(in >> start >> object >> format >> field >> symmetry)) return GMSX_ERR_FORMAT;
    if (start != "%%MatrixMarket" || object != "matrix" || format != "coordinate" || field == "complex") return GMSX_ERR_FORMAT;
    const bool weights = field == "real" || field == "double" || field == "integer";
    if (!weights && field != "pattern") return GMSX_ERR_FORMAT;
    if (symmetry != "symmetric" && symmetry != "general" && symmetry != "skew-symmetric") return GMSX_ERR_FORMAT;
    std::getline(in, line);
    long long rows = -1, cols = -1, nz = -1;
    while (std::getline(in, line)) {
        if (!line.empty() && line[0] == '%') continue;
        std::istringstream hs(line);
        if (!(hs >> rows >> cols >> nz)) return GMSX_ERR_FORMAT;
        break;
    }
    if (rows < 0 || rows != cols) return GMSX_ERR_FORMAT;
    std::vector<int32_t> us, vs;
    while (std::getline(in, line)) {
        std::istringstream ls(line);
        long long a, b;
        if (!(ls >> a >> b)) continue;
        if (int rc = push_edge(us, vs, a - 1, b - 1)) return rc;
        if (symmetry == "symmetric")
            if (int rc = push_edge(us, vs, b - 1, a - 1)) return rc;
    }
    return finish_el(us, vs, el);
}

static int validate_csr_arrays(const int64_t *off, const int32_t *ng, int64_t n, int64_t nnz);
static int read_sg(const std::string &path, Csr &g) {
    std::FILE *f = std::fopen(path.c_str(), "rb");
    if (!f) return GMSX_ERR_IO;
    struct Closer { std::FILE *f; ~Closer() { std::fclose(f); } } closer{f};
    unsigned char directed = 0;
    int64_t nnz = 0, n = 0;
    if (std::fread(&directed, 1, 1, f) != 1 || std::fread(&nnz, 8, 1, f) != 1 || std::fread(&n, 8, 1, f) != 1)
        return GMSX_ERR_FORMAT;
    if (n < 0 || nnz < 0 || n > std::numeric_limits<int32_t>::max()) return GMSX_ERR_FORMAT;
    if (int rc = alloc_csr(g, n, nnz)) return rc;
    if (std::fread(g.off.get(), 8, size_t(n + 1), f) != size_t(n + 1)) return GMSX_ERR_FORMAT;
    if (nnz && std::fread(g.neigh.get(), 4, size_t(nnz), f) != size_t(nnz)) return GMSX_ERR_FORMAT;
    if (int rc = validate_csr_arrays(g.off.get(), g.neigh.get(), n, nnz)) return rc;
    g.directed = directed != 0;
    return GMSX_OK;
}


static constexpr char kSgxMagic[8] = {'G', 'M', 'S', 'X', 'C', 'S', 'R', '1'};
static constexpr int64_t kSgxAlign = 64;
static int64_t sgx_neigh_offset(int64_t n) { return (kSgxAlign + (n + 1) * 8 + kSgxAlign - 1) / kSgxAlign * kSgxAlign; }

void ArrayFree::unmap(void *base, size_t bytes) { (void)munmap(base, bytes); }

static int write_sgx(const Csr &g, const char *path) {
    std::FILE *f = std::fopen(path, "wb");
    if (!f) return GMSX_ERR_IO;
    int64_t head[8] = {0, g.directed ? 1 : 0, g.n, g.nnz, 0, 0, 0, 0};
    std::memcpy(head, kSgxMagic, 8);
    const int64_t pad = sgx_neigh_offset(g.n) - (kSgxAlign + (g.n + 1) * 8);
    const char zeros[64] = {0};
    bool ok = std::fwrite(head, 8, 8, f) == 8 && std::fwrite(g.off.get(), 8, size_t(g.n + 1), f) == size_t(g.n + 1) &&
              (pad == 0 || std::fwrite(zeros, 1, size_t(pad), f) == size_t(pad)) &&
              (g.nnz == 0 || std::fwrite(g.neigh.get(), 4, size_t(g.nnz), f) == size_t(g.nnz));
    ok = (std::fclose(f) == 0) && ok;
    return ok ? GMSX_OK : GMSX_ERR_IO;
}

static int validate_csr_arrays(const int64_t *off, const int32_t *ng, int64_t n, int64_t nnz) {
    if (off[0] != 0 || off[n] != nnz) return GMSX_ERR_FORMAT;
    int bad = 0;
#pragma omp parallel for reduction(| : bad) schedule(static)
    for (int64_t u = 0; u < n; ++u) bad |= int(off[u + 1] < off[u]);
    if (bad) return GMSX_ERR_FORMAT;
#pragma omp parallel for reduction(| : bad) schedule(static)
    for (int64_t j = 0; j < nnz; ++j) bad |= int(ng[j] < 0 || int64_t(ng[j]) >= n);
    return bad ? GMSX_ERR_FORMAT : GMSX_OK;
}

static int read_sgx(const std::string &path, Csr &g) {
    const int fd = open(path.c_str(), O_RDONLY | O_CLOEXEC);
    if (fd < 0) return GMSX_ERR_IO;
    struct Closer { int fd; ~Closer() { close(fd); } } closer{fd};
    struct stat st;
    if (fstat(fd, &st) != 0) return GMSX_ERR_IO;
    int64_t head[8];
    if (pread(fd, head, sizeof(head), 0) != ssize_t(sizeof(head)) || std::memcmp(head, kSgxMagic, 8) != 0) return GMSX_ERR_FORMAT;
    const int64_t n = head[2], nnz = head[3];
    if (n < 0 || nnz < 0 || n > std::numeric_limits<int32_t>::max() || (head[1] != 0 && head[1] != 1)) return GMSX_ERR_FORMAT;
    const int64_t noff = sgx_neigh_offset(n);
    if (nnz > (std::numeric_limits<int64_t>::max() - noff) / 4 || int64_t(st.st_size) < noff + nnz * 4) return GMSX_ERR_FORMAT;
    const int64_t page = int64_t(sysconf(_SC_PAGESIZE));
    auto map_part = [&](int64_t at, int64_t bytes, void **base, size_t *len) -> void * {
        const int64_t lo = at / page * page;
        *len = size_t(at - lo + std::max<int64_t>(bytes, 1));
        *base = mmap(nullptr, *len, PROT_READ | PROT_WRITE, MAP_PRIVATE, fd, off_t(lo));
        if (*base == MAP_FAILED) return nullptr;
        (void)madvise(*base, *len, MADV_WILLNEED);
        return static_cast<char *>(*base) + (at - lo);
    };
    void *b0 = nullptr, *b1 = nullptr;
    size_t l0 = 0, l1 = 0;
    void *p_off = map_part(kSgxAlign, (n + 1) * 8, &b0, &l0);
    if (!p_off) return GMSX_ERR_NOMEM;
    g.off = std::unique_ptr<int64_t[], ArrayFree>(static_cast<int64_t *>(p_off), ArrayFree{b0, l0});
    void *p_ng = map_part(noff, nnz * 4, &b1, &l1);
    if (!p_ng) return GMSX_ERR_NOMEM;
    g.neigh = std::unique_ptr<int32_t[], ArrayFree>(static_cast<int32_t *>(p_ng), ArrayFree{b1, l1});
    g.n = n;
    g.nnz = nnz;
    g.directed = head[1] != 0;
    g.mapped = true;
    return validate_csr_arrays(g.off.get(), g.neigh.get(), n, nnz);
}

}

namespace gmsx {
int host_threads() {
#ifdef _OPENMP
    return omp_get_max_threads();
#else
    return 1;
#endif
}
void parallel_memcpy(void *dst, const void *src, size_t bytes) {
#ifdef _OPENMP
#pragma omp parallel
    {
        const size_t nt = size_t(omp_get_num_threads()), t = size_t(omp_get_thread_num());
        const size_t per = ((bytes + nt - 1) / nt + 4095) & ~size_t(4095), lo = std::min(bytes, per * t), hi = std::min(bytes, lo + per);
        if (hi > lo) std::memcpy(static_cast<char *>(dst) + lo, static_cast<const char *>(src) + lo, hi - lo);
    }
#else
    std::memcpy(dst, src, bytes);
#endif
}
namespace {
struct Option {
    const char *name;
    char value[32];
    bool set;
};
Option g_options[] = {
    {"TIMING", "", false}, {"MEM_TRACE", "", false}, {"BK_VERBOSE", "", false},
    {"INLINE_LIMIT", "", false}, {"TC_INLINE_FIRST", "", false}, {"TC_DELTA", "", false}, {"TC_DELTA_PCT", "", false}, {"TC_GAP12", "", false},
    {"TC_HYBRID", "", false}, {"TC_TAIL_DELTA", "", false}, {"TC_TWO_SIDED", "", false}, {"TC_HOT_WINDOWS", "", false}, {"TC_HOT_KB", "", false},
    {"TC_HOT_MIN", "", false}, {"TC_TEST_MAX_UNITS", "", false}, {"TC_KEEP_ROWS", "", false}, {"TC_MEM_LIMIT_MB", "", false}, {"TC_OVERLAP", "", false},
    {"TC_PERSIST", "", false}, {"TC_ITEM_WGS", "", false}, {"TC_CORE", "", false}, {"SORT_CHUNK", "", false}, {"UPLOAD_STAGED", "", false}, {"INIT_LAZY", "", false},
    {"KC_SLAB_MB", "", false}, {"KC_MAXD", "", false}, {"KC_STREAMS", "", false}, {"KC_PIPE_ALL", "", false}, {"KC_STREAM_BUILD", "", false},
    {"KC_REVERSE", "", false}, {"KC_REV_MIN", "", false}, {"KC_REV_FACTOR", "", false}, {"KC_REV_TAIL", "", false}, {"KC_REV_TAIL_MIN", "", false}, {"KC_REV_GW", "", false}, {"KC_TRI", "", false}, {"KC_MFMA", "", false}, {"KC_POOL_MB", "", false},
    {"BK_MAXC", "", false}, {"BK_ARENA_MB", "", false}, {"BK_GROUPS", "", false}, {"BK_SMALL_P", "", false}, {"BK_SMALL_P_GROUPS", "", false},
    {"BK_BUDGET", "", false}, {"BK_BUDGET0", "", false}, {"BK_RESUME_GRAB", "", false}, {"BK_SPLIT_BUILD", "", false}, {"BK_TINY_ROOTS", "", false},
    {"BK_TINY_BESIDE", "", false},
    {"BK_LIST_ARENA_MB", "", false},
    {"KCSTAR_SLAB_MB", "", false},
    {"CORE_WG_FRONTIER", "", false},
    {"COLOR_WG_FRONTIER", "", false},
    {"TRUSS_WG_FRONTIER", "", false},
    {"LP_LDS_MAXN", "", false}, {"LP_SLAB_MB", "", false},
};
Option *find_option(const char *name) {
    if (!name) return nullptr;
    for (Option &o : g_options)
        if (std::strcmp(o.name, name) == 0) return &o;
    return nullptr;
}
}

const char *opt(const char *name) {
    const Option *o = find_option(name);
    return o && o->set ? o->value : nullptr;
}

}

using namespace gmsx;

extern "C" {

int gmsx_csr_generate(int generator, int scale, int degree, int relabel, int threads, gmsx_csr **out) {
    return gmsx::guard([&]() -> int {
        if (!out || scale < 1 || degree < 1 || relabel < 0 || relabel > 2) return GMSX_ERR_INVALID;
        if (scale > 30) return GMSX_ERR_OVERFLOW;
        if (generator != GMSX_GEN_KRONECKER && generator != GMSX_GEN_UNIFORM) return GMSX_ERR_INVALID;
    #ifdef _OPENMP
        struct Threads {
            int saved, set;
            ~Threads() { if (set > 0) omp_set_num_threads(saved); }
        } threads_guard{omp_get_max_threads(), threads};
        if (threads > 0) omp_set_num_threads(threads);
    #else
        (void)threads;
    #endif
        int rc;
        {
            Csr g;
            {
                PhaseTimer pt;
                EdgeList el;
                rc = generator == GMSX_GEN_UNIFORM ? make_uniform(scale, degree, el) : make_rmat(scale, degree, el);
                pt.lap("generate edge list");
                if (!rc) rc = build_from_el(el, -1, true, g);
            }
            PhaseTimer pf;
            if (!rc) rc = finish(std::move(g), relabel, out);
            pf.lap("relabel decision + relabel");
        }
        return rc;
    });
}

int gmsx_csr_generate_rmat(int scale, int degree, double a, double b, double c, int relabel, int threads, gmsx_csr **out) {
    return gmsx::guard([&]() -> int {
        if (!out || scale < 1 || degree < 1 || relabel < 0 || relabel > 2) return GMSX_ERR_INVALID;
        if (!(a > 0 && b >= 0 && c >= 0 && a + b + c < 1.0)) return GMSX_ERR_INVALID;
        if (scale > 30) return GMSX_ERR_OVERFLOW;
    #ifdef _OPENMP
        struct Threads {
            int saved, set;
            ~Threads() { if (set > 0) omp_set_num_threads(saved); }
        } threads_guard{omp_get_max_threads(), threads};
        if (threads > 0) omp_set_num_threads(threads);
    #else
        (void)threads;
    #endif
        int rc;
        {
            Csr g;
            {
                EdgeList el;
                rc = make_rmat(scale, degree, el, float(a), float(b), float(c));
                if (!rc) rc = build_from_el(el, -1, true, g);
            }
            if (!rc) rc = finish(std::move(g), relabel, out);
        }
        return rc;
    });
}

int gmsx_csr_from_edges(int64_t num_nodes, int64_t num_edges, const int32_t *src, const int32_t *dst,
                        int symmetrize, int relabel, gmsx_csr **out) {
    return gmsx::guard([&]() -> int {
        if (!out || num_edges < 0 || (num_edges && (!src || !dst)) || relabel < 0 || relabel > 2) return GMSX_ERR_INVALID;
        EdgeList el;
        if (int rc = el.alloc(num_edges)) return rc;
        if (num_edges) {
            std::memcpy(el.u.get(), src, size_t(num_edges) * 4);
            std::memcpy(el.v.get(), dst, size_t(num_edges) * 4);
        }
        Csr g;
        if (int rc = build_from_el(el, num_nodes, symmetrize != 0, g)) return rc;
        return finish(std::move(g), relabel, out);
    });
}

int gmsx_csr_load(const char *path, int symmetrize, int relabel, gmsx_csr **out) {
    return gmsx::guard([&]() -> int {
        if (!path || !out || relabel < 0 || relabel > 2) return GMSX_ERR_INVALID;
        const std::string p(path), suf = suffix_of(p);
        Csr g;
        if (suf == ".sg") {
            if (int rc = read_sg(p, g)) return rc;
        } else if (suf == ".sgx") {
            if (int rc = read_sgx(p, g)) return rc;
        } else if (suf == ".el" || suf == ".wel" || suf == ".gr" || suf == ".graph" || suf == ".mtx") {
            EdgeList el;
            const int rc = suf == ".el" ? read_el(p, el) : suf == ".wel" ? read_wel(p, el) : suf == ".gr" ? read_gr(p, el)
                         : suf == ".graph" ? read_metis(p, el) : read_mtx(p, el);
            if (rc) return rc;
            if (int rc2 = build_from_el(el, -1, symmetrize != 0, g)) return rc2;
        } else {
            return GMSX_ERR_FORMAT;
        }
        return finish(std::move(g), relabel, out);
    });
}

int gmsx_csr_save_sg(const gmsx_csr *h, const char *path) {
    return gmsx::guard([&]() -> int {
        if (!h || !path) return GMSX_ERR_INVALID;
        std::FILE *f = std::fopen(path, "wb");
        if (!f) return GMSX_ERR_IO;
        const Csr &g = h->g;
        const unsigned char directed = g.directed ? 1 : 0;
        bool ok = std::fwrite(&directed, 1, 1, f) == 1 && std::fwrite(&g.nnz, 8, 1, f) == 1 &&
                  std::fwrite(&g.n, 8, 1, f) == 1 && std::fwrite(g.off.get(), 8, size_t(g.n + 1), f) == size_t(g.n + 1) &&
                  (g.nnz == 0 || std::fwrite(g.neigh.get(), 4, size_t(g.nnz), f) == size_t(g.nnz));
        ok = (std::fclose(f) == 0) && ok;
        return ok ? GMSX_OK : GMSX_ERR_IO;
    });
}

int gmsx_csr_save_sgx(const gmsx_csr *h, const char *path) {
    return gmsx::guard([&]() -> int {
        if (!h || !path) return GMSX_ERR_INVALID;
        return write_sgx(h->g, path);
    });
}
int gmsx_csr_is_mapped(const gmsx_csr *h) { return h ? int(h->g.mapped) : GMSX_ERR_INVALID; }

int gmsx_csr_from_arrays(int64_t n, const int64_t *offsets, const int32_t *neigh, gmsx_csr **out) {
// ... 112 lines not shown
```

### gms_amd/csrc/host/tc_core_plan.hpp

```cpp
#pragma once
#include <algorithm>
#include <cstdint>
#include <vector>

namespace gmsx {

constexpr int kTcCoreBucket = 1024;
constexpr int kTcCoreCap = 32768;
constexpr double kTcCoreStreamBytesPerSec = 7.35e12;
constexpr double kTcCoreBitMacsPerSec = 1.7e15;
constexpr double kTcCoreLaunchSec = 20e-6;
constexpr int kTcCoreDefault = -1;

inline int tc_core_clamp(long long want, long long hub_limit, long long n) {
    return int(std::max<long long>(0, std::min<long long>(std::min<long long>(want, kTcCoreCap), std::min<long long>(hub_limit, n))));
}

inline int choose_tc_core(const std::vector<uint64_t> &bucket_units, int cap, double b_stream = kTcCoreStreamBytesPerSec,
                          double r_core = kTcCoreBitMacsPerSec, double launch_sec = kTcCoreLaunchSec) {
    int best_k = 0;
    double best = 0.0;
    unsigned long long units = 0;
    for (size_t b = 0; b < bucket_units.size(); ++b) {
        const long long k = (long long)(b + 1) * kTcCoreBucket;
        if (k > cap) break;
        units += bucket_units[b];
        const double gain = double(units) * 16.0 / b_stream - (double(k) * double(k) * double(k) / 6.0) / r_core - launch_sec;
        if (gain > best) {
            best = gain;
            best_k = int(k);
        }
    }
    return best_k;
}

inline long long tc_core_blocks(int k) {
    const long long nb = (k + 63) / 64;
    return nb * (nb + 1) / 2;
}
inline unsigned long long tc_core_block_bytes(int bj) { return 1024ull * (unsigned long long)(bj + 1) + 1024ull; }
inline unsigned long long tc_core_bytes(int k, int part, int nparts) {
    const long long nb = (k + 63) / 64;
    unsigned long long bytes = 0;
    long long t = 0;
    for (long long c = 0; c < nb; ++c)
        for (long long r = 0; r <= c; ++r, ++t)
            if (nparts <= 1 || t % nparts == part) bytes += tc_core_block_bytes(int(nb - 1 - c));
    return bytes;
}

}
```

Measured before the change: 16.00 billion.

## Extend dense MFMA triangle core to a banded region of rows beyond K

Generalises the dense bit-matrix core from a KxK square to a region of up to 131072 rows. Each row bucket beyond K gets its own column bound, chosen by a cost model over a per-bucket 2D units table. Edges inside the region are skipped by the inline, light-edge and heavy-row streaming paths and counted by block-wise MFMA bit-matrix products instead. The aim is to move more intersection work from memory-bound streaming to matrix cores. The cost is a larger bitset (up to 512MB), a more complex block schedule, and a risk that the cost model misjudges where the crossover lies.

Result: no change. 16.07 billion, median of 6 (+0.4%).

```diff
diff --git a/gms_amd/capi.py b/gms_amd/capi.py
--- a/gms_amd/capi.py
+++ b/gms_amd/capi.py
@@ -440,7 +440,7 @@
     BREAKDOWN = ["hub_rows_list", "hub_rows_bitset", "hub_rows_delta", "tail_rows_list", "tail_rows_delta", "entries", "pivot_containers",
                  "of_which_inline_rows", "light_streamed_hub_rows", "light_streamed_tail_rows", "light_pivot_lists_and_descriptors",
                  "count_entries", "count_inline_entries", "count_work_items", "count_light_streamed_members",
-                 "core_matrix", "core_k", "reserved17", "reserved18", "reserved19", "reserved20"]
+                 "core_matrix", "core_k", "core_rows", "reserved18", "reserved19", "reserved20"]
     BREAKDOWN_BYTES = ("hub_rows_list", "hub_rows_bitset", "hub_rows_delta", "tail_rows_list", "tail_rows_delta", "entries", "pivot_containers",
                        "light_streamed_hub_rows", "light_streamed_tail_rows", "light_pivot_lists_and_descriptors", "core_matrix")
 
diff --git a/gms_amd/csrc/hip/device_graph.hip b/gms_amd/csrc/hip/device_graph.hip
--- a/gms_amd/csrc/hip/device_graph.hip
+++ b/gms_amd/csrc/hip/device_graph.hip
@@ -411,34 +411,43 @@
         }
     }
 }
-__global__ __launch_bounds__(256) void k_core_fill(int32_t K, int WS, const int64_t *__restrict__ hoff, const uint16_t *__restrict__ hadj,
+__global__ __launch_bounds__(256) void k_core_fill(TcRegionDev rg, int WS, const int64_t *__restrict__ hoff, const uint16_t *__restrict__ hadj,
                                                    uint32_t *__restrict__ bits) {
     const int lane = threadIdx.x & 63;
     const int32_t wave0 = int32_t((int64_t(blockIdx.x) * blockDim.x + threadIdx.x) >> 6);
     const int32_t nwaves = int32_t((int64_t(gridDim.x) * blockDim.x) >> 6);
-    for (int32_t i = wave0; i < K; i += nwaves)
+    for (int32_t i = wave0; i < rg.rows; i += nwaves) {
+        const uint32_t ji = uint32_t(rg.J(i));
         for (int64_t j = hoff[i] + lane; j < hoff[i + 1]; j += 64) {
             const uint32_t id = hadj[j];
-            if (id < uint32_t(i)) atomicOr(&bits[size_t(i) * size_t(WS) + (id >> 5)], 1u << (id & 31u));
-        }
-}
-__global__ __launch_bounds__(256) void k_core_units(int32_t cap, const int64_t *__restrict__ hoff, const uint16_t *__restrict__ hadj,
-                                                    const int32_t *__restrict__ dplus, unsigned long long *__restrict__ bucket) {
-    const int lane = threadIdx.x & 63;
+            if (id < ji) atomicOr(&bits[size_t(i) * size_t(WS) + (id >> 5)], 1u << (id & 31u));
+        }
+    }
+}
+__global__ __launch_bounds__(256) void k_core_units(int32_t rows, int32_t cap, int ncb, const int64_t *__restrict__ hoff, const uint16_t *__restrict__ hadj,
+                                                    const int32_t *__restrict__ dplus, unsigned long long *__restrict__ table) {
+    __shared__ unsigned long long col[4][kTcCoreCap / kTcCoreBucket];
+    const int lane = threadIdx.x & 63, wave = threadIdx.x >> 6;
+    auto wave_sync = [] {
+        __builtin_amdgcn_fence(__ATOMIC_ACQ_REL, "wavefront");
+        __builtin_amdgcn_wave_barrier();
+    };
     const int32_t wave0 = int32_t((int64_t(blockIdx.x) * blockDim.x + threadIdx.x) >> 6);
     const int32_t nwaves = int32_t((int64_t(gridDim.x) * blockDim.x) >> 6);
-    for (int32_t u = wave0; u < cap; u += nwaves) {
+    for (int32_t u = wave0; u < rows; u += nwaves) {
+        if (lane < kTcCoreCap / kTcCoreBucket) col[wave][lane] = 0;
+        wave_sync();
         const int64_t hb = hoff[u];
         const int hl = int(hoff[u + 1] - hb);
-        unsigned long long units = 0;
         for (int i = lane; i < hl; i += 64) {
             const uint32_t v = hadj[hb + i];
-            if (v >= uint32_t(u)) continue;
+            if (v >= uint32_t(u) || v >= uint32_t(cap)) continue;
             const uint32_t ids = uint32_t(min(i, dplus[v]));
-            units += min((ids + 7u) / 8u, (v + 127u) / 128u);
-        }
-        for (int s = 32; s > 0; s >>= 1) units += __shfl_down(units, s);
-        if (lane == 0 && units) atomicAdd(&bucket[u / kTcCoreBucket], units);
+            atomicAdd(&col[wave][v / kTcCoreBucket], (unsigned long long)min((ids + 7u) / 8u, (v + 127u) / 128u));
+        }
+        wave_sync();
+        if (lane < ncb && col[wave][lane]) atomicAdd(&table[size_t(u / kTcCoreBucket) * size_t(ncb) + lane], col[wave][lane]);
+        wave_sync();
     }
 }
 __global__ __launch_bounds__(256) void k_tail_split(int64_t n, const int64_t *__restrict__ toff, const int32_t *__restrict__ tadj, int32_t limit,
@@ -489,7 +498,7 @@
 template <bool FILL>
 __global__ __launch_bounds__(256) void k_inline_rows(int64_t first, int64_t end, const int32_t *__restrict__ order, const int64_t *__restrict__ hoff,
                                                      const uint16_t *__restrict__ hadj, const int64_t *__restrict__ toff, const int32_t *__restrict__ tadj,
-                                                     const int32_t *__restrict__ dplus, int32_t inline_limit, int inline_first, int32_t core, const int32_t *__restrict__ opos, int nparts, int part,
+                                                     const int32_t *__restrict__ dplus, int32_t inline_limit, int inline_first, TcRegionDev rg, const int32_t *__restrict__ opos, int nparts, int part,
                                                      unsigned long long *__restrict__ cnt_h,
                                                      unsigned long long *__restrict__ cnt_t, const int64_t *__restrict__ ihoff,
                                                      const int64_t *__restrict__ itoff, int64_t base_h, uint16_t *__restrict__ pool_h, int64_t base_t,
@@ -499,7 +508,8 @@
     const int64_t nwaves = (int64_t(gridDim.x) * blockDim.x) >> 6;
     for (int64_t pos = first + wave0; pos < end; pos += nwaves) {
         const int32_t u = order[pos];
-        if (u < core) continue;
+        const int32_t ju = rg.J(u);
+        if (ju >= u) continue;
         const int64_t hb = hoff[u], tb = toff[u];
         const int first_u = dplus[u] >= kHeavy ? inline_first : kInlineFirstMax;
         const int hl = min(int(hoff[u + 1] - hb), first_u), tl = min(int(toff[u + 1] - tb), first_u - hl);
@@ -514,7 +524,7 @@
         const unsigned long long vmask = __ballot(valid);
         const int nhub = __popcll(__ballot(valid && lane < hl));
         const int below = __popcll(vmask & ((1ull << lane) - 1ull));
-        const bool give = valid && below > 0 && takes_inline(mv, inline_limit, dplus);
+        const bool give = valid && below > 0 && mv >= ju && takes_inline(mv, inline_limit, dplus);
         const bool mine = give && (nparts <= 1 || shard_of(opos[mv], nparts) == part);
         const int nh = mine ? (is_tail ? nhub : below) : 0;
         const int nt = mine && is_tail ? lane - hl : 0;
@@ -609,7 +619,7 @@
 }
 
 __global__ void k_ledge_count(int64_t first, int64_t end, const int32_t *__restrict__ order, const int64_t *__restrict__ toff, const int32_t *__restrict__ tadj,
-                              const int32_t *__restrict__ tsplit, const int32_t *__restrict__ dplus, int32_t core, int64_t *__restrict__ cnt) {
+                              const int32_t *__restrict__ tsplit, const int32_t *__restrict__ dplus, TcRegionDev rg, int64_t *__restrict__ cnt) {
     const int64_t pos = first + int64_t(blockIdx.x) * blockDim.x + threadIdx.x;
     if (pos > end) return;
     int64_t c = 0;
@@ -617,25 +627,28 @@
         const int32_t u = order[pos];
         const int64_t tb = toff[u];
         const int tl = int(toff[u + 1] - tb);
-        if (u >= core)
-            for (int i = tsplit[u]; i < tl; ++i) c += dplus[tadj[tb + i]] < kHeavy ? 1 : 0;
+        const int32_t ju = rg.J(u);
+        for (int i = tsplit[u]; i < tl; ++i) {
+            const int32_t v = tadj[tb + i];
+            c += (v >= ju && dplus[v] < kHeavy) ? 1 : 0;
+        }
     }
     cnt[pos - first] = c;
 }
 __global__ void k_ledge_fill(int64_t first, int64_t end, const int32_t *__restrict__ order, const int64_t *__restrict__ hoff, const int64_t *__restrict__ toff,
                              const int32_t *__restrict__ tadj, const int32_t *__restrict__ tsplit, const int32_t *__restrict__ dplus,
-                             int32_t core, const int64_t *__restrict__ ebeg, int nparts, int part, uint4 *__restrict__ ledge) {
+                             TcRegionDev rg, const int64_t *__restrict__ ebeg, int nparts, int part, uint4 *__restrict__ ledge) {
     const int64_t pos = first + int64_t(blockIdx.x) * blockDim.x + threadIdx.x;
     if (pos >= end) return;
     const int32_t u = order[pos];
-    if (u < core) return;
+    const int32_t ju = rg.J(u);
     const int64_t hb = hoff[u], tb = toff[u];
     const int tl = int(toff[u + 1] - tb);
     const unsigned long long hu = (unsigned long long)hb | ((unsigned long long)(hoff[u + 1] - hb) << 40);
     int64_t e = ebeg[pos - first];
     for (int i = tsplit[u]; i < tl; ++i) {
         const int32_t v = tadj[tb + i];
-        if (dplus[v] >= kHeavy) continue;
+        if (v < ju || dplus[v] >= kHeavy) continue;
         if (nparts <= 1 || shard_of(e, nparts) == part) {
             const unsigned long long tu = (unsigned long long)tb | ((unsigned long long)i << 40);
             const unsigned long long hv = (unsigned long long)hoff[v] | ((unsigned long long)(hoff[v + 1] - hoff[v]) << 40);
@@ -695,7 +708,7 @@
                                                     uint32_t *__restrict__ cnt, uint32_t *__restrict__ cur, const int64_t *__restrict__ hbeg,
                                                     const int64_t *__restrict__ tbeg, TaskList htask, TaskList ttask,
                                                     int32_t *__restrict__ tunits, unsigned long long *__restrict__ reversed, const uint32_t *__restrict__ spool,
-                                                    const uint32_t *__restrict__ tpool, int32_t inline_limit, int inline_first, int32_t core, int nparts, int part, TcClasses cc) {
+                                                    const uint32_t *__restrict__ tpool, int32_t inline_limit, int inline_first, TcRegionDev rg, int nparts, int part, TcClasses cc) {
     const int kClasses = cc.count();
     const int lane = threadIdx.x & 63;
     const int64_t wave0 = (int64_t(blockIdx.x) * blockDim.x + threadIdx.x) >> 6;
@@ -703,7 +716,8 @@
     unsigned long long rev = 0;
     for (int64_t pos = wave0; pos < n_heavy; pos += nwaves) {
         const int32_t u = order[pos];
-        if (u < core) continue;
+        const int32_t ju = rg.J(u);
+        if (ju >= u) continue;
         const int64_t hb = hoff[u], tb = toff[u];
         const int hl = int(hoff[u + 1] - hb), tl = int(toff[u + 1] - tb);
         const unsigned long long du_s = srow[u], du_s2 = srow2[u], du_t = trow[u];
@@ -718,6 +732,7 @@
                 const uint32_t x = hadj[hb + i];
                 if (x != 0xFFFFu) v = int32_t(x);
             } else if (i < hl + tl) v = tadj[tb + i - hl];
+            if (v >= 0 && v < ju) v = -1;
             if (v >= 0 && i > 0 && i < inline_first && takes_inline(v, inline_limit, dplus)) v = -1;
             bool reverse = false;
             uint32_t ch = 0, ch2 = 0, ct = 0;
@@ -851,8 +866,10 @@
         p = nullptr;
     };
     drop(g->tsplit); drop(g->srow); drop(g->srow2); drop(g->ksplit); drop(g->spool); drop(g->trow); drop(g->htask.lo); drop(g->htask.hi); drop(g->ttask.lo); drop(g->ttask.hi); drop(g->hitem); drop(g->titem); drop(g->tunits);
-    drop(g->ledge); drop(g->tpool); drop(g->shard_hitem); drop(g->shard_titem); drop(g->core_bits);
-    g->tc_core = 0;
+    drop(g->ledge); drop(g->tpool); drop(g->shard_hitem); drop(g->shard_titem); drop(g->core_bits); drop(g->core_jtab); drop(g->core_blocks);
+    g->tc_core = g->tc_core_rows = 0;
+    g->core_blk_host.clear();
+    g->core_bytes_part = g->core_bytes_nparts = -1;
     g->shard_idx_part = g->shard_idx_nparts = -1;
     g->device_bytes -= g->tc_bytes;
     g->tc_bytes = 0;
@@ -892,6 +909,8 @@
     (void)hipFree(g->shard_titem);
     (void)hipFree(g->ledge);
     (void)hipFree(g->core_bits);
+    (void)hipFree(g->core_jtab);
+    (void)hipFree(g->core_blocks);
     (void)hipFree(g->tpool);
     (void)hipFree(g->dplus);
     (void)hipFree(g->order);
@@ -1242,31 +1261,64 @@
     {
         long long want = kTcCoreDefault;
         if (const char *e = opt("TC_CORE")) want = std::atoll(e);
-        g->tc_core = 0;
-        if (want > 0) g->tc_core = tc_core_clamp(want, hub_limit, n);
-        else if (want < 0) {
+        TcRegion region;
+        if (want > 0) {
+            long long rows = 0;
+            if (const char *e = opt("TC_CORE_ROWS")) rows = std::atoll(e);
+            region = tc_region_forced(tc_core_clamp(want, hub_limit, n), rows, n);
+        } else if (want < 0) {
             const int cap = tc_core_clamp(kTcCoreCap, hub_limit, n) / kTcCoreBucket * kTcCoreBucket;
             if (cap > 0) {
-                const int nbk = cap / kTcCoreBucket;
-                unsigned long long *bucket = nullptr;
-                if (int rc = dmalloc(&bucket, nbk, nullptr)) return rc;
-                DevGuard g_b{bucket};
-                GMSX_HIP(hipMemsetAsync(bucket, 0, size_t(nbk) * sizeof(unsigned long long), s));
-                hipLaunchKernelGGL(k_core_units, dim3(grid_for_waves(cap)), dim3(256), 0, s, cap, g->hoff, g->hadj, g->dplus, bucket);
-                std::vector<uint64_t> h(size_t(nbk), 0);
-                static_assert(sizeof(uint64_t) == sizeof(unsigned long long), "bucket words");
-                GMSX_HIP(hipMemcpyAsync(h.data(), bucket, size_t(nbk) * sizeof(uint64_t), hipMemcpyDeviceToHost, s));
+                const int32_t rows = int32_t(std::min<int64_t>(n, kTcRegionRowCap));
+                const int ncb = cap / kTcCoreBucket, nrb = (rows + kTcCoreBucket - 1) / kTcCoreBucket;
+                unsigned long long *table = nullptr;
+                if (int rc = dmalloc(&table, int64_t(nrb) * ncb, nullptr)) return rc;
+                DevGuard g_b{table};
+                GMSX_HIP(hipMemsetAsync(table, 0, size_t(nrb) * size_t(ncb) * sizeof(unsigned long long), s));
+                hipLaunchKernelGGL(k_core_units, dim3(grid_for_waves(rows)), dim3(256), 0, s, rows, int32_t(cap), ncb, g->hoff, g->hadj, g->dplus, table);
+                std::vector<uint64_t> h(size_t(nrb) * size_t(ncb), 0);
+                static_assert(sizeof(uint64_t) == sizeof(unsigned long long), "table words");
+                GMSX_HIP(hipMemcpyAsync(h.data(), table, h.size() * sizeof(uint64_t), hipMemcpyDeviceToHost, s));
                 GMSX_HIP(hipStreamSynchronize(s));
-                g->tc_core = choose_tc_core(h, cap);
+                if (const char *e = opt("TIMING"))
+                    if (std::atoi(e) >= 2)
+                        for (int rb = 0; rb < nrb; ++rb) {
+                            std::fprintf(stderr, "gmsx tc region units[%d]:", rb);
+                            for (int cb = 0; cb < ncb; ++cb) std::fprintf(stderr, " %llu", (unsigned long long)h[size_t(rb) * size_t(ncb) + size_t(cb)]);
+                            std::fprintf(stderr, "\n");
+                        }
+                region = choose_tc_region(h, nrb, ncb, cap);
+                tc_region_fit(region, n);
             }
         }
-        if (g->tc_core > 0) {
-            const int32_t K = g->tc_core;
-            const int WS = kc4m_stride(K);
-            const int64_t words = int64_t(K) * WS + 8;
+        g->tc_core = g->tc_core_rows = 0;
+        g->core_blk_host.clear();
+        g->core_bytes_part = g->core_bytes_nparts = -1;
+        if (region.k > 0) {
+            g->tc_core = region.k;
+            g->tc_core_rows = region.rows;
+            const int WS = kc4m_stride(region.k);
+            static_assert(kTcRegionMaxBytes / 4 + 8 < (1ull << 31), "Kc4mBlock::run forms word offsets in 32 bits");
+            const int64_t words = int64_t(region.rows) * WS + 8;
+            const int64_t nj = std::max<int64_t>(1, int64_t(region.jb.size()));
+            if (int rc = dmalloc(&g->core_jtab, nj, g)) return rc;
+            GMSX_HIP(hipMemsetAsync(g->core_jtab, 0, size_t(nj) * sizeof(int32_t), s));
+            if (!region.jb.empty()) GMSX_HIP(hipMemcpyAsync(g->core_jtab, region.jb.data(), region.jb.size() * sizeof(int32_t), hipMemcpyHostToDevice, s));
+            g->core_blk_host = tc_region_blocks(region);
+            if (opt("TIMING")) {
+                std::fprintf(stderr, "gmsx tc region: K=%d R=%d blocks=%zu bit-MACs=%.4g J/1024 of the buckets from K on:", region.k, region.rows, g->core_blk_host.size(),
+                             tc_region_bitmacs(g->core_blk_host));
+                for (size_t b = size_t(region.k / kTcCoreBucket); b < region.jb.size(); ++b)
+                    if (int64_t(b) * kTcCoreBucket >= region.k) std::fprintf(stderr, " %d", region.jb[b] / kTcCoreBucket);
+                std::fprintf(stderr, "\n");
+            }
+            if (int rc = dmalloc(&g->core_blocks, int64_t(g->core_blk_host.size()), g)) return rc;
+            if (!g->core_blk_host.empty())
+                GMSX_HIP(hipMemcpyAsync(g->core_blocks, g->core_blk_host.data(), g->core_blk_host.size() * sizeof(uint32_t), hipMemcpyHostToDevice, s));
             if (int rc = dmalloc(&g->core_bits, words, g)) return rc;
             GMSX_HIP(hipMemsetAsync(g->core_bits, 0, size_t(words) * sizeof(uint32_t), s));
-            hipLaunchKernelGGL(k_core_fill, dim3(grid_for_waves(K)), dim3(256), 0, s, K, WS, g->hoff, g->hadj, g->core_bits);
+            hipLaunchKernelGGL(k_core_fill, dim3(grid_for_waves(region.rows)), dim3(256), 0, s, g->region(), WS, g->hoff, g->hadj, g->core_bits);
+            GMSX_HIP(hipStreamSynchronize(s));
         }
     }
     pt.mark("core matrix");
@@ -1315,7 +1367,7 @@
         GMSX_HIP(hipMemsetAsync(inl_t, 0, size_t(n + 1) * sizeof(unsigned long long), s));
         if (n_work > 0)
             hipLaunchKernelGGL(k_inline_rows<false>, dim3(grid_for_waves(n_work)), dim3(256), 0, s, int64_t(0), n_work, g->order, g->hoff, g->hadj,
-                               g->toff, g->tadj, g->dplus, g->inline_limit, g->inline_first, g->tc_core, opos, g->shard_nparts, g->shard_part, inl_h, inl_t, ihoff, itoff, int64_t(0), static_cast<uint16_t *>(nullptr),
+                               g->toff, g->tadj, g->dplus, g->inline_limit, g->inline_first, g->region(), opos, g->shard_nparts, g->shard_part, inl_h, inl_t, ihoff, itoff, int64_t(0), static_cast<uint16_t *>(nullptr),
                                int64_t(0), static_cast<int32_t *>(nullptr));
         int64_t *uh = nullptr, *ut = nullptr;
         if (int rc = dmalloc(&uh, n + 1, nullptr)) return rc;
@@ -1433,7 +1485,7 @@
         GMSX_HIP(hipMemsetAsync(inl_h, 0, size_t(n + 1) * sizeof(unsigned long long), s));
         GMSX_HIP(hipMemsetAsync(inl_t, 0, size_t(n + 1) * sizeof(unsigned long long), s));
         hipLaunchKernelGGL(k_inline_rows<true>, dim3(grid_for_waves(n_work)), dim3(256), 0, s, int64_t(0), n_work, g->order, g->hoff, g->hadj, g->toff,
-                           g->tadj, g->dplus, g->inline_limit, g->inline_first, g->tc_core, opos, g->shard_nparts, g->shard_part, inl_h, inl_t, ihoff, itoff, inline_h_base, reinterpret_cast<uint16_t *>(g->spool),
+                           g->tadj, g->dplus, g->inline_limit, g->inline_first, g->region(), opos, g->shard_nparts, g->shard_part, inl_h, inl_t, ihoff, itoff, inline_h_base, reinterpret_cast<uint16_t *>(g->spool),
                            inline_t_base, reinterpret_cast<int32_t *>(g->tpool));
     }
     pt.mark("inline rows fill");
@@ -1446,7 +1498,7 @@
             DevGuard g_ec{ecnt};
             if (int rc = dmalloc(&ebeg, nl + 1, nullptr)) return rc;
             DevGuard g_eb{ebeg};
-            hipLaunchKernelGGL(k_ledge_count, dim3(unsigned(nl / 256 + 1)), dim3(256), 0, s, n_heavy, n_work, g->order, g->toff, g->tadj, g->tsplit, g->dplus, g->tc_core, ecnt);
+            hipLaunchKernelGGL(k_ledge_count, dim3(unsigned(nl / 256 + 1)), dim3(256), 0, s, n_heavy, n_work, g->order, g->toff, g->tadj, g->tsplit, g->dplus, g->region(), ecnt);
             if (int rc = exclusive_scan_i64(ecnt, ebeg, nl + 1, s)) return rc;
             GMSX_HIP(hipMemcpy(&g->ledge_total, ebeg + nl, sizeof(int64_t), hipMemcpyDeviceToHost));
             const int np = g->shard_nparts > 1 ? g->shard_nparts : 1, pp = g->shard_nparts > 1 ? g->shard_part : 0;
@@ -1455,7 +1507,7 @@
                 g->n_ledge = np <= 1 ? g->ledge_total : full + (((full & 1) ? np - 1 - pp : pp) < rem ? 1 : 0);
             }
             if (int rc = dmalloc(&g->ledge, 2 * g->n_ledge + 2, g)) return rc;
-            hipLaunchKernelGGL(k_ledge_fill, dim3(unsigned(nl / 256 + 1)), dim3(256), 0, s, n_heavy, n_work, g->order, g->hoff, g->toff, g->tadj, g->tsplit, g->dplus, g->tc_core, ebeg,
+            hipLaunchKernelGGL(k_ledge_fill, dim3(unsigned(nl / 256 + 1)), dim3(256), 0, s, n_heavy, n_work, g->order, g->hoff, g->toff, g->tadj, g->tsplit, g->dplus, g->region(), ebeg,
                                np, pp, g->ledge);
             GMSX_HIP(hipStreamSynchronize(s));
         }
@@ -1524,7 +1576,7 @@
         if (n_heavy > 0)
             hipLaunchKernelGGL(k_task_lists<false>, dim3(grid), dim3(256), 0, s, n_heavy, g->order, g->hoff, g->hadj, g->toff, g->tadj, g->dplus, g->srow, g->srow2, g->ksplit, g->trow,
                                two_sided, opos, cnt, cur, hbeg, tbeg, TaskList{}, TaskList{}, g->tunits,
-                               totals + 2, g->spool, g->tpool, g->inline_limit, g->inline_first, g->tc_core, g->shard_nparts, g->shard_part, cc);
+                               totals + 2, g->spool, g->tpool, g->inline_limit, g->inline_first, g->region(), g->shard_nparts, g->shard_part, cc);
         pt.mark("task lists count");
         hipLaunchKernelGGL(k_list_sizes, dim3(unsigned(n_recv / 256 + 1)), dim3(256), 0, s, n_recv, cnt, hcnt, tcnt, cc);
         if (int rc = exclusive_scan_i64(hcnt, hbeg, n_recv + 1, s)) return rc;
@@ -1547,7 +1599,7 @@
                                inline_t_base, cnt, cur, hbeg, tbeg, g->htask, g->ttask, totals, cc);
         if (n_heavy > 0)
             hipLaunchKernelGGL(k_task_lists<true>, dim3(grid), dim3(256), 0, s, n_heavy, g->order, g->hoff, g->hadj, g->toff, g->tadj, g->dplus, g->srow, g->srow2, g->ksplit, g->trow,
-                               two_sided, opos, cnt, cur, hbeg, tbeg, g->htask, g->ttask, g->tunits, totals + 2, g->spool, g->tpool, g->inline_limit, g->inline_first, g->tc_core, g->shard_nparts, g->shard_part, cc);
+                               two_sided, opos, cnt, cur, hbeg, tbeg, g->htask, g->ttask, g->tunits, totals + 2, g->spool, g->tpool, g->inline_limit, g->inline_first, g->region(), g->shard_nparts, g->shard_part, cc);
         pt.mark("task lists fill");
         const int hub_phases = cc.hub_phases();
         const int64_t slots = int64_t(hub_phases) * n_recv;
diff --git a/gms_amd/csrc/hip/device_graph.hpp b/gms_amd/csrc/hip/device_graph.hpp
--- a/gms_amd/csrc/hip/device_graph.hpp
+++ b/gms_amd/csrc/hip/device_graph.hpp
@@ -2,6 +2,7 @@
 #include <hip/hip_runtime.h>
 
 #include <cstdint>
+#include <vector>
 
 #include "gmsx.h"
 #include "gmsx_internal.hpp"
@@ -23,6 +24,11 @@
     uint32_t reserved[7];
 };
 static_assert(sizeof(gmsx_tc_item) == 64, "work item record = one 64-byte line");
+struct TcRegionDev {
+    int32_t k, rows;
+    const int32_t *jtab;
+    __device__ __forceinline__ int32_t J(int32_t u) const { return u < k ? u : (u < rows ? jtab[u >> 10] : 0); }
+};
 constexpr uint32_t kTaskHubUnitsMax = (1u << 14) - 1, kTaskTailUnitsMax = (1u << 15) - 1;
 struct TaskList {
     uint32_t *lo = nullptr;
@@ -75,8 +81,13 @@
     int64_t n_ledge = 0, ledge_total = 0;
     uint32_t *core_bits = nullptr;
     int32_t tc_core = 0;
-    mutable int core_bytes_k = -1, core_bytes_part = -1, core_bytes_nparts = -1;
+    int32_t tc_core_rows = 0;
+    int32_t *core_jtab = nullptr;
+    uint32_t *core_blocks = nullptr;
+    std::vector<uint32_t> core_blk_host;
+    mutable int core_bytes_part = -1, core_bytes_nparts = -1;
     mutable uint64_t core_bytes = 0;
+    TcRegionDev region() const { return TcRegionDev{tc_core, tc_core_rows, core_jtab}; }
     int tc_hot_windows = 0;
     uint32_t tc_window_units = 1;
     int tc_hot_min = 0;
diff --git a/gms_amd/csrc/hip/tc.hip b/gms_amd/csrc/hip/tc.hip
--- a/gms_amd/csrc/hip/tc.hip
+++ b/gms_amd/csrc/hip/tc.hip
@@ -660,7 +660,7 @@
     block_add(total, red, lane, wave, tid, acc);
 }
 
-__global__ __launch_bounds__(1024) void k_tc_core(const uint32_t *__restrict__ bits, int WS, int K, int nb, int nblk, int part, int nparts,
+__global__ __launch_bounds__(1024) void k_tc_core(const uint32_t *__restrict__ bits, int WS, int R, const uint32_t *__restrict__ blocks, int nblk, int part, int nparts,
                                                   unsigned long long *__restrict__ acc) {
     __shared__ unsigned long long red[16];
     auto lane_id = [] { return int(__builtin_amdgcn_mbcnt_hi(~0u, __builtin_amdgcn_mbcnt_lo(~0u, 0u))); };
@@ -672,14 +672,11 @@
     for (int j = 0;; ++j) {
         const int sidx = (8 * j + ((j & 1) ? 7 - x : x)) * Q + q;
         if (sidx >= ns) break;
-        const int t = sidx * nparts + part;
-        int c = int((__builtin_sqrtf(8.0f * float(t) + 1.0f) - 1.0f) * 0.5f);
-        while (c * (c + 1) / 2 > t) --c;
-        while ((c + 1) * (c + 2) / 2 <= t) ++c;
-        const int bj = nb - 1 - c, bi = bj + (t - c * (c + 1) / 2);
+        const uint32_t b = uni32(int(blocks[sidx * nparts + part]));
+        const int bi = int(b & 0xffffu), bj = int(b >> 16);
         int lane = lane_id();
         asm volatile("" : "+v"(lane));
-        cnt += Kc4mBlock<2>::run(bits, WS, K, bi, bj, lane);
+        cnt += Kc4mBlock<2>::run(bits, WS, R, bi, bj, lane);
     }
     const int lane = lane_id();
     unsigned long long total = cnt;
@@ -696,7 +693,7 @@
 __global__ __launch_bounds__(256) void k_tc_stats(const int64_t *__restrict__ hoff, const uint16_t *__restrict__ hadj,
                                                   const int64_t *__restrict__ toff, const int32_t *__restrict__ tadj,
                                                   const int32_t *__restrict__ dplus, const int32_t *__restrict__ order,
-                                                  const int32_t *__restrict__ tunits, int32_t inline_limit, int inline_first, int32_t core, int64_t end, int nparts, int part,
+                                                  const int32_t *__restrict__ tunits, int32_t inline_limit, int inline_first, TcRegionDev rg, int64_t end, int nparts, int part,
                                                   unsigned long long *__restrict__ out) {
     const int lane = threadIdx.x & 63;
     const int64_t wave0 = (int64_t(blockIdx.x) * blockDim.x + threadIdx.x) >> 6;
@@ -708,25 +705,26 @@
         const int du = dplus[u];
         if (du >= kHeavy) {
             if (lane == 0) units += (unsigned long long)tunits[pos];
-            if (u < core) {
-                if (lane == 0) units += (unsigned long long)du;
-                continue;
-            }
+            const int32_t ju = rg.J(u);
+            if (ju > 0)
+                for (int64_t j = hoff[u] + lane; j < hoff[u + 1]; j += 64) units += int32_t(hadj[j]) < ju ? 1ull : 0ull;
+            if (ju >= u) continue;
             const int hl = min(int(hoff[u + 1] - hoff[u]), inline_first), tl = min(int(toff[u + 1] - toff[u]), inline_first - hl);
             int32_t v = -1;
             if (lane < hl) {
                 const uint32_t x = hadj[hoff[u] + lane];
                 if (x != 0xFFFFu) v = int32_t(x);
             } else if (lane - hl < tl) v = tadj[toff[u] + lane - hl];
-            if (v >= 0 && lane > 0 && (v < inline_limit || dplus[v] >= kHeavy)) ++units;
+            if (v >= ju && lane > 0 && (v < inline_limit || dplus[v] >= kHeavy)) ++units;
             continue;
         }
         const int hl = int(hoff[u + 1] - hoff[u]);
         if (lane == 0) units += (unsigned long long)du;
-        if (du < 2 || u < core) continue;
+        if (du < 2) continue;
+        const int32_t ju = rg.J(u);
         for (int64_t j = toff[u] + lane; j < toff[u + 1]; j += 64) {
             const int32_t v = tadj[j];
-            if (v < inline_limit || dplus[v] >= kHeavy) continue;
+            if (v < ju || v < inline_limit || dplus[v] >= kHeavy) continue;
             const unsigned long long hv = (unsigned long long)(hoff[v + 1] - hoff[v]), tv = (unsigned long long)(toff[v + 1] - toff[v]);
             bytes += 32ull + 2ull * hl + 4ull * (unsigned long long)(j - toff[u]) + 2ull * hv + 4ull * tv;
             probes += hv + tv;
@@ -780,7 +778,7 @@
                                                       const int32_t *__restrict__ dplus, const int32_t *__restrict__ order,
                                                       const TaskList htask, const gmsx_tc_item *__restrict__ hitem, int64_t hitems,
                                                       const TaskList ttask, const gmsx_tc_item *__restrict__ titem, int64_t titems,
-                                                      int32_t inline_limit, int32_t core, int64_t first_light, int64_t end_light,
+                                                      int32_t inline_limit, TcRegionDev rg, int64_t first_light, int64_t end_light,
                                                       unsigned long long *__restrict__ out) {
     const int lane = threadIdx.x & 63;
     const int64_t wave0 = (int64_t(blockIdx.x) * blockDim.x + threadIdx.x) >> 6;
@@ -808,12 +806,12 @@
     }
     for (int64_t pos = first_light + wave0; pos < end_light; pos += nwaves) {
         const int32_t u = order[pos];
-        if (u < core) continue;
+        const int32_t ju = rg.J(u);
         const int64_t tb0 = toff[u], te = toff[u + 1];
         const unsigned long long hl = (unsigned long long)(hoff[u + 1] - hoff[u]);
         for (int64_t j = tb0 + lane; j < te; j += 64) {
             const int32_t v = tadj[j];
-            if (v < inline_limit || dplus[v] >= kHeavy) continue;
+            if (v < ju || v < inline_limit || dplus[v] >= kHeavy) continue;
             c[8] += 2ull * (unsigned long long)(hoff[v + 1] - hoff[v]);
             c[9] += 4ull * (unsigned long long)(toff[v + 1] - toff[v]);
             c[10] += 32ull + 2ull * hl + 4ull * (unsigned long long)(j - tb0);
@@ -933,9 +931,8 @@
 static int tc_one(const gmsx_graph *g, int part, int nparts, int cpart, int cnparts, uint64_t *partial, gmsx_stats *st);
 static uint64_t core_bytes_of(const gmsx_graph *g, int part, int nparts) {
     if (g->tc_core <= 0 || nparts < 1) return 0;
-    if (!(g->core_bytes_k == g->tc_core && g->core_bytes_part == part && g->core_bytes_nparts == nparts)) {
-        g->core_bytes = tc_core_bytes(g->tc_core, part, nparts);
-        g->core_bytes_k = g->tc_core;
+    if (!(g->core_bytes_part == part && g->core_bytes_nparts == nparts)) {
+        g->core_bytes = tc_region_bytes(g->core_blk_host, part, nparts);
         g->core_bytes_part = part;
         g->core_bytes_nparts = nparts;
     }
@@ -1064,12 +1061,16 @@
     }
     const bool run_core = g->tc_core > 0 && cnparts > 0 && !only;
     if (run_core) {
-        const int K = g->tc_core, nb = (K + 63) / 64, nblk = int(tc_core_blocks(K));
+        const int nblk = int(g->core_blk_host.size());
         const int64_t ns = (int64_t(nblk) - cpart + cnparts - 1) / cnparts;
         if (ns > 0) {
             const int64_t wgs = std::max<int64_t>(8, std::min<int64_t>(cus / 8 * 8, ((ns + 15) / 16 + 7) / 8 * 8));
-            hipLaunchKernelGGL(k_tc_core, dim3(unsigned(wgs)), dim3(1024), 0, s, g->core_bits, kc4m_stride(K), K, nb, nblk, cpart, cnparts, acc);
-            ++launches;
+            const int cuts = int((ns + wgs * 16 * 2047 - 1) / (wgs * 16 * 2047));
+            for (int cut = 0; cut < cuts; ++cut) {
+                hipLaunchKernelGGL(k_tc_core, dim3(unsigned(wgs)), dim3(1024), 0, s, g->core_bits, kc4m_stride(g->tc_core), g->tc_core_rows, g->core_blocks, nblk,
+                                   cpart + cut * cnparts, cnparts * cuts, acc);
+                ++launches;
+            }
         }
     }
     if (persist) {
@@ -1116,7 +1117,7 @@
         if (g->n > 0) {
             const int64_t blocks = std::min<int64_t>((g->n + 3) / 4, cap_blocks);
             hipLaunchKernelGGL(k_tc_stats, dim3(unsigned(blocks)), dim3(256), 0, s, g->hoff, g->hadj, g->toff, g->tadj, g->dplus, g->order,
-                               g->tunits, g->inline_limit, g->inline_first, g->tc_core, g->n, nparts, part, acc + kAccSlots * kAccStride);
+                               g->tunits, g->inline_limit, g->inline_first, g->region(), g->n, nparts, part, acc + kAccSlots * kAccStride);
         }
         if (g->hitems > 0)
             hipLaunchKernelGGL(k_tc_item_stats, dim3(unsigned(std::min<int64_t>((g->hitems + 3) / 4, cap_blocks))), dim3(256), 0, s, g->hoff, 2, 0, g->htask, g->hitem,
@@ -1179,7 +1180,7 @@
         GMSX_HIP(hipMemsetAsync(acc, 0, 21 * 8, s));
         const int cus = ctx().compute_units > 0 ? ctx().compute_units : 256;
         hipLaunchKernelGGL(k_tc_breakdown, dim3(unsigned(cus * 16)), dim3(256), 0, s, g->hoff, g->toff, g->tadj, g->dplus, g->order, g->htask,
-                           g->hitem, g->hitems, g->ttask, g->titem, g->titems, g->inline_limit, g->tc_core, n_block, n_work, acc);
+                           g->hitem, g->hitems, g->ttask, g->titem, g->titems, g->inline_limit, g->region(), n_block, n_work, acc);
         GMSX_HIP(hipMemcpyAsync(out21, acc, 21 * 8, hipMemcpyDeviceToHost, s));
         GMSX_HIP(hipStreamSynchronize(s));
         GMSX_HIP(hipGetLastError());
@@ -1187,6 +1188,7 @@
         out21[12] = uint64_t(g->inline_hentries + g->inline_tentries);
         out21[15] = core_bytes_of(g, 0, 1);
         out21[16] = uint64_t(g->tc_core);
+        out21[17] = uint64_t(g->tc_core_rows);
         return GMSX_OK;
     });
 }
diff --git a/gms_amd/csrc/host/loader.cpp b/gms_amd/csrc/host/loader.cpp
--- a/gms_amd/csrc/host/loader.cpp
+++ b/gms_amd/csrc/host/loader.cpp
@@ -677,7 +677,7 @@
     {"INLINE_LIMIT", "", false}, {"TC_INLINE_FIRST", "", false}, {"TC_DELTA", "", false}, {"TC_DELTA_PCT", "", false}, {"TC_GAP12", "", false},
     {"TC_HYBRID", "", false}, {"TC_TAIL_DELTA", "", false}, {"TC_TWO_SIDED", "", false}, {"TC_HOT_WINDOWS", "", false}, {"TC_HOT_KB", "", false},
     {"TC_HOT_MIN", "", false}, {"TC_TEST_MAX_UNITS", "", false}, {"TC_KEEP_ROWS", "", false}, {"TC_MEM_LIMIT_MB", "", false}, {"TC_OVERLAP", "", false},
-    {"TC_PERSIST", "", false}, {"TC_ITEM_WGS", "", false}, {"TC_CORE", "", false}, {"SORT_CHUNK", "", false}, {"UPLOAD_STAGED", "", false}, {"INIT_LAZY", "", false},
+    {"TC_PERSIST", "", false}, {"TC_ITEM_WGS", "", false}, {"TC_CORE", "", false}, {"TC_CORE_ROWS", "", false}, {"SORT_CHUNK", "", false}, {"UPLOAD_STAGED", "", false}, {"INIT_LAZY", "", false},
     {"KC_SLAB_MB", "", false}, {"KC_MAXD", "", false}, {"KC_STREAMS", "", false}, {"KC_PIPE_ALL", "", false}, {"KC_STREAM_BUILD", "", false},
     {"KC_REVERSE", "", false}, {"KC_REV_MIN", "", false}, {"KC_REV_FACTOR", "", false}, {"KC_REV_TAIL", "", false}, {"KC_REV_TAIL_MIN", "", false}, {"KC_REV_GW", "", false}, {"KC_TRI", "", false}, {"KC_MFMA", "", false}, {"KC_POOL_MB", "", false},
     {"BK_MAXC", "", false}, {"BK_ARENA_MB", "", false}, {"BK_GROUPS", "", false}, {"BK_SMALL_P", "", false}, {"BK_SMALL_P_GROUPS", "", false},
diff --git a/gms_amd/csrc/host/tc_core_plan.hpp b/gms_amd/csrc/host/tc_core_plan.hpp
--- a/gms_amd/csrc/host/tc_core_plan.hpp
+++ b/gms_amd/csrc/host/tc_core_plan.hpp
@@ -49,4 +49,113 @@
     return bytes;
 }
 
+constexpr int kTcRegionRowCap = 131072;
+constexpr unsigned long long kTcRegionMaxBytes = 512ull << 20;
+constexpr double kTcRegionBandRateShare = 1.40e15 / 1.7e15;
+constexpr double kTcRegionBandRealised = 0.65;
+struct TcRegion {
+    int k = 0, rows = 0;
+    std::vector<int32_t> jb;
+    int col_bound(long long u) const { return u < k ? int(u) : (u < rows ? jb[size_t(u / kTcCoreBucket)] : 0); }
+    bool empty() const { return rows <= 0; }
+};
+inline int tc_region_stride_words(int k) { return (((k + 31) >> 5) + 7) & ~7; }
+inline void tc_region_fit(TcRegion &r, long long n) {
+    long long rows = std::max<long long>(r.k, std::min<long long>(std::min<long long>(r.rows, n), kTcRegionRowCap));
+    const unsigned long long row_bytes = 4ull * (unsigned long long)tc_region_stride_words(r.k);
+    if (r.k > 0 && (unsigned long long)rows * row_bytes > kTcRegionMaxBytes) rows = std::max<long long>(r.k, (long long)(kTcRegionMaxBytes / row_bytes));
+    while (rows > r.k && ((rows - 1) / kTcCoreBucket >= (long long)r.jb.size() || r.jb[size_t((rows - 1) / kTcCoreBucket)] <= 0))
+        rows = std::max<long long>(r.k, (rows - 1) / kTcCoreBucket * kTcCoreBucket);
+    r.rows = r.k > 0 ? int(rows) : 0;
+    r.jb.resize(size_t((r.rows + kTcCoreBucket - 1) / kTcCoreBucket), 0);
+    for (int32_t &j : r.jb) j = std::max<int32_t>(0, std::min<int32_t>(j, r.k));
 }
+inline TcRegion tc_region_forced(int k, long long want_rows, long long n) {
+    TcRegion r;
+    r.k = k;
+    r.rows = int(std::max<long long>(k, std::min<long long>(want_rows, kTcRegionRowCap)));
+    r.jb.assign(size_t((r.rows + kTcCoreBucket - 1) / kTcCoreBucket), k);
+    tc_region_fit(r, n);
+    return r;
+}
+inline double tc_region_band_cost(int c) {
+    const double nbj = 16.0 * c;
+    return 16.0 * 262144.0 * nbj * (nbj + 1.0) / 2.0;
+}
+inline double tc_region_cost(const TcRegion &r, double band_rate_share = kTcRegionBandRateShare) {
+    double c = double(r.k) * double(r.k) * double(r.k) / 6.0;
+    for (size_t b = size_t(r.k / kTcCoreBucket); b < r.jb.size(); ++b)
+        if ((long long)b * kTcCoreBucket >= r.k) c += tc_region_band_cost((r.jb[b] + kTcCoreBucket - 1) / kTcCoreBucket) / band_rate_share;
+    return c;
+}
+inline TcRegion choose_tc_region(const std::vector<uint64_t> &table, int nrb, int ncb, int cap, double b_stream = kTcCoreStreamBytesPerSec,
+                                 double r_core = kTcCoreBitMacsPerSec, double launch_sec = kTcCoreLaunchSec,
+                                 double band_rate_share = kTcRegionBandRateShare, double band_realised = kTcRegionBandRealised) {
+    TcRegion best_r;
+    double best = 0.0;
+    const int kb_max = std::min(std::min(nrb, ncb), cap / kTcCoreBucket);
+    unsigned long long units = 0;
+    std::vector<int32_t> jb(size_t(std::max(nrb, 0)), 0);
+    for (int kb = 1; kb <= kb_max; ++kb) {
+        for (int cb = 0; cb < ncb; ++cb) units += table[size_t(kb - 1) * size_t(ncb) + size_t(cb)];
+        const double k = double(kb) * kTcCoreBucket;
+        double gain = double(units) * 16.0 / b_stream - (k * k * k / 6.0) / r_core - launch_sec;
+        std::fill(jb.begin(), jb.end(), 0);
+        int last = kb;
+        for (int rb = kb; rb < nrb; ++rb) {
+            unsigned long long saved = 0;
+            double band = 0.0;
+            for (int c = 1; c <= kb; ++c) {
+                saved += table[size_t(rb) * size_t(ncb) + size_t(c - 1)];
+                const double x = band_realised * double(saved) * 16.0 / b_stream - tc_region_band_cost(c) / (band_rate_share * r_core);
+                if (x > band) {
+                    band = x;
+                    jb[size_t(rb)] = c * kTcCoreBucket;
+                }
+            }
+            if (band > 0.0) {
+                gain += band;
+                last = rb + 1;
+            }
+        }
+        if (gain > best) {
+            best = gain;
+            best_r.k = kb * kTcCoreBucket;
+            best_r.rows = last * kTcCoreBucket;
+            best_r.jb.assign(jb.begin(), jb.begin() + last);
+        }
+    }
+    return best_r;
+}
+
+inline std::vector<uint32_t> tc_region_blocks(const TcRegion &r) {
+    const int nbi = (r.rows + 63) / 64;
+    std::vector<int> nbj(size_t(nbi), 0);
+    int top = 0;
+    for (int bi = 0; bi < nbi; ++bi) {
+        const long long lo = 64ll * bi, hi = std::min<long long>(lo + 64, r.rows);
+        long long cb = 0;
+        if (lo < r.k) cb = std::min<long long>(hi, r.k);
+        if (hi > r.k) cb = std::max<long long>(cb, r.col_bound(hi - 1));
+        nbj[size_t(bi)] = int(std::min<long long>((cb + 63) / 64, bi + 1));
+        top = std::max(top, nbj[size_t(bi)]);
+    }
+    std::vector<uint32_t> out;
+    for (int bj = top - 1; bj >= 0; --bj)
+        for (int bi = bj; bi < nbi; ++bi)
+            if (nbj[size_t(bi)] > bj) out.push_back(uint32_t(bi) | (uint32_t(bj) << 16));
+    return out;
+}
+inline unsigned long long tc_region_bytes(const std::vector<uint32_t> &blocks, int part, int nparts) {
+    unsigned long long bytes = 0;
+    for (size_t t = 0; t < blocks.size(); ++t)
+        if (nparts <= 1 || int(t % size_t(nparts)) == part) bytes += tc_core_block_bytes(int(blocks[t] >> 16));
+    return bytes;
+}
+inline double tc_region_bitmacs(const std::vector<uint32_t> &blocks) {
+    double s = 0.0;
+    for (uint32_t b : blocks) s += 262144.0 * double((b >> 16) + 1);
+    return s;
+}
+
+}
```
